# angelocatalani/neural-network-compression

Hardware: AMD Instinct MI355X
Metric: weights/sec through prune+k-means (K=256) (higher is better)
Workload: dtype f32

## Files before the change

include/nnc.h:

```cpp
#ifndef NNC_H
#define NNC_H

#include <stddef.h>
#include <stdint.h>

#ifdef __cplusplus
extern "C" {
#endif

#define NNC_VERSION 100

#define NNC_OK 0
#define NNC_EINVAL (-1)
#define NNC_ENOSPACE (-2)
#define NNC_EHIP (-3)
#define NNC_ENODEV (-4)

#define NNC_KMAX 1040
#define NNC_CHUNK 8192

int nnc_version(void);
const char *nnc_last_error(void);
int nnc_device_info(char *arch_out, size_t arch_len, int *cu_count_out);


int nnc_chunk_sums_f32(const float *x, int64_t n, int sqdev, const float *mean_dev, float *chunk_out,
                       void *stream);

#define NNC_FOLD_SUM 0
#define NNC_FOLD_MEAN 1
#define NNC_FOLD_STD 2
int nnc_fold_f32(const float *chunks, int64_t nchunks, int64_t count, int op, const float *scale_dev,
                 float *out_dev, void *stream);


size_t nnc_prune_workspace_bytes(int64_t n);

int nnc_prune_f32(float *x, int64_t n, float q, int std_smooth, uint8_t *mask, float *stats_dev,
                  int64_t *nzeroed_dev, void *ws, size_t ws_bytes, void *stream);

size_t nnc_prune_stats_workspace_bytes(int64_t n);
int nnc_prune_stats_f32(float *x, int64_t n, float q, int std_smooth, uint8_t *mask, float *stats_dev, int64_t *nzeroed_dev,
                        float *minmax4_dev, int64_t *signs_dev, void *ws, size_t ws_bytes, void *stream);

int nnc_threshold_mask_f32(float *x, int64_t n, const float *thr_dev, uint8_t *mask, int64_t *nzeroed_dev,
                           void *stream);

int nnc_apply_mask_f32(float *x, const uint8_t *mask, int64_t n, void *stream);


size_t nnc_minmax_workspace_bytes(int64_t n);
int nnc_minmax_f32(const float *x, int64_t n, int skip_zeros, float *out_dev, int64_t *count_dev, void *ws,
                   size_t ws_bytes, void *stream);

int nnc_minmax_signs_f32(const float *x, int64_t n, float *out_dev, int64_t *signs_dev, void *ws, size_t ws_bytes,
                         void *stream);

int32_t nnc_sort_pruned_bounded_bits(float vmin, float vmax, float thr, int64_t n_neg, int64_t n_pos);
size_t nnc_sort_pruned_bounded_workspace_bytes(int64_t n_nonzero);
const int32_t *nnc_sort_pruned_bounded_flag(void *ws, int64_t n_nonzero);
int nnc_sort_pruned_bounded_f32(const float *x, int64_t n, int64_t n_neg, int64_t n_zero, float vmin, float vmax, float thr,
                                float *sorted_out, void *ws, size_t ws_bytes, void *stream);

size_t nnc_layer_stats_workspace_bytes(int64_t n);
int nnc_layer_stats_f32(const float *x, int64_t n, float *out6_dev, int64_t *signs_dev, void *ws, size_t ws_bytes,
                        void *stream);

int nnc_rank_sorted_f32(const float *x_sorted, int64_t n, const float *values_dev, int32_t m, int64_t *ranks_out_dev, void *stream);
int nnc_hist31_f32(const float *x, int64_t n, int skip_zeros, const float *steps32_dev, int64_t *counts_dev,
                   void *stream);


size_t nnc_sort_workspace_bytes(int64_t n);
int nnc_sort_f32(const float *x, int64_t n, float *sorted_out, void *ws, size_t ws_bytes, void *stream);
size_t nnc_sort_pruned_workspace_bytes(int64_t n, int64_t n_neg, int64_t n_zero);
int nnc_sort_pruned_f32(const float *x, int64_t n, int64_t n_neg, int64_t n_zero, float *sorted_out, void *ws,
                        size_t ws_bytes, void *stream);

typedef struct nnc_kmeans_params {
    int64_t n;
    int64_t n_total;
    int32_t k;
    int32_t max_iter;
    int32_t fix_shift;
    int32_t grid_log2;
    int32_t replicas_log2;
    int32_t flags;
    float x_mean;
    float tol;
    float lo, hi;
    const int64_t *prefix_dev;
} nnc_kmeans_params;

#define NNC_KM_TWO_LAUNCH 1
#define NNC_KM_LOOP 2
#define NNC_KM_MASS_IN_PLACE 4
#define NNC_KM_LOOP_KMAX 64

typedef struct nnc_kmeans_status {
    int32_t iter;
    int32_t done;
    int32_t paused;
    int32_t n_empty;
    float shift_tot;
    float tol;
    int32_t k;
    int32_t same_counts;
    int32_t reloc_ties;
    int32_t reloc_multi;
    int32_t n_relocated;
    int32_t n_unproven;
    int32_t n_in_place;
    int32_t n_reloc_null;
} nnc_kmeans_status;

int32_t nnc_fix_shift(float absmax, int64_t n_total);
size_t nnc_kmeans_workspace_bytes(int32_t k);

#define NNC_PREFIX_BLOCK 256
size_t nnc_kmeans_prefix_bytes(int64_t n);
int nnc_kmeans_loop_stats(void *ws, int32_t *out8, void *stream);
int nnc_kmeans_prefix_build(const float *x_sorted, const nnc_kmeans_params *p, int64_t *prefix_dev, void *stream);

int nnc_kmeans_init(void *ws, size_t ws_bytes, const nnc_kmeans_params *p, const float *centers_init_dev,
                    void *stream);
int nnc_kmeans_set_centers(void *ws, const nnc_kmeans_params *p, const float *centers_dev, int centred, void *stream);
int nnc_kmeans_accumulate(const float *x, void *ws, const nnc_kmeans_params *p, void *stream);
int64_t *nnc_kmeans_partials(void *ws);
int nnc_kmeans_finalize(void *ws, int resume, void *stream);
int nnc_kmeans_iterate(const float *x, void *ws, const nnc_kmeans_params *p, int32_t iters, void *stream);
int nnc_kmeans_status_async(void *ws, nnc_kmeans_status *host_out, void *stream);
int nnc_kmeans_status_publish(void *ws, void *host_mapped, uint64_t ticket, void *stream);
int nnc_kmeans_iterate_publish(const float *x, void *ws, const nnc_kmeans_params *p, int32_t iters, void *host_mapped,
                               uint64_t ticket, void *stream);
int nnc_kmeans_fit(const float *x_iter, void *ws, const nnc_kmeans_params *p, int32_t max_batch, int32_t sorted,
                   void *reloc_scratch_dev, size_t reloc_scratch_bytes, void *host_mapped, uint64_t *ticket_io,
                   nnc_kmeans_status *status_out, int32_t *n_windowed_out, void *stream);
int nnc_kmeans_set_done(void *ws, int32_t done_code, void *stream);
int nnc_kmeans_label_counts(const float *x, void *ws, const nnc_kmeans_params *p, int which, int64_t *counts_dev,
                            void *stream);

int nnc_kmeans_get_centers(void *ws, int which, int centred, float *out_dev, void *stream);

int nnc_kmeans_assign(const float *x, void *ws, const nnc_kmeans_params *p, int which, void *labels_out,
                      int label_bytes, float *quant_out, float *dist_out, int64_t *dist_hist4096_dev, void *stream);

int nnc_topm_hist_f32(const float *d, int64_t n, int32_t shift, int32_t width, int32_t prefix_shift, uint32_t prefix,
                      int64_t *hist4096_dev, void *stream);
int nnc_topm_compact_f32(const float *d, const float *x, int64_t n, uint32_t thr_bits, int64_t *keys_dev,
                         int64_t cap, int64_t *count_dev, void *stream);

int nnc_kmeans_relocate(void *ws, const int64_t *keys_sorted_dev, int32_t nkeys, void *stream);

int nnc_kmeans_reloc_candidates(const float *x_sorted, void *ws, const nnc_kmeans_params *p, int32_t window,
                                float *cand_x_dev, int64_t cap, void *win_dev, int32_t *meta_dev, void *stream);
int nnc_kmeans_relocate_checked(void *ws, const float *cand_x_dev, const float *cand_d_dev, const void *win_dev,
                                const int32_t *meta_dev, int32_t n_empty, int64_t *keys_out_dev, void *stream);
int32_t nnc_kmeans_reloc_window(int64_t n, int32_t n_empty);
size_t nnc_kmeans_reloc_scratch_bytes(int32_t k, int32_t window);
int nnc_kmeans_relocate_windowed(const float *x_sorted, void *ws, const nnc_kmeans_params *p, int32_t n_empty,
                                 void *scratch_dev, size_t scratch_bytes, void *stream);
int nnc_kmeans_reloc_select_local(const float *x_sorted, void *ws, const nnc_kmeans_params *p, int32_t n_empty,
                                  void *scratch_dev, size_t scratch_bytes, int64_t *keys_out_dev, void *stream);
int32_t *nnc_kmeans_reloc_flag(void *ws);
int nnc_kmeans_relocate_if_proven(void *ws, const int64_t *keys_sorted_dev, int32_t nkeys, void *stream);
int nnc_labels_equal(const void *a, const void *b, int64_t n, int label_bytes, int32_t *flag_dev, void *stream);
int nnc_ref_sums_f32(const float *x, int64_t n, float x_mean, const void *labels, int32_t label_bytes, int32_t k,
                     float *sums_out_dev, int64_t *counts_out_dev, void *stream);
int nnc_kmeans_set_done_if(void *ws, const int32_t *flag_dev, int32_t done_code, void *stream);

int nnc_bincount(const void *labels, int label_bytes, int64_t n, int32_t k, int64_t *counts_dev, void *stream);

#define NNC_REF_NMAX 4096
#define NNC_REF_KMAX 128
int nnc_kmeans_fit_reference_f32(const float *x, int32_t n, const float *centers_init_dev, int32_t k, int32_t max_iter, float tol,
                                 uint8_t *labels_out, float *values_out, float *centers_out, int64_t *counts_out,
                                 void *result_dev, void *stream);

#define NNC_INIT_LINEAR 0
#define NNC_INIT_DENSITY 1
#define NNC_LAYER_DONE 0
#define NNC_LAYER_HOST 1
#define NNC_ARITH_FIXED 0
#define NNC_ARITH_REFERENCE 1
typedef struct nnc_layer_params {
    float q;
    int32_t prune;
    int32_t std_smooth;
    int32_t bits;
    int32_t mode;
    int32_t want_values;
    int32_t km_flags;
    int32_t reserved;
} nnc_layer_params;
typedef struct nnc_layer_result {
    int32_t status, k, label_bytes, arith;
    int32_t n_iter, stop, n_relocations, n_reloc_windowed, reloc_ties, reloc_multi;
    float sigma, threshold;
    int64_t n_zeroed, total_bits;
    float centers[NNC_KMAX];
    int64_t counts[NNC_KMAX];
    uint8_t code_lengths[NNC_KMAX];
} nnc_layer_result;
size_t nnc_compress_layer_workspace_bytes(int64_t n, int32_t k);
size_t nnc_compress_layer_host_bytes(void);
int nnc_compress_layer_f32(float *x, int64_t n, const nnc_layer_params *p, uint8_t *mask_out, void *labels_out, float *values_out,
                           void *ws_dev, size_t ws_bytes, void *host_pinned, size_t host_bytes, uint64_t *ticket_io,
                           nnc_layer_result *result, void *stream);
int nnc_host_linspace_f32(float start, float stop, int32_t num, float *out);
int nnc_host_cdf(const float *steps32, const int64_t *counts31, float *xnew300, double *cdf300);
int nnc_host_density_init(const float *xnew300, const double *cdf300, int32_t bits, float *space_out);

int32_t nnc_kmeanspp_trials(int32_t k);
size_t nnc_kmeanspp_workspace_bytes(int64_t n, int32_t k);
int nnc_kmeanspp_seed_f32(const float *x, int64_t n, float x_mean, int32_t k, int64_t first_id, const double *uniforms_dev,
                          float *seeds_out_dev, int64_t *seed_ids_out_dev, void *ws, size_t ws_bytes, void *stream);

int nnc_centroid_grad_f32(const float *grad, const void *labels, int label_bytes, int64_t n, int32_t k, int32_t fix_shift,
                          int64_t *sums_dev, int64_t *counts_dev, int64_t *nonfinite_dev, void *stream);
int nnc_gather_f32(const float *centers_dev, int32_t k, const void *labels, int label_bytes, int64_t n, float *out, void *stream);

int64_t nnc_cbmm_workspace_bytes(int64_t m, int64_t kdim, int64_t ncols, int label_bytes);
#define NNC_CBMM_NONE 0
#define NNC_CBMM_STREAM 1
#define NNC_CBMM_TILED 2
#define NNC_CBMM_BIAS 3
#define NNC_CBMM_P_PATH 0
#define NNC_CBMM_P_VB 1
#define NNC_CBMM_P_MT 2
#define NNC_CBMM_P_COPIES 3
#define NNC_CBMM_P_ENTRIES 4
#define NNC_CBMM_P_SPLITS 5
#define NNC_CBMM_P_RPS 6
#define NNC_CBMM_P_ALIGNED 7
#define NNC_CBMM_P_LDS 8
#define NNC_CBMM_P_COL_TILES 9
#define NNC_CBMM_P_ROW_TILES 10
#define NNC_CBMM_P_WORKSPACE 11
#define NNC_CBMM_PLAN_LEN 12
int nnc_cbmm_plan(int64_t m, int64_t kdim, int64_t ncols, int label_bytes, int32_t k, int32_t cus, uint64_t labels_addr, int64_t *out);
int nnc_cbmm_f32(const float *x, int64_t m, int64_t kdim, const void *labels, int label_bytes, int64_t ncols, const float *centers_dev, int32_t k,
                 const float *bias_dev, int32_t relu, float *y, void *workspace, int64_t workspace_bytes, void *stream);

#define NNC_DT_F32 0
#define NNC_DT_BF16 1
#define NNC_DT_F16 2
#define NNC_CBMM_MFMA 5
#define NNC_CBMM_H16_P_DTYPE 12
#define NNC_CBMM_H16_PLAN_LEN 13
int64_t nnc_cbmm_h16_workspace_bytes(int64_t m, int64_t kdim, int64_t ncols, int label_bytes);
int nnc_cbmm_h16_plan(int x_dtype, int64_t m, int64_t kdim, int64_t ncols, int label_bytes, int32_t k, int32_t cus, uint64_t labels_addr, int64_t *out);
int nnc_cbmm_h16(const void *x, int x_dtype, int64_t m, int64_t kdim, const void *labels, int label_bytes, int64_t ncols, const float *centers_dev,
                 int32_t k, const float *bias_dev, int32_t relu, void *y, int y_dtype, void *workspace, int64_t workspace_bytes, void *stream);

#define NNC_CBMM_GROUPED_P_GROUP_ROWS 13
#define NNC_CBMM_GROUPED_P_GROUPS 14
#define NNC_CBMM_GROUPED_P_MAX_GROUPS_PER_SPLIT 15
#define NNC_CBMM_GROUPED_PLAN_LEN 16
int64_t nnc_cbmm_grouped_workspace_bytes(int x_dtype, int64_t m, int64_t kdim, int64_t ncols);
int nnc_cbmm_grouped_plan(int x_dtype, int64_t m, int64_t kdim, int64_t ncols, int32_t k, int64_t group_rows, int32_t cus, uint64_t labels_addr, int64_t *out);
int nnc_cbmm_grouped(const void *x, int x_dtype, int64_t m, int64_t kdim, const void *labels, int64_t ncols, const float *centers_dev, int32_t k,
                     int64_t group_rows, const float *bias_dev, int32_t relu, void *y, int y_dtype, void *workspace, int64_t workspace_bytes, void *stream);

#define NNC_CBMM_ZERO 4
#define NNC_CBDX_P_PATH 0
#define NNC_CBDX_P_VB 1
#define NNC_CBDX_P_MT 2
#define NNC_CBDX_P_COPIES 3
#define NNC_CBDX_P_ENTRIES 4
#define NNC_CBDX_P_SPLITS 5
#define NNC_CBDX_P_CPS 6
#define NNC_CBDX_P_ALIGNED 7
#define NNC_CBDX_P_LDS 8
#define NNC_CBDX_P_COL_TILES 9
#define NNC_CBDX_P_ROW_TILES 10
#define NNC_CBDX_P_WORKSPACE 11
#define NNC_CBDX_PLAN_LEN 12
#define NNC_CBDC_P_PATH 0
#define NNC_CBDC_P_VB 1
#define NNC_CBDC_P_MT 2
#define NNC_CBDC_P_COPIES 3
#define NNC_CBDC_P_SPLITS 4
#define NNC_CBDC_P_RPS 5
#define NNC_CBDC_P_ALIGNED 6
#define NNC_CBDC_P_LDS 7
#define NNC_CBDC_P_COL_TILES 8
#define NNC_CBDC_P_ROW_TILES 9
#define NNC_CBDC_P_TERMS_LOG2 10
#define NNC_CBDC_P_WORKSPACE 11
#define NNC_CBDC_PLAN_LEN 12
int64_t nnc_cbmm_dx_workspace_bytes(int64_t m, int64_t kdim, int64_t ncols, int label_bytes);
int nnc_cbmm_dx_plan(int64_t m, int64_t kdim, int64_t ncols, int label_bytes, int32_t k, int32_t cus, uint64_t labels_addr, int64_t *out);
int nnc_cbmm_dx_f32(const float *g, int64_t m, int64_t kdim, const void *labels, int label_bytes, int64_t ncols, const float *centers_dev, int32_t k,
                    float *dx, void *workspace, int64_t workspace_bytes, void *stream);
// ... 221 lines not shown
```

neural_network_compression_amd/_native.py:

```python
from __future__ import annotations

import ctypes
import os

from . import build as _build

c_void_p = ctypes.c_void_p
c_int = ctypes.c_int
c_i32 = ctypes.c_int32
c_i64 = ctypes.c_int64
c_f32 = ctypes.c_float
c_size = ctypes.c_size_t

NNC_OK = 0
NNC_KMAX = 1040
NNC_CHUNK = 8192
FOLD_SUM, FOLD_MEAN, FOLD_STD = 0, 1, 2
NNC_KM_TWO_LAUNCH = 1
NNC_KM_LOOP = 2
NNC_KM_MASS_IN_PLACE = 4
NNC_KM_LOOP_KMAX = 64
CBMM_NONE, CBMM_STREAM, CBMM_TILED, CBMM_BIAS = 0, 1, 2, 3
CBMM_PLAN_LEN = 12
CBMM_PLAN_FIELDS = ("path", "vb", "mt", "copies", "entries", "splits", "rps", "aligned", "lds", "col_tiles", "row_tiles", "workspace")
# ... 24 lines not shown
CBPK_PLAN_LEN = 14
CBPK_PLAN_FIELDS = ("path", "vb", "mt", "cols", "xrows", "table", "copies", "entries", "splits", "rps", "lds", "col_tiles", "row_tiles", "workspace")
CBPK_GROUPED_PLAN_LEN = 19
CBPK_GROUPED_PLAN_FIELDS = CBPK_PLAN_FIELDS + ("dtype", "group_rows", "groups", "max_groups_per_split", "tables")
CBPKDX_PLAN_LEN = 12
CBPKDX_PLAN_FIELDS = ("path", "vb", "mt", "cols", "copies", "entries", "splits", "cps", "lds", "col_tiles", "row_tiles", "workspace")
CBPKDC_PLAN_LEN = 12
CBPKDC_PLAN_FIELDS = ("path", "vb", "mt", "cols", "copies", "splits", "rps", "lds", "col_tiles", "row_tiles", "terms_log2", "workspace")
CBPKGRAD_GROUPED_PLAN_LEN = 17
_CBPKGRAD_GROUPED_TAIL = _CBGRAD_GROUPED_TAIL + ("held",)
CBPKDX_GROUPED_PLAN_FIELDS = CBPKDX_PLAN_FIELDS + _CBPKGRAD_GROUPED_TAIL
CBPKDC_GROUPED_PLAN_FIELDS = CBPKDC_PLAN_FIELDS + _CBPKGRAD_GROUPED_TAIL
CBSPDX_PLAN_LEN = 11
CBSPDX_PLAN_FIELDS = ("path", "mt", "segs", "copies", "entries", "splits", "cps", "lds", "col_tiles", "row_tiles", "workspace")
CBSPDC_PLAN_LEN = 11
CBSPDC_PLAN_FIELDS = ("path", "mt", "segs", "copies", "splits", "rps", "lds", "col_tiles", "row_tiles", "terms_log2", "workspace")
CBSPGRAD_H16_PLAN_LEN = 12
CBSPDX_H16_PLAN_FIELDS = CBSPDX_PLAN_FIELDS + ("dtype",)
CBSPDC_H16_PLAN_FIELDS = CBSPDC_PLAN_FIELDS + ("dtype",)


class NativeLibraryError(RuntimeError):
    pass


class NncError(RuntimeError):
    def __init__(self, code: int, message: str):
        super().__init__(f"nnc error {code}: {message}")
        self.code = code


class KMeansParams(ctypes.Structure):
    _fields_ = [
        ("n", c_i64), ("n_total", c_i64), ("k", c_i32), ("max_iter", c_i32), ("fix_shift", c_i32),
        ("grid_log2", c_i32), ("replicas_log2", c_i32), ("flags", c_i32),
        ("x_mean", c_f32), ("tol", c_f32), ("lo", c_f32), ("hi", c_f32),
        ("prefix_dev", c_void_p),
    ]


class KMeansStatus(ctypes.Structure):
    _fields_ = [
        ("iter", c_i32), ("done", c_i32), ("paused", c_i32), ("n_empty", c_i32),
        ("shift_tot", c_f32), ("tol", c_f32), ("k", c_i32), ("same_counts", c_i32),
        ("reloc_ties", c_i32), ("reloc_multi", c_i32), ("n_relocated", c_i32), ("n_unproven", c_i32),
        ("n_in_place", c_i32), ("n_reloc_null", c_i32),
    ]


class LayerParams(ctypes.Structure):
    _fields_ = [("q", c_f32), ("prune", c_i32), ("std_smooth", c_i32), ("bits", c_i32), ("mode", c_i32), ("want_values", c_i32),
                ("km_flags", c_i32), ("reserved", c_i32)]


class LayerResult(ctypes.Structure):
    _fields_ = [
        ("status", c_i32), ("k", c_i32), ("label_bytes", c_i32), ("arith", c_i32),
        ("n_iter", c_i32), ("stop", c_i32), ("n_relocations", c_i32), ("n_reloc_windowed", c_i32), ("reloc_ties", c_i32), ("reloc_multi", c_i32),
        ("sigma", c_f32), ("threshold", c_f32),
        ("n_zeroed", c_i64), ("total_bits", c_i64),
        ("centers", c_f32 * NNC_KMAX), ("counts", c_i64 * NNC_KMAX), ("code_lengths", ctypes.c_uint8 * NNC_KMAX),
    ]


SIGNATURES = {
    "nnc_version": (c_int, []),
    "nnc_last_error": (ctypes.c_char_p, []),
    "nnc_device_info": (c_int, [ctypes.c_char_p, c_size, ctypes.POINTER(c_int)]),
    "nnc_chunk_sums_f32": (c_int, [c_void_p, c_i64, c_int, c_void_p, c_void_p, c_void_p]),
    "nnc_fold_f32": (c_int, [c_void_p, c_i64, c_i64, c_int, c_void_p, c_void_p, c_void_p]),
    "nnc_prune_workspace_bytes": (c_size, [c_i64]),
    "nnc_prune_f32": (c_int, [c_void_p, c_i64, c_f32, c_int, c_void_p, c_void_p, c_void_p, c_void_p, c_size, c_void_p]),
    "nnc_sort_pruned_bounded_bits": (c_i32, [c_f32, c_f32, c_f32, c_i64, c_i64]),
    "nnc_sort_pruned_bounded_workspace_bytes": (c_size, [c_i64]),
    "nnc_sort_pruned_bounded_flag": (c_void_p, [c_void_p, c_i64]),
    "nnc_sort_pruned_bounded_f32": (c_int, [c_void_p, c_i64, c_i64, c_i64, c_f32, c_f32, c_f32, c_void_p, c_void_p, c_size, c_void_p]),
    "nnc_prune_stats_workspace_bytes": (c_size, [c_i64]),
    "nnc_prune_stats_f32": (c_int, [c_void_p, c_i64, c_f32, c_int, c_void_p, c_void_p, c_void_p, c_void_p, c_void_p, c_void_p, c_size, c_void_p]),
    "nnc_threshold_mask_f32": (c_int, [c_void_p, c_i64, c_void_p, c_void_p, c_void_p, c_void_p]),
    "nnc_apply_mask_f32": (c_int, [c_void_p, c_void_p, c_i64, c_void_p]),
    "nnc_minmax_workspace_bytes": (c_size, [c_i64]),
    "nnc_minmax_f32": (c_int, [c_void_p, c_i64, c_int, c_void_p, c_void_p, c_void_p, c_size, c_void_p]),
    "nnc_minmax_signs_f32": (c_int, [c_void_p, c_i64, c_void_p, c_void_p, c_void_p, c_size, c_void_p]),
    "nnc_layer_stats_workspace_bytes": (c_size, [c_i64]),
    "nnc_layer_stats_f32": (c_int, [c_void_p, c_i64, c_void_p, c_void_p, c_void_p, c_size, c_void_p]),
    "nnc_rank_sorted_f32": (c_int, [c_void_p, c_i64, c_void_p, c_i32, c_void_p, c_void_p]),
    "nnc_hist31_f32": (c_int, [c_void_p, c_i64, c_int, c_void_p, c_void_p, c_void_p]),
    "nnc_sort_workspace_bytes": (c_size, [c_i64]),
    "nnc_sort_f32": (c_int, [c_void_p, c_i64, c_void_p, c_void_p, c_size, c_void_p]),
    "nnc_sort_pruned_workspace_bytes": (c_size, [c_i64, c_i64, c_i64]),
    "nnc_sort_pruned_f32": (c_int, [c_void_p, c_i64, c_i64, c_i64, c_void_p, c_void_p, c_size, c_void_p]),
    "nnc_fix_shift": (c_i32, [c_f32, c_i64]),
    "nnc_kmeans_workspace_bytes": (c_size, [c_i32]),
    "nnc_kmeans_prefix_bytes": (c_size, [c_i64]),
    "nnc_kmeans_loop_stats": (c_int, [c_void_p, c_void_p, c_void_p]),
    "nnc_kmeans_prefix_build": (c_int, [c_void_p, ctypes.POINTER(KMeansParams), c_void_p, c_void_p]),
    "nnc_kmeans_init": (c_int, [c_void_p, c_size, ctypes.POINTER(KMeansParams), c_void_p, c_void_p]),
    "nnc_kmeans_set_centers": (c_int, [c_void_p, ctypes.POINTER(KMeansParams), c_void_p, c_int, c_void_p]),
    "nnc_kmeans_accumulate": (c_int, [c_void_p, c_void_p, ctypes.POINTER(KMeansParams), c_void_p]),
    "nnc_kmeans_partials": (c_void_p, [c_void_p]),
    "nnc_kmeans_finalize": (c_int, [c_void_p, c_int, c_void_p]),
    "nnc_kmeans_iterate": (c_int, [c_void_p, c_void_p, ctypes.POINTER(KMeansParams), c_i32, c_void_p]),
    "nnc_kmeans_status_async": (c_int, [c_void_p, ctypes.POINTER(KMeansStatus), c_void_p]),
    "nnc_kmeans_status_publish": (c_int, [c_void_p, c_void_p, ctypes.c_uint64, c_void_p]),
    "nnc_kmeans_iterate_publish": (c_int, [c_void_p, c_void_p, ctypes.POINTER(KMeansParams), c_i32, c_void_p, ctypes.c_uint64, c_void_p]),
    "nnc_kmeans_fit": (c_int, [c_void_p, c_void_p, ctypes.POINTER(KMeansParams), c_i32, c_i32, c_void_p, c_size, c_void_p,
                               ctypes.POINTER(ctypes.c_uint64), ctypes.POINTER(KMeansStatus), ctypes.POINTER(c_i32), c_void_p]),
    "nnc_kmeans_fit_sharded": (c_int, [c_void_p, c_void_p, c_void_p, ctypes.POINTER(KMeansParams), ctypes.c_int64, c_i32, c_i32, c_void_p, c_size,
                                       c_void_p, ctypes.POINTER(ctypes.c_uint64), ctypes.POINTER(KMeansStatus), ctypes.POINTER(c_i32), c_void_p]),
    "nnc_kmeans_set_done": (c_int, [c_void_p, c_i32, c_void_p]),
    "nnc_kmeans_label_counts": (c_int, [c_void_p, c_void_p, ctypes.POINTER(KMeansParams), c_int, c_void_p, c_void_p]),
    "nnc_kmeans_get_centers": (c_int, [c_void_p, c_int, c_int, c_void_p, c_void_p]),
    "nnc_kmeans_assign": (c_int, [c_void_p, c_void_p, ctypes.POINTER(KMeansParams), c_int, c_void_p, c_int, c_void_p, c_void_p, c_void_p, c_void_p]),
    "nnc_topm_hist_f32": (c_int, [c_void_p, c_i64, c_i32, c_i32, c_i32, ctypes.c_uint32, c_void_p, c_void_p]),
    "nnc_topm_compact_f32": (c_int, [c_void_p, c_void_p, c_i64, ctypes.c_uint32, c_void_p, c_i64, c_void_p, c_void_p]),
    "nnc_kmeans_relocate": (c_int, [c_void_p, c_void_p, c_i32, c_void_p]),
    "nnc_kmeans_reloc_candidates": (c_int, [c_void_p, c_void_p, ctypes.POINTER(KMeansParams), c_i32, c_void_p, c_i64, c_void_p, c_void_p, c_void_p]),
    "nnc_kmeans_relocate_checked": (c_int, [c_void_p, c_void_p, c_void_p, c_void_p, c_void_p, c_i32, c_void_p, c_void_p]),
    "nnc_kmeans_reloc_window": (c_i32, [c_i64, c_i32]),
    "nnc_kmeans_reloc_scratch_bytes": (c_size, [c_i32, c_i32]),
    "nnc_kmeans_relocate_windowed": (c_int, [c_void_p, c_void_p, ctypes.POINTER(KMeansParams), c_i32, c_void_p, c_size, c_void_p]),
    "nnc_kmeans_reloc_select_local": (c_int, [c_void_p, c_void_p, ctypes.POINTER(KMeansParams), c_i32, c_void_p, c_size, c_void_p, c_void_p]),
    "nnc_kmeans_reloc_flag": (c_void_p, [c_void_p]),
    "nnc_kmeans_relocate_if_proven": (c_int, [c_void_p, c_void_p, c_i32, c_void_p]),
    "nnc_labels_equal": (c_int, [c_void_p, c_void_p, c_i64, c_int, c_void_p, c_void_p]),
    "nnc_ref_sums_f32": (c_int, [c_void_p, c_i64, ctypes.c_float, c_void_p, c_i32, c_i32, c_void_p, c_void_p, c_void_p]),
    "nnc_kmeans_set_done_if": (c_int, [c_void_p, c_void_p, c_i32, c_void_p]),
    "nnc_bincount": (c_int, [c_void_p, c_int, c_i64, c_i32, c_void_p, c_void_p]),
    "nnc_kmeans_fit_reference_f32": (c_int, [c_void_p, c_i32, c_void_p, c_i32, c_i32, c_f32, c_void_p, c_void_p, c_void_p, c_void_p, c_void_p, c_void_p]),
    "nnc_compress_layer_workspace_bytes": (c_size, [c_i64, c_i32]),
    "nnc_compress_layer_host_bytes": (c_size, []),
    "nnc_compress_layer_f32": (c_int, [c_void_p, c_i64, ctypes.POINTER(LayerParams), c_void_p, c_void_p, c_void_p, c_void_p, c_size, c_void_p, c_size,
                                       ctypes.POINTER(ctypes.c_uint64), ctypes.POINTER(LayerResult), c_void_p]),
    "nnc_host_linspace_f32": (c_int, [c_f32, c_f32, c_i32, c_void_p]),
    "nnc_host_cdf": (c_int, [c_void_p, c_void_p, c_void_p, c_void_p]),
    "nnc_host_density_init": (c_int, [c_void_p, c_void_p, c_i32, c_void_p]),
    "nnc_kmeanspp_trials": (c_i32, [c_i32]),
    "nnc_kmeanspp_workspace_bytes": (c_size, [c_i64, c_i32]),
    "nnc_kmeanspp_seed_f32": (c_int, [c_void_p, c_i64, c_f32, c_i32, c_i64, c_void_p, c_void_p, c_void_p, c_void_p, c_size, c_void_p]),
    "nnc_centroid_grad_f32": (c_int, [c_void_p, c_void_p, c_int, c_i64, c_i32, c_i32, c_void_p, c_void_p, c_void_p, c_void_p]),
    "nnc_gather_f32": (c_int, [c_void_p, c_i32, c_void_p, c_int, c_i64, c_void_p, c_void_p]),
    "nnc_cbmm_workspace_bytes": (c_i64, [c_i64, c_i64, c_i64, c_int]),
    "nnc_cbmm_plan": (c_int, [c_i64, c_i64, c_i64, c_int, c_i32, c_i32, ctypes.c_uint64, ctypes.POINTER(c_i64)]),
    "nnc_cbmm_f32": (c_int, [c_void_p, c_i64, c_i64, c_void_p, c_int, c_i64, c_void_p, c_i32, c_void_p, c_i32, c_void_p, c_void_p, c_i64, c_void_p]),
    "nnc_cbmm_h16_workspace_bytes": (c_i64, [c_i64, c_i64, c_i64, c_int]),
    "nnc_cbmm_h16_plan": (c_int, [c_int, c_i64, c_i64, c_i64, c_int, c_i32, c_i32, ctypes.c_uint64, ctypes.POINTER(c_i64)]),
    "nnc_cbmm_h16": (c_int, [c_void_p, c_int, c_i64, c_i64, c_void_p, c_int, c_i64, c_void_p, c_i32, c_void_p, c_i32, c_void_p, c_int, c_void_p, c_i64,
                             c_void_p]),
    "nnc_cbmm_grouped_workspace_bytes": (c_i64, [c_int, c_i64, c_i64, c_i64]),
    "nnc_cbmm_grouped_plan": (c_int, [c_int, c_i64, c_i64, c_i64, c_i32, c_i64, c_i32, ctypes.c_uint64, ctypes.POINTER(c_i64)]),
    "nnc_cbmm_grouped": (c_int, [c_void_p, c_int, c_i64, c_i64, c_void_p, c_i64, c_void_p, c_i32, c_i64, c_void_p, c_i32, c_void_p, c_int, c_void_p, c_i64,
                                 c_void_p]),
    "nnc_cbmm_dx_workspace_bytes": (c_i64, [c_i64, c_i64, c_i64, c_int]),
    "nnc_cbmm_dx_plan": (c_int, [c_i64, c_i64, c_i64, c_int, c_i32, c_i32, ctypes.c_uint64, ctypes.POINTER(c_i64)]),
    "nnc_cbmm_dx_f32": (c_int, [c_void_p, c_i64, c_i64, c_void_p, c_int, c_i64, c_void_p, c_i32, c_void_p, c_void_p, c_i64, c_void_p]),
    "nnc_cbmm_dc_workspace_bytes": (c_i64, [c_i64, c_i64, c_i64, c_int, c_i32]),
    "nnc_cbmm_dc_plan": (c_int, [c_i64, c_i64, c_i64, c_int, c_i32, c_i32, ctypes.c_uint64, ctypes.POINTER(c_i64)]),
    "nnc_cbmm_dc_f32": (c_int, [c_void_p, c_void_p, c_i64, c_i64, c_void_p, c_int, c_i64, c_i32, c_void_p, c_i32, c_void_p, c_i64, c_void_p]),
    "nnc_cbsp_pack_bytes": (c_i64, [c_i64, c_i64, c_int, c_i64]),
    "nnc_cbsp_pack": (c_int, [c_void_p, c_int, c_i64, c_i64, c_i32, c_void_p, c_i64, c_void_p, c_void_p]),
    "nnc_cbsp_unpack": (c_int, [c_void_p, c_i64, c_int, c_i64, c_i64, c_i32, c_i64, c_void_p, c_void_p]),
    "nnc_cbsp_workspace_bytes": (c_i64, [c_i64, c_i64, c_i64, c_int]),
    "nnc_cbsp_plan": (c_int, [c_i64, c_i64, c_i64, c_int, c_i32, c_i32, ctypes.POINTER(c_i64)]),
    "nnc_cbsp_f32": (c_int, [c_void_p, c_i64, c_i64, c_void_p, c_i64, c_int, c_i64, c_i32, c_i64, c_void_p, c_i32, c_void_p, c_i32, c_void_p,
                             c_void_p, c_i64, c_void_p]),
    "nnc_cbsp_dx_workspace_bytes": (c_i64, [c_i64, c_i64, c_i64, c_int]),
    "nnc_cbsp_dx_plan": (c_int, [c_i64, c_i64, c_i64, c_int, c_i32, c_i32, ctypes.POINTER(c_i64)]),
    "nnc_cbsp_dx_f32": (c_int, [c_void_p, c_i64, c_i64, c_void_p, c_i64, c_int, c_i64, c_i32, c_i64, c_void_p, c_i32, c_void_p, c_void_p, c_i64,
                                c_void_p]),
    "nnc_cbsp_dc_workspace_bytes": (c_i64, [c_i64, c_i64, c_i64, c_int, c_i32]),
    "nnc_cbsp_dc_plan": (c_int, [c_i64, c_i64, c_i64, c_int, c_i32, c_i32, ctypes.POINTER(c_i64)]),
    "nnc_cbsp_dc_f32": (c_int, [c_void_p, c_void_p, c_i64, c_i64, c_void_p, c_i64, c_int, c_i64, c_i32, c_i64, c_i32, c_void_p, c_i32, c_void_p,
                                c_i64, c_void_p]),
    "nnc_cbpk_row_bytes": (c_i64, [c_i64, c_int]),
    "nnc_cbpk_pack_bytes": (c_i64, [c_i64, c_i64, c_int]),
    "nnc_cbpk_pack": (c_int, [c_void_p, c_int, c_i64, c_i64, c_int, c_void_p, c_i64, c_void_p, c_void_p]),
    "nnc_cbpk_unpack": (c_int, [c_void_p, c_i64, c_int, c_i64, c_i64, c_void_p, c_int, c_void_p]),
    "nnc_cbpk_workspace_bytes": (c_i64, [c_i64, c_i64, c_i64, c_int]),
    "nnc_cbpk_plan": (c_int, [c_i64, c_i64, c_i64, c_int, c_i32, c_i32, ctypes.POINTER(c_i64)]),
    "nnc_cbpk_f32": (c_int, [c_void_p, c_i64, c_i64, c_void_p, c_i64, c_int, c_i64, c_void_p, c_i32, c_void_p, c_i32, c_void_p, c_void_p, c_i64,
                             c_void_p]),
    "nnc_cbpk_grouped_workspace_bytes": (c_i64, [c_int, c_i64, c_i64, c_i64, c_int]),
    "nnc_cbpk_grouped_plan": (c_int, [c_int, c_i64, c_i64, c_i64, c_int, c_i32, c_i64, c_i32, ctypes.POINTER(c_i64)]),
    "nnc_cbpk_grouped": (c_int, [c_void_p, c_int, c_i64, c_i64, c_void_p, c_i64, c_int, c_i64, c_void_p, c_i32, c_i64, c_void_p, c_i32, c_void_p, c_int,
                                 c_void_p, c_i64, c_void_p]),
    "nnc_cbpk_dx_workspace_bytes": (c_i64, [c_i64, c_i64, c_i64, c_int]),
    "nnc_cbpk_dx_plan": (c_int, [c_i64, c_i64, c_i64, c_int, c_i32, c_i32, ctypes.POINTER(c_i64)]),
    "nnc_cbpk_dx_f32": (c_int, [c_void_p, c_i64, c_i64, c_void_p, c_i64, c_int, c_i64, c_void_p, c_i32, c_void_p, c_void_p, c_i64, c_void_p]),
    "nnc_cbpk_dc_workspace_bytes": (c_i64, [c_i64, c_i64, c_i64, c_int, c_i32]),
    "nnc_cbpk_dc_plan": (c_int, [c_i64, c_i64, c_i64, c_int, c_i32, c_i32, ctypes.POINTER(c_i64)]),
    "nnc_cbpk_dc_f32": (c_int, [c_void_p, c_void_p, c_i64, c_i64, c_void_p, c_i64, c_int, c_i64, c_i32, c_void_p, c_i32, c_void_p, c_i64, c_void_p]),
    "nnc_huffman_codes": (c_int, [ctypes.POINTER(ctypes.c_uint8), c_i32, ctypes.POINTER(ctypes.c_uint32)]),
    "nnc_codec_chunks": (c_size, [c_i64]),
    "nnc_huffman_chunk_offsets": (c_int, [c_void_p, c_int, c_i64, c_void_p, c_i32, c_void_p, c_void_p]),
    "nnc_huffman_encode": (c_int, [c_void_p, c_int, c_i64, c_void_p, c_void_p, c_i32, c_void_p, c_void_p, c_i64, c_void_p]),
    "nnc_huffman_decode_tables_bytes": (c_size, []),
    "nnc_huffman_decode_tables": (c_int, [ctypes.POINTER(ctypes.c_uint8), c_i32, c_void_p, c_size]),
    "nnc_huffman_decode": (c_int, [c_void_p, c_void_p, c_i64, c_void_p, c_i32, c_void_p, c_int, c_void_p, c_void_p]),
    "nnc_sparse_entry_offsets": (c_int, [c_void_p, c_int, c_i64, c_i32, c_i32, c_void_p, c_void_p]),
    "nnc_sparse_emit": (c_int, [c_void_p, c_int, c_i64, c_i32, c_i32, c_void_p, c_void_p, c_void_p, c_void_p]),
    "nnc_sparse_expand": (c_int, [c_void_p, c_void_p, c_int, c_void_p, c_i64, c_i32, c_void_p, c_void_p, c_void_p]),
    "nnc_comm_unique_id": (c_int, [c_void_p, c_size]),
    "nnc_comm_init": (c_int, [ctypes.POINTER(c_void_p), c_void_p, c_size, c_i32, c_i32]),
    "nnc_comm_destroy": (c_int, [c_void_p]),
    "nnc_comm_rank": (c_int, [c_void_p]),
    "nnc_comm_world": (c_int, [c_void_p]),
    "nnc_comm_allreduce": (c_int, [c_void_p, c_void_p, c_i64, c_i32, c_i32, c_void_p]),
    "nnc_comm_allgather": (c_int, [c_void_p, c_void_p, c_void_p, c_i64, c_void_p]),
    "nnc_kmeans_iterate_sharded": (c_int, [c_void_p, c_void_p, c_void_p, ctypes.POINTER(KMeansParams), c_i32, c_void_p, ctypes.c_uint64, c_void_p]),
    "nnc_merge_keys": (c_int, [c_void_p, c_i32, c_i32, c_void_p, c_i32, c_void_p]),
    "nnc_kmeans_reloc_scratch_bytes_sharded": (c_size, [c_i32, c_i32, c_i32]),
    "nnc_kmeans_relocate_windowed_sharded": (c_int, [c_void_p, c_void_p, c_void_p, ctypes.POINTER(KMeansParams), c_i32, c_void_p, c_size, c_void_p]),
    "nnc_comm_available": (c_int, []),
    "nnc_profile_tags": (c_int, [ctypes.c_uint32]),
    "nnc_profile_begin": (c_int, [c_i32]),
    "nnc_profile_end": (c_int, [ctypes.POINTER(c_f32), ctypes.POINTER(c_i32), c_i64, ctypes.POINTER(c_i64)]),
    "nnc_huffman_lengths": (c_int, [ctypes.POINTER(c_i64), c_i32, ctypes.POINTER(ctypes.c_uint8), ctypes.POINTER(c_i64), ctypes.POINTER(c_i64)]),
}

# ... 95 lines not shown
```

neural_network_compression_amd/csrc/nnc_hip.hip:

```cpp
#include "nnc_common.hpp"
#include "nnc_km_shared.hpp"


extern "C" size_t nnc_kmeans_workspace_bytes(int32_t k)
{
    (void)k;
    return sizeof(KmWs) + 256;
}

extern "C" int32_t nnc_fix_shift(float absmax, int64_t n_total)
{
    int L = 1;
    while (((int64_t)1 << L) < n_total && L < 62) L++;
    if (!(absmax > 0.0f) || !std::isfinite(absmax)) return 0;
    int P = 0;
    (void)std::frexp((double)absmax, &P);
    return std::min(28, 62 - L) - P;
}

__device__ __forceinline__ int fix_f32(float v, int Sft)
{
    return (int)rintf(ldexpf(v, Sft));
}

// ... 1742 lines not shown
    }
}

__global__ void k_cells_prepare(KmWs *__restrict__ ws, int which) { ws->tab[ws->cur ^ (which & 1)].n_ovf = 0; }

__device__ __forceinline__ void km_cells_body(KmWs *__restrict__ ws, nnc_kmeans_status *host_st, unsigned long long *host_ticket,
                                              unsigned long long ticket, int force, int which, int spec, const int bid)
{
    __shared__ int gcell[NNC_KMAX], hcell[NNC_KMAX];
    if (spec && !ws->spec_go) return;
    if (host_st && bid == 0 && threadIdx.x == 0) {
        *host_st = ws->st;
        __threadfence_system();
        *reinterpret_cast<volatile unsigned long long *>(host_ticket) = ticket;
    }
    if (!force && !ws->cells_pending) return;
    const int G = 1 << ws->glog2;
    const int g = bid * KM_THREADS + threadIdx.x;
    if ((int)(bid * KM_THREADS) >= G) return;
    KmTab *tab = &ws->tab[ws->cur ^ (which & 1)];
    const int ku = force ? tab->ku : ws->ku_cur;
    if (!force) {
        for (int p = threadIdx.x; p < ku; p += KM_THREADS) { gcell[p] = tab->gc[p]; hcell[p] = tab->hc[p]; }
        __syncthreads();
    } else {
        const double U = 5.9604644775390625e-08;
        const double lo = (double)ws->p.lo, inv = (double)ws->inv;
        const double ra = inv > 0.0 ? (1.0 - 4.0 * U) / inv * (1.0 - 4.0 * U) : 0.0;
        const double rb = inv > 0.0 ? (1.0 + 4.0 * U) / inv * (1.0 + 4.0 * U) : 0.0;
        for (int p = threadIdx.x; p < ku; p += KM_THREADS) {
            const double left = tab->zl[p], right = tab->zr[p];
            int gp = G - 1, hp_ = 0;
            if (inv > 0.0) {
                const double qa = (right - lo) / ra;
                gp = (qa >= (double)(G - 1)) ? (G - 1) : (qa < 0.0 ? -1 : (int)(qa * (1.0 + 1e-12)));
                if (gp > G - 1) gp = G - 1;
                const double qb = ((left - lo) / rb - 1.0) * (1.0 - 1e-12);
                if (qb <= 0.0) hp_ = 0;
                else if (qb >= (double)G) hp_ = G;
                else { hp_ = (int)qb; if ((double)hp_ < qb) hp_++; }
            }
            gcell[p] = gp; hcell[p] = hp_;
        }
        __syncthreads();
        for (int off = 1; off < ku; off <<= 1) {
            int a[2], b[2];
            for (int r = 0; r < 2; r++) {
                const int q = threadIdx.x + r * KM_THREADS;
                a[r] = (q < ku) ? ((q >= off) ? max(gcell[q], gcell[q - off]) : gcell[q]) : 0;
                b[r] = (q < ku) ? ((q + off < ku) ? min(hcell[q], hcell[q + off]) : hcell[q]) : 0;
            }
            __syncthreads();
            for (int r = 0; r < 2; r++) {
                const int q = threadIdx.x + r * KM_THREADS;
                if (q < ku) { gcell[q] = a[r]; hcell[q] = b[r]; }
            }
            __syncthreads();
        }
    }
    if (g >= G) return;
    tab->cell[g] = km_cell_entry(g, G, ku, gcell, hcell, &tab->n_ovf, tab->ovf);
}

__global__ __launch_bounds__(KM_THREADS) void k_cells(KmWs *__restrict__ ws, nnc_kmeans_status *host_st,
                                                      unsigned long long *host_ticket, unsigned long long ticket,
                                                      int force = 0, int which = 0, int spec = 0)
{
    km_cells_body(ws, host_st, host_ticket, ticket, force, which, spec, (int)blockIdx.x);
}


static bool km_fused(const nnc_kmeans_params *p)
{
    int glog2, rlog2;
    km_defaults(p, &glog2, &rlog2);
    return p->k <= KM_FUSE_KMAX && glog2 <= KM_FUSE_GLOG2;
}

static bool km_one_launch_fit(const nnc_kmeans_params *p, const float *x)
{
    return p->prefix_dev && p->n > 0 && p->n == p->n_total && km_fused(p) && (reinterpret_cast<uintptr_t>(x) & 15) == 0;
}

static int km_ensure_cells(KmWs *w, const nnc_kmeans_params *p, int which, void *stream)
{
    if (!p->prefix_dev) return NNC_OK;
    hipLaunchKernelGGL(k_cells_prepare, dim3(1), dim3(1), 0, S(stream), w, which);
    LAUNCHCHK("k_cells_prepare");
    hipLaunchKernelGGL(k_cells, dim3(KM_GMAX / KM_THREADS), dim3(KM_THREADS), 0, S(stream), w, (nnc_kmeans_status *)nullptr,
                       (unsigned long long *)nullptr, 0ull, 1, which);
    LAUNCHCHK("k_cells");
    return NNC_OK;
}

int km_launch_finalize(KmWs *w, const nnc_kmeans_params *p, int mode, int resume, void *stream, void *host_mapped,
                       uint64_t ticket, bool cond, const float *reloc_xs)
{
    const int k = p ? p->k : 0;
    bool fused = false;
    if (p && mode != FIN_PACK_ONLY) fused = km_fused(p);
    const bool lazy = p && p->prefix_dev;
    const bool cells = mode != FIN_PACK_ONLY && !fused && !lazy;
    unsigned char *hb = reinterpret_cast<unsigned char *>(host_mapped);
    nnc_kmeans_status *hs = reinterpret_cast<nnc_kmeans_status *>(hb);
    unsigned long long *ht = reinterpret_cast<unsigned long long *>(hb ? hb + sizeof(nnc_kmeans_status) : nullptr);
    nnc_kmeans_status *fs = cells ? nullptr : hs;
#define KM_LAUNCH_FIN(NT, FUSED, THREADS) NNC_LAUNCH_PROF(NNC_PROF_FINALIZE, (k_finalize<NT, FUSED>), dim3(1), dim3(THREADS), 0, S(stream), w, mode, resume, fs, ht, (unsigned long long)ticket, (lazy ? 1 : 0) | (cond ? 2 : 0) | (k > 0 ? k << 8 : 0), reloc_xs, (long long)(p ? p->n : 0))
#define KM_LAUNCH_FIN_MASS(NT, THREADS) NNC_LAUNCH_PROF(NNC_PROF_FINALIZE, (k_finalize<NT, false, true>), dim3(1), dim3(THREADS), 0, S(stream), w, mode, resume, fs, ht, (unsigned long long)ticket, (lazy ? 1 : 0) | (cond ? 2 : 0) | (k > 0 ? k << 8 : 0), reloc_xs, (long long)(p ? p->n : 0))
    const bool mass = p && (p->flags & NNC_KM_MASS_IN_PLACE) && reloc_xs && !fused && k > 64;
    if (fused) KM_LAUNCH_FIN(64, true, KM_THREADS);
    else if (k > 0 && k <= 64) KM_LAUNCH_FIN(64, false, 64);
    else if (k > 0 && k <= 256) { if (mass) KM_LAUNCH_FIN_MASS(256, 256); else KM_LAUNCH_FIN(256, false, 256); }
    else { if (mass) KM_LAUNCH_FIN_MASS(KM_THREADS, KM_THREADS); else KM_LAUNCH_FIN(KM_THREADS, false, KM_THREADS); }
#undef KM_LAUNCH_FIN_MASS
#undef KM_LAUNCH_FIN
    LAUNCHCHK("k_finalize");
    if (cells) {
        hipLaunchKernelGGL(k_cells, dim3(KM_GMAX / KM_THREADS), dim3(KM_THREADS), 0, S(stream), w, hs, ht, (unsigned long long)ticket, 0, 0);
        LAUNCHCHK("k_cells");
    }
    return NNC_OK;
}

int km_check(void *ws, const nnc_kmeans_params *p, const char *who)
{
    if (!ws || !p) return fail(NNC_EINVAL, std::string(who) + ": null workspace/params");
    if (p->k < 1 || p->k > NNC_KMAX - 8) return fail(NNC_EINVAL, std::string(who) + ": k out of range");
    if (p->n < 0 || p->n_total < p->n) return fail(NNC_EINVAL, std::string(who) + ": bad n / n_total");
    if ((reinterpret_cast<uintptr_t>(ws) & 15) != 0) return fail(NNC_EINVAL, std::string(who) + ": workspace must be 16-byte aligned");
    return NNC_OK;
}

__device__ __forceinline__ void km_init_body(KmWs *ws, const nnc_kmeans_params &p, int glog2, int rlog2, float inv,
                                             const float *__restrict__ centers_init)
{
    const int tid = threadIdx.x;
    if (tid == 0) {
        ws->st.iter = 0; ws->st.done = 0; ws->st.paused = 0; ws->st.n_empty = 0;
        ws->st.shift_tot = 0.0f; ws->st.tol = p.tol; ws->st.k = p.k; ws->st.same_counts = 0;
        ws->st.reloc_ties = 0; ws->st.reloc_multi = 0; ws->st.n_relocated = 0; ws->st.n_unproven = 0; ws->st.n_in_place = 0; ws->st.n_reloc_null = 0; ws->spec_go = 0;
        ws->p = p; ws->cur = 0; ws->glog2 = glog2; ws->rlog2 = rlog2; ws->inv = inv; ws->reloc_fail = 0; ws->cells_pending = 0;
    }
    for (int j = tid; j < p.k; j += KM_THREADS) {
        float c = centers_init[j] - p.x_mean;
        ws->c[0][j] = c; ws->c[1][j] = c;
    }
    for (int i = tid; i < KM_NSHARD * NNC_KMAX; i += KM_THREADS) {
        (&ws->shard_sum[0][0])[i] = 0; (&ws->shard_cnt[0][0])[i] = 0;
    }
    for (int i = tid; i < 2 * NNC_KMAX; i += KM_THREADS) { ws->partials[i] = 0; ws->partials_local[i] = 0; }
    for (int i = tid; i < NNC_KMAX; i += KM_THREADS) { ws->prev_counts[i] = -1; ws->q_w0[i] = 0ull; ws->q_w1[i] = 0ull; ws->q_next[i] = 0; ws->hint_a[i] = -1; ws->hint_b[i] = -1; }
    for (int i = tid; i < 2 * NNC_KMAX; i += KM_THREADS) { ws->kl_hL[i] = 0.0f; ws->kl_hR[i] = 0.0f; }
    if (tid == 0) { ws->q_n = 0; ws->q_searched = 0; ws->help_hint = 0; ws->help_pad = 0; ws->wide = 0; ws->kl_budget = 0; }
    if (tid < 8) ws->kl_stats[tid] = 0;
    if (tid < 24) ws->kl_trace[tid] = 0ull;
}

__global__ __launch_bounds__(KM_THREADS) void k_km_init(KmWs *ws, nnc_kmeans_params p, int glog2, int rlog2, float inv,
                                                        const float *__restrict__ centers_init)
{
    km_init_body(ws, p, glog2, rlog2, inv, centers_init);
}

__global__ __launch_bounds__(KM_THREADS) void k_km_init_finalize(KmWs *ws, nnc_kmeans_params p, int glog2, int rlog2, float inv,
                                                                 const float *__restrict__ centers_init)
{
    km_init_body(ws, p, glog2, rlog2, inv, centers_init);
    __syncthreads();
    __builtin_amdgcn_fence(__ATOMIC_ACQUIRE, "agent");
    km_finalize_kernel<KM_THREADS, false, false>(ws, FIN_INIT, 0, nullptr, nullptr, 0ull, 1 | (p.k << 8), nullptr, 0);
}

extern "C" int nnc_kmeans_init(void *ws, size_t ws_bytes, const nnc_kmeans_params *p, const float *centers_init_dev,
                               void *stream)
{
    int rc = km_check(ws, p, "nnc_kmeans_init");
    if (rc) return rc;
    if (!centers_init_dev) return fail(NNC_EINVAL, "nnc_kmeans_init: null centers");
    if (ws_bytes < nnc_kmeans_workspace_bytes(p->k)) return fail(NNC_ENOSPACE, "nnc_kmeans_init: workspace too small");
    if (!std::isfinite(p->x_mean) || !std::isfinite(p->tol) || !std::isfinite(p->lo) || !std::isfinite(p->hi))
        return fail(NNC_EINVAL, "nnc_kmeans_init: Input X contains NaN or infinity (mean / variance / range of the data are not finite)");
    int glog2, rlog2;
    km_defaults(p, &glog2, &rlog2);
    float inv = 0.0f;
    double range = (double)p->hi - (double)p->lo;
    if (range > 0.0) inv = (float)(((double)(1 << glog2)) / range * (1.0 - 1.0 / 1048576.0));
    if (!std::isfinite(inv)) inv = 0.0f;
    KmWs *w = reinterpret_cast<KmWs *>(ws);
#ifndef KM_INIT_TWO
    if (p->k > 256 && !km_fused(p) && p->prefix_dev) {
        hipLaunchKernelGGL(k_km_init_finalize, dim3(1), dim3(KM_THREADS), 0, S(stream), w, *p, glog2, rlog2, inv, centers_init_dev);
        LAUNCHCHK("k_km_init_finalize");
        return NNC_OK;
    }
#endif
    hipLaunchKernelGGL(k_km_init, dim3(1), dim3(KM_THREADS), 0, S(stream), w, *p, glog2, rlog2, inv, centers_init_dev);
    LAUNCHCHK("k_km_init");
    return km_launch_finalize(w, p, FIN_INIT, 0, stream);
}

__global__ __launch_bounds__(KM_THREADS) void k_km_set_centers(KmWs *ws, const float *__restrict__ centers, int centred)
{
    const int tid = threadIdx.x;
    const int k = ws->p.k, cur = ws->cur;
    const float mean = ws->p.x_mean;
    for (int j = tid; j < k; j += KM_THREADS) ws->c[cur][j] = centred ? centers[j] : (centers[j] - mean);
    for (int j = tid; j < NNC_KMAX; j += KM_THREADS) ws->prev_counts[j] = -1;
    if (tid == 0) { ws->st.done = 0; ws->st.paused = 0; ws->st.n_empty = 0; ws->st.same_counts = 0; ws->reloc_fail = 0; }
}

extern "C" int nnc_kmeans_set_centers(void *ws, const nnc_kmeans_params *p, const float *centers_dev, int centred, void *stream)
{
    int rc = km_check(ws, p, "nnc_kmeans_set_centers");
    if (rc) return rc;
    if (!centers_dev) return fail(NNC_EINVAL, "nnc_kmeans_set_centers: null centers");
    KmWs *w = reinterpret_cast<KmWs *>(ws);
    hipLaunchKernelGGL(k_km_set_centers, dim3(1), dim3(KM_THREADS), 0, S(stream), w, centers_dev, centred);
    LAUNCHCHK("k_km_set_centers");
    return km_launch_finalize(w, p, FIN_INIT, 0, stream);
}

static int km_grid(int64_t n, size_t lds_bytes)
{
    int64_t blocks = ((n + 7) / 8 + KM_THREADS - 1) / KM_THREADS;
    if (blocks < 1) blocks = 1;
    int per_cu = (lds_bytes + 1024 <= 80 * 1024) ? 2 : 1;
    int mult_q = 4;
#ifdef NNC_DIAG
    static int mult_env = -1;
    if (mult_env < 0) { const char *e = getenv("NNC_KM_GRID_QUARTERS"); mult_env = e ? atoi(e) : 4; if (mult_env < 1) mult_env = 4; }
    mult_q = mult_env;
#endif
    return (int)std::min<int64_t>(blocks, (int64_t)cu_count() * per_cu * mult_q / 4);
}

#ifdef NNC_DIAG
__global__ void k_debug_clock(int iters, float *out)
{
    float a = threadIdx.x * 1e-3f, b = 1.0001f;
    unsigned long long t0 = __builtin_amdgcn_s_memtime();
    unsigned long long r0 = __builtin_amdgcn_s_memrealtime();
    for (int i = 0; i < iters; i++) { a = a * b + 0.5f; b = b * 0.99999f + 1e-6f; }
    unsigned long long t1 = __builtin_amdgcn_s_memtime();
    unsigned long long r1 = __builtin_amdgcn_s_memrealtime();
    if (threadIdx.x == 0) {
        out[2 * blockIdx.x] = (float)((double)(t1 - t0) / (double)(r1 - r0) * 0.1);
        out[2 * blockIdx.x + 1] = (float)((double)(r1 - r0) * 0.01);
    }
    if (a + b == 123.456f) out[0] = a;
}

extern "C" int nnc_debug_kl_trace(void *ws, unsigned long long *out8)
{
    if (!ws || !out8) return fail(NNC_EINVAL, "nnc_debug_kl_trace: null pointer");
    HIPCHK(hipMemcpy(out8, reinterpret_cast<KmWs *>(ws)->kl_trace, 24 * sizeof(unsigned long long), hipMemcpyDeviceToHost));
    return NNC_OK;
}

extern "C" int nnc_debug_set_trace(unsigned long long *buf_dev)
{
    HIPCHK(hipMemcpyToSymbol(HIP_SYMBOL(g_km_trace), &buf_dev, sizeof(buf_dev)));
    unsigned long long *fin = buf_dev ? buf_dev + 6 * 1024 : nullptr;
    HIPCHK(hipMemcpyToSymbol(HIP_SYMBOL(g_fin_trace), &fin, sizeof(fin)));
    return NNC_OK;
}

extern "C" int nnc_debug_clock(int blocks, int iters, float *out_dev, void *stream)
{
    hipLaunchKernelGGL(k_debug_clock, dim3(blocks), dim3(256), 0, S(stream), iters, out_dev);
    LAUNCHCHK("k_debug_clock");
// ... 270 lines not shown
                           (unsigned long long)ticket);
        LAUNCHCHK("k_fit_small");
        return NNC_OK;
    }
    for (int i = 0; i < iters; i++) {
        if ((rc = km_launch_accumulate(x, w, &p, stream))) return rc;
        const bool last = i == std::max(0, (int)iters - 1 - lag);
        if ((rc = km_launch_finalize(w, &p, FIN_FROM_SHARDS, 0, stream, last ? host_mapped : nullptr, ticket, false,
                                     (reloc_in_place && p.prefix_dev) ? x : nullptr))) return rc;
    }
    return NNC_OK;
}

extern "C" int nnc_kmeans_status_async(void *ws, nnc_kmeans_status *host_out, void *stream)
{
    if (!ws || !host_out) return fail(NNC_EINVAL, "nnc_kmeans_status_async: null pointer");
    HIPCHK(hipMemcpyAsync(host_out, &reinterpret_cast<KmWs *>(ws)->st, sizeof(nnc_kmeans_status), hipMemcpyDeviceToHost, S(stream)));
    return NNC_OK;
}

__global__ void k_publish_status(const KmWs *ws, nnc_kmeans_status *host_st, unsigned long long *host_ticket, unsigned long long ticket)
{
    *host_st = ws->st;
    __threadfence_system();
    *reinterpret_cast<volatile unsigned long long *>(host_ticket) = ticket;
}

extern "C" int nnc_kmeans_status_publish(void *ws, void *host_mapped, uint64_t ticket, void *stream)
{
    if (!ws || !host_mapped || (reinterpret_cast<uintptr_t>(host_mapped) & 7) != 0) return fail(NNC_EINVAL, "nnc_kmeans_status_publish: null or unaligned pointer");
    unsigned char *b = reinterpret_cast<unsigned char *>(host_mapped);
    hipLaunchKernelGGL(k_publish_status, dim3(1), dim3(1), 0, S(stream), reinterpret_cast<const KmWs *>(ws),
                       reinterpret_cast<nnc_kmeans_status *>(b), reinterpret_cast<unsigned long long *>(b + sizeof(nnc_kmeans_status)),
                       (unsigned long long)ticket);
    LAUNCHCHK("k_publish_status");
    return NNC_OK;
}

__global__ __launch_bounds__(256) void k_publish_bytes(const unsigned long long *__restrict__ src, unsigned long long *__restrict__ dst_host, int nwords,
                                                       unsigned long long *host_ticket, unsigned long long ticket)
{
    for (int i = threadIdx.x; i < nwords; i += 256) dst_host[i] = src[i];
    __threadfence_system();
    __syncthreads();
    if (threadIdx.x == 0) *reinterpret_cast<volatile unsigned long long *>(host_ticket) = ticket;
}

int nnc_publish_bytes_(const void *src_dev, void *dst_host_mapped, int nbytes, void *host_ticket, uint64_t ticket, void *stream)
{
    if (!src_dev || !dst_host_mapped || !host_ticket || nbytes < 0 || (nbytes & 7) || ((reinterpret_cast<uintptr_t>(src_dev) | reinterpret_cast<uintptr_t>(dst_host_mapped)) & 7))
        return fail(NNC_EINVAL, "publish: bad argument");
    hipLaunchKernelGGL(k_publish_bytes, dim3(1), dim3(256), 0, S(stream), reinterpret_cast<const unsigned long long *>(src_dev),
                       reinterpret_cast<unsigned long long *>(dst_host_mapped), nbytes / 8, reinterpret_cast<unsigned long long *>(host_ticket), (unsigned long long)ticket);
    LAUNCHCHK("k_publish_bytes");
    return NNC_OK;
}

__global__ void k_set_done(KmWs *ws, int code) { ws->st.done = code; }

extern "C" int nnc_kmeans_set_done(void *ws, int32_t done_code, void *stream)
{
    if (!ws) return fail(NNC_EINVAL, "nnc_kmeans_set_done: null workspace");
    hipLaunchKernelGGL(k_set_done, dim3(1), dim3(1), 0, S(stream), reinterpret_cast<KmWs *>(ws), done_code);
    LAUNCHCHK("k_set_done");
    return NNC_OK;
}

__global__ void k_get_centers(const KmWs *ws, int which, int centred, float *out)
{
    const int k = ws->p.k;
    const float *c = ws->c[ws->cur ^ (which & 1)];
    const float mean = ws->p.x_mean;
    for (int j = threadIdx.x; j < k; j += blockDim.x) out[j] = centred ? c[j] : (c[j] + mean);
}

extern "C" int nnc_kmeans_get_centers(void *ws, int which, int centred, float *out_dev, void *stream)
{
    if (!ws || !out_dev) return fail(NNC_EINVAL, "nnc_kmeans_get_centers: null pointer");
    hipLaunchKernelGGL(k_get_centers, dim3(1), dim3(256), 0, S(stream), reinterpret_cast<const KmWs *>(ws), which, centred, out_dev);
    LAUNCHCHK("k_get_centers");
    return NNC_OK;
}

static int km_assign(const float *x, void *ws, const nnc_kmeans_params *pp, int which, void *labels_out,
                     int label_bytes, float *quant_out, float *dist_out, int64_t *dist_hist4096_dev,
                     const int *n_dev, void *stream)
{
    int rc = km_check(ws, pp, "nnc_kmeans_assign");
    if (rc) return rc;
    const nnc_kmeans_params p = *pp;
    if (p.n > 0 && !x) return fail(NNC_EINVAL, "nnc_kmeans_assign: null x");
    if (labels_out && label_bytes != 1 && label_bytes != 2) return fail(NNC_EINVAL, "nnc_kmeans_assign: label_bytes must be 1 or 2");
    if (labels_out && label_bytes == 1 && p.k > 256) return fail(NNC_EINVAL, "nnc_kmeans_assign: k > 256 needs 2-byte labels");
    if (p.n == 0) return NNC_OK;
    if ((rc = km_set_lds_attr())) return rc;
    int glog2, rlog2;
    km_defaults(&p, &glog2, &rlog2);
    if (dist_hist4096_dev && !dist_out) return fail(NNC_EINVAL, "nnc_kmeans_assign: the distance histogram needs dist_out");
    size_t lds = km_lds_bytes(p.k, glog2, rlog2, false) + (dist_hist4096_dev ? 4096 * sizeof(unsigned) : 0);
    const bool vec = ((reinterpret_cast<uintptr_t>(x) | reinterpret_cast<uintptr_t>(quant_out) | reinterpret_cast<uintptr_t>(dist_out)) & 15) == 0 &&
                     (reinterpret_cast<uintptr_t>(labels_out) & (size_t)(4 * label_bytes - 1)) == 0;
    int grid = km_grid(p.n, lds);
    KmWs *w = reinterpret_cast<KmWs *>(ws);
    if ((rc = km_ensure_cells(w, &p, which, stream))) return rc;
    unsigned long long *dh = reinterpret_cast<unsigned long long *>(dist_hist4096_dev);
    if (dh) HIPCHK(hipMemsetAsync(dh, 0, 4096 * sizeof(int64_t), S(stream)));
    if (label_bytes == 2) {
        if (vec) NNC_LAUNCH_PROF(NNC_PROF_ASSIGN_LABELS, (k_assign<1, true, uint16_t>), dim3(grid), dim3(KM_THREADS), lds, S(stream), x, p.n, w, which, reinterpret_cast<uint16_t *>(labels_out), quant_out, dist_out, dh, n_dev);
        else NNC_LAUNCH_PROF(NNC_PROF_ASSIGN_LABELS, (k_assign<1, false, uint16_t>), dim3(grid), dim3(KM_THREADS), lds, S(stream), x, p.n, w, which, reinterpret_cast<uint16_t *>(labels_out), quant_out, dist_out, dh, n_dev);
    } else {
        if (vec) NNC_LAUNCH_PROF(NNC_PROF_ASSIGN_LABELS, (k_assign<1, true, uint8_t>), dim3(grid), dim3(KM_THREADS), lds, S(stream), x, p.n, w, which, reinterpret_cast<uint8_t *>(labels_out), quant_out, dist_out, dh, n_dev);
        else NNC_LAUNCH_PROF(NNC_PROF_ASSIGN_LABELS, (k_assign<1, false, uint8_t>), dim3(grid), dim3(KM_THREADS), lds, S(stream), x, p.n, w, which, reinterpret_cast<uint8_t *>(labels_out), quant_out, dist_out, dh, n_dev);
    }
    LAUNCHCHK("k_assign<labels>");
    return NNC_OK;
}

extern "C" int nnc_kmeans_assign(const float *x, void *ws, const nnc_kmeans_params *pp, int which, void *labels_out,
                                 int label_bytes, float *quant_out, float *dist_out, int64_t *dist_hist4096_dev,
                                 void *stream)
{
    return km_assign(x, ws, pp, which, labels_out, label_bytes, quant_out, dist_out, dist_hist4096_dev, nullptr, stream);
}



__global__ __launch_bounds__(256) void k_topm_hist(const float *__restrict__ d, int64_t n, int shift, unsigned mask, int pshift,
                                                   unsigned prefix, unsigned long long *__restrict__ hist)
{
    __shared__ unsigned h[4096];
    for (int i = threadIdx.x; i < 4096; i += 256) h[i] = 0;
    __syncthreads();
    const int64_t tid = (int64_t)blockIdx.x * blockDim.x + threadIdx.x;
    const int64_t nthreads = (int64_t)gridDim.x * blockDim.x;
    const int64_t nvec = ((reinterpret_cast<uintptr_t>(d) & 15) == 0) ? (n >> 2) : 0;
    const uint4 *d4 = reinterpret_cast<const uint4 *>(d);
    unsigned run_bin = 0xFFFFFFFFu, run_cnt = 0;
#define TH1(u) do { const unsigned u_ = (u); if (pshift < 0 || (u_ >> pshift) == prefix) { const unsigned b_ = (u_ >> shift) & mask; \
        if (b_ != run_bin) { if (run_cnt) atomicAdd(&h[run_bin], run_cnt); run_bin = b_; run_cnt = 0; } run_cnt++; } } while (0)
    for (int64_t v = tid; v < nvec; v += nthreads) {
        const uint4 a = d4[v];
        TH1(a.x); TH1(a.y); TH1(a.z); TH1(a.w);
    }
    for (int64_t i = (nvec << 2) + tid; i < n; i += nthreads) TH1(__float_as_uint(d[i]));
#undef TH1
    if (run_cnt) atomicAdd(&h[run_bin], run_cnt);
    __syncthreads();
    for (int i = threadIdx.x; i < 4096; i += 256)
        if (h[i]) atomicAdd(&hist[i], (unsigned long long)h[i]);
}

__global__ __launch_bounds__(256) void k_topm_compact(const float *__restrict__ d, const float *__restrict__ x, int64_t n,
                                                      unsigned thr_bits, long long *__restrict__ keys, long long cap,
                                                      unsigned long long *__restrict__ count)
{
    const int64_t tid = (int64_t)blockIdx.x * blockDim.x + threadIdx.x;
    const int64_t nthreads = (int64_t)gridDim.x * blockDim.x;
    for (int64_t i = tid; i < n; i += nthreads) {
        const unsigned u = __float_as_uint(d[i]);
        if (u >= thr_bits) {
            const unsigned long long slot = atomicAdd(count, 1ull);
            if ((long long)slot < cap) keys[slot] = ((long long)u << 32) | (long long)f32_ordered_bits(x[i]);
        }
    }
}

extern "C" int nnc_topm_hist_f32(const float *d, int64_t n, int32_t shift, int32_t width, int32_t prefix_shift, uint32_t prefix,
                                 int64_t *hist4096_dev, void *stream)
{
    if (n < 0 || !hist4096_dev || (n > 0 && !d) || shift < 0 || shift > 31 || prefix_shift > 31 || width < 1 || width > 12)
        return fail(NNC_EINVAL, "nnc_topm_hist_f32: bad argument");
    HIPCHK(hipMemsetAsync(hist4096_dev, 0, 4096 * sizeof(int64_t), S(stream)));
    if (n == 0) return NNC_OK;
    int grid = stream_grid((n + 3) / 4, 256, 2);
    hipLaunchKernelGGL(k_topm_hist, dim3(grid), dim3(256), 0, S(stream), d, n, (int)shift, (1u << width) - 1u, (int)prefix_shift, (unsigned)prefix,
                       reinterpret_cast<unsigned long long *>(hist4096_dev));
    LAUNCHCHK("k_topm_hist");
    return NNC_OK;
}

extern "C" int nnc_topm_compact_f32(const float *d, const float *x, int64_t n, uint32_t thr_bits, int64_t *keys_dev,
                                    int64_t cap, int64_t *count_dev, void *stream)
{
    if (n < 0 || !keys_dev || !count_dev || cap <= 0 || (n > 0 && (!d || !x)))
        return fail(NNC_EINVAL, "nnc_topm_compact_f32: bad argument");
    HIPCHK(hipMemsetAsync(count_dev, 0, sizeof(int64_t), S(stream)));
    if (n == 0) return NNC_OK;
// ... 994 lines not shown
```

neural_network_compression_amd/csrc/nnc_layer.hip:

```cpp
#include <hip/hip_runtime.h>

#include <algorithm>
#include <cmath>
#include <cstdint>
#include <cstring>
#include <string>
#include <vector>

#include "nnc.h"

int nnc_set_error_(int code, const char *msg);
int nnc_publish_bytes_(const void *src_dev, void *dst_host_mapped, int nbytes, void *host_ticket, uint64_t ticket, void *stream);
int nnc_wait_ticket_(void *host_ticket, uint64_t ticket, void *stream);
int nnc_sort_pruned_bounded_flagged_(const float *x, int64_t n, int64_t n_neg, int64_t n_zero, float vmin, float vmax, float thr,
                                     float *sorted_out, void *ws, size_t ws_bytes, int32_t *flag_dev, void *stream);
extern "C" int nnc_host_linspace_f32(float start, float stop, int32_t num, float *out)
{
    if (num < 0 || (num > 0 && !out)) return nnc_set_error_(NNC_EINVAL, "nnc_host_linspace_f32: bad argument");
    if (num == 0) return NNC_OK;
    const int div = num - 1;
    const volatile float delta = stop - start;
    if (div > 0) {
        const volatile float step = delta / (float)div;
        for (int i = 0; i < num; i++) {
            volatile float y = (float)i;
            if (step == 0.0f) { y = y / (float)div; y = y * delta; }
            else y = y * step;
            y = y + start;
            out[i] = y;
        }
        out[num - 1] = stop;
    } else {
        volatile float y = 0.0f;
        y = y * delta;
        y = y + start;
        out[0] = y;
    }
    return NNC_OK;
}

static void linspace_f64(double start, double stop, int num, double *out)
{
    const int div = num - 1;
    const volatile double delta = stop - start;
    if (div > 0) {
        const volatile double step = delta / (double)div;
        for (int i = 0; i < num; i++) {
            volatile double y = (double)i;
            if (step == 0.0) { y = y / (double)div; y = y * delta; }
            else y = y * step;
            y = y + start;
            out[i] = y;
        }
        out[num - 1] = stop;
    } else if (num == 1) {
        volatile double y = 0.0;
        y = y * delta;
        out[0] = y + start;
    }
}

extern "C" int nnc_host_cdf(const float *steps32, const int64_t *counts31, float *xnew300, double *cdf300)
{
    if (!steps32 || !counts31 || !xnew300 || !cdf300) return nnc_set_error_(NNC_EINVAL, "nnc_host_cdf: null pointer");
    const float *x = steps32;
    int64_t tot = 0;
    for (int i = 0; i < 31; i++) tot += counts31[i];
    double cdf[31];
    volatile double acc = 0.0;
    for (int i = 0; i < 31; i++) {
        const volatile double t = (double)counts31[i] / (double)tot;
        acc = (i == 0) ? (double)t : acc + t;
        cdf[i] = acc;
    }
    const double last = cdf[30];
    for (int i = 0; i < 31; i++) { const volatile double q = cdf[i] / last; cdf[i] = q; }
    float xmin = x[0], xmax = x[0];
    for (int i = 1; i < 31; i++) { xmin = std::min(xmin, x[i]); xmax = std::max(xmax, x[i]); }
    int rc = nnc_host_linspace_f32(xmin, xmax, 300, xnew300);
    if (rc) return rc;
    for (int j = 0; j < 300; j++) {
        const float v = xnew300[j];
        int idx = (int)(std::lower_bound(x, x + 31, v) - x);
        idx = std::min(std::max(idx, 1), 30);
        const int lo = idx - 1, hi = idx;
        const volatile float dx = x[hi] - x[lo];
        const volatile double dy = cdf[hi] - cdf[lo];
        const volatile double slope = dy / (double)dx;
        const volatile float xr = v - x[lo];
        const volatile double prod = slope * (double)xr;
        cdf300[j] = prod + cdf[lo];
    }
    return NNC_OK;
}

extern "C" int nnc_host_density_init(const float *xnew300, const double *cdf300, int32_t bits, float *space_out)
{
    if (!xnew300 || !cdf300 || !space_out || bits < 0 || bits > 10) return nnc_set_error_(NNC_EINVAL, "nnc_host_density_init: bad argument");
    const int k = (1 << bits) + 1;
    std::vector<double> tmp((size_t)k);
    linspace_f64(0.0, 1.0, k, tmp.data());
    bool rising = true;
    for (int j = 1; j < 300; j++) rising = rising && cdf300[j - 1] <= cdf300[j];
    for (int t = 0; rising && t < k; t++) {
        const int hi = (int)(std::lower_bound(cdf300, cdf300 + 300, tmp[t]) - cdf300);
        int best = hi;
        if (hi > 0) {
            const double dl = std::fabs(cdf300[hi - 1] - tmp[t]);
            if (hi == 300 || dl <= std::fabs(cdf300[hi] - tmp[t])) {
                best = hi - 1;
                while (best > 0 && std::fabs(cdf300[best - 1] - tmp[t]) == dl) best--;
            }
        }
        space_out[t] = xnew300[best];
    }
    if (rising) return NNC_OK;
    for (int t = 0; t < k; t++) {
        int best = 0;
        double bd = std::fabs(cdf300[0] - tmp[t]);
        for (int j = 1; j < 300; j++) {
            const double d = std::fabs(cdf300[j] - tmp[t]);
            if (d < bd) { bd = d; best = j; }
        }
        space_out[t] = xnew300[best];
    }
    return NNC_OK;
}

static size_t al(size_t b) { return (b + 255) & ~(size_t)255; }

struct SideStream { int dev = -1; hipStream_t stream = nullptr; hipEvent_t fork = nullptr, sorted = nullptr, join = nullptr; };
static int side_stream(SideStream **out)
{
    static thread_local SideStream side;
    int dev = 0;
    if (hipGetDevice(&dev) != hipSuccess) return nnc_set_error_(NNC_EHIP, "hipGetDevice failed");
    if (side.dev != dev) {
        if (side.stream) { (void)hipStreamDestroy(side.stream); (void)hipEventDestroy(side.fork); (void)hipEventDestroy(side.sorted); (void)hipEventDestroy(side.join); side = SideStream(); }
        if (hipStreamCreateWithFlags(&side.stream, hipStreamNonBlocking) != hipSuccess || hipEventCreateWithFlags(&side.fork, hipEventDisableTiming) != hipSuccess ||
            hipEventCreateWithFlags(&side.sorted, hipEventDisableTiming) != hipSuccess || hipEventCreateWithFlags(&side.join, hipEventDisableTiming) != hipSuccess)
            return nnc_set_error_(NNC_EHIP, "could not create the second stream");
        side.dev = dev;
    }
    *out = &side;
    return NNC_OK;
}

struct LayerLayout {
    size_t prune_ws, stats_out, stats_ws, sorted, sort_ws, km_ws, prefix, reloc, back, small_out, total;
    size_t prune_ws_bytes, stats_ws_bytes, sort_ws_bytes, km_ws_bytes, prefix_bytes, reloc_bytes;
};

static LayerLayout layer_layout(int64_t n, int32_t k)
{
    LayerLayout L;
    size_t o = 0;
    auto take = [&](size_t bytes) { const size_t at = o; o += al(bytes); return at; };
    L.prune_ws_bytes = nnc_prune_stats_workspace_bytes(n);
    L.stats_ws_bytes = std::max(nnc_layer_stats_workspace_bytes(n), nnc_minmax_workspace_bytes(n));
    L.sort_ws_bytes = std::max(std::max(nnc_sort_workspace_bytes(n), nnc_sort_pruned_workspace_bytes(n, 0, (n + 3) / 4)),
                               nnc_sort_pruned_bounded_workspace_bytes(n - (n + 3) / 4));
    L.km_ws_bytes = nnc_kmeans_workspace_bytes(k);
    L.prefix_bytes = nnc_kmeans_prefix_bytes(n);
    L.reloc_bytes = n >= 512 ? nnc_kmeans_reloc_scratch_bytes(k, 256) : 0;
    L.prune_ws = take(std::max<size_t>(L.prune_ws_bytes, 16));
    L.stats_out = take(512);
    L.stats_ws = take(std::max<size_t>(L.stats_ws_bytes, 16));
    L.sorted = take((size_t)n * 4 + 16);
    L.sort_ws = take(std::max<size_t>(L.sort_ws_bytes, 16));
    L.km_ws = take(L.km_ws_bytes);
    L.prefix = take(std::max<size_t>(L.prefix_bytes, 16));
    L.reloc = take(std::max<size_t>(L.reloc_bytes, 16));
    L.back = take((size_t)k * 12);
    L.small_out = take(64 + 256);
    L.total = o + 256;
    return L;
}

extern "C" size_t nnc_compress_layer_workspace_bytes(int64_t n, int32_t k)
{
    if (n < 1 || k < 1 || k > NNC_KMAX - 8) return 0;
    return layer_layout(n, k).total;
}

extern "C" size_t nnc_compress_layer_host_bytes(void) { return 24576; }

#define LCHK(call) do { int rc_ = (call); if (rc_) return rc_; } while (0)
#define LHIP(call) do { hipError_t e_ = (call); if (e_ != hipSuccess) return nnc_set_error_(NNC_EHIP, hipGetErrorString(e_)); } while (0)

extern "C" int nnc_compress_layer_f32(float *x, int64_t n, const nnc_layer_params *lp, uint8_t *mask_out, void *labels_out,
                                      float *values_out, void *ws_dev, size_t ws_bytes, void *host_pinned, size_t host_bytes,
                                      uint64_t *ticket_io, nnc_layer_result *res, void *stream)
{
    if (!x || n < 1 || !lp || !labels_out || !ws_dev || !host_pinned || !ticket_io || !res)
        return nnc_set_error_(NNC_EINVAL, "nnc_compress_layer_f32: null pointer or empty tensor");
    if (lp->bits < 1 || lp->bits > 10 || (lp->mode != NNC_INIT_LINEAR && lp->mode != NNC_INIT_DENSITY))
        return nnc_set_error_(NNC_EINVAL, "nnc_compress_layer_f32: bits in 1..10, mode linear or density");
    if (lp->prune && !mask_out) return nnc_set_error_(NNC_EINVAL, "nnc_compress_layer_f32: pruning needs mask_out");
    const int32_t k = (1 << lp->bits) + (lp->mode == NNC_INIT_DENSITY ? 1 : 0);
    if (n < (int64_t)(1 << lp->bits) + 1) return nnc_set_error_(NNC_EINVAL, "nnc_compress_layer_f32: not enough weights for this many centroids");
    if (host_bytes < nnc_compress_layer_host_bytes() || (reinterpret_cast<uintptr_t>(host_pinned) & 7) != 0)
        return nnc_set_error_(NNC_EINVAL, "nnc_compress_layer_f32: host block too small or unaligned");
    const LayerLayout L = layer_layout(n, k);
    if (ws_bytes < L.total) return nnc_set_error_(NNC_ENOSPACE, "nnc_compress_layer_f32: workspace too small");
    hipStream_t s = reinterpret_cast<hipStream_t>(stream);
    unsigned char *wb = reinterpret_cast<unsigned char *>((reinterpret_cast<uintptr_t>(ws_dev) + 255) & ~(uintptr_t)255);
    unsigned char *hb = reinterpret_cast<unsigned char *>(host_pinned);
    const float *h_f = reinterpret_cast<const float *>(hb + 512);
    const int64_t *h_signs = reinterpret_cast<const int64_t *>(hb + 512 + 32);
    const float *h_prune = reinterpret_cast<const float *>(hb + 512 + 48);
    const int64_t *h_nz = reinterpret_cast<const int64_t *>(hb + 512 + 56);
    int64_t *h_ranks = reinterpret_cast<int64_t *>(hb + 576);
    void *h_ticket = hb + 504;
    auto read_back = [&](const void *src, void *dst, int nbytes) -> int {
        const uint64_t t = ++(*ticket_io);
        int rc = nnc_publish_bytes_(src, dst, nbytes, h_ticket, t, stream);
        if (rc) return rc;
        return nnc_wait_ticket_(h_ticket, t, stream);
    };
    std::memset(res, 0, sizeof(*res));
    res->k = k;
    res->label_bytes = k <= 256 ? 1 : 2;

    float *out6 = reinterpret_cast<float *>(wb + L.stats_out);
    int64_t *signs = reinterpret_cast<int64_t *>(wb + L.stats_out + 32);
    float *pstats = reinterpret_cast<float *>(wb + L.stats_out + 48);
    int64_t *nzeroed = reinterpret_cast<int64_t *>(wb + L.stats_out + 56);
    if (lp->prune)
        LCHK(nnc_prune_stats_f32(x, n, lp->q, lp->std_smooth ? 1 : 0, mask_out, pstats, nzeroed, out6 + 2, signs, wb + L.prune_ws, L.prune_ws_bytes, stream));
    else
        LCHK(nnc_minmax_signs_f32(x, n, out6 + 2, signs, wb + L.stats_ws, L.stats_ws_bytes, stream));
    const bool short_tensor = n <= NNC_REF_NMAX && k <= NNC_REF_KMAX;
    if ((short_tensor && lp->mode != NNC_INIT_LINEAR) || (!short_tensor && n < 512)) {
        if (lp->prune) {
            LCHK(read_back(out6, hb + 512, 64));
            res->sigma = h_prune[0]; res->threshold = h_prune[1]; res->n_zeroed = h_nz[0];
        }
        res->status = NNC_LAYER_HOST;
        return NNC_OK;
    }
    float space[NNC_KMAX];
    unsigned char *back = wb + L.back;
    int64_t *counts_d = reinterpret_cast<int64_t *>(back);
    float *centers_d = reinterpret_cast<float *>(back + (size_t)k * 8);
    int64_t *h_counts = reinterpret_cast<int64_t *>(hb + 1024);
    float *h_centers = reinterpret_cast<float *>(hb + 1024 + (size_t)k * 8);
    float *h_steps = reinterpret_cast<float *>(hb + 896), *h_space = reinterpret_cast<float *>(hb + 16384);

    if (short_tensor) {
        LCHK(read_back(out6, hb + 512, 64));
        LCHK(nnc_host_linspace_f32(h_f[2], h_f[3], k, space));
        std::memcpy(h_space, space, (size_t)k * 4);
        void *result_d = wb + L.small_out;
        LCHK(nnc_kmeans_fit_reference_f32(x, (int32_t)n, h_space, k, 300, 1e-4f, reinterpret_cast<uint8_t *>(labels_out), lp->want_values ? values_out : nullptr,
                                          centers_d, counts_d, result_d, stream));
        const int back_bytes = (int)al((size_t)k * 12) + 32;
        LCHK(read_back(back, hb + 1024, back_bytes));
        const int32_t *h_res = reinterpret_cast<const int32_t *>(hb + 1024 + al((size_t)k * 12));
        {
            const float *h_resf = reinterpret_cast<const float *>(h_res);
            if (!std::isfinite(h_resf[6]) || !std::isfinite(h_resf[7])) {
                if (lp->prune) { res->sigma = h_prune[0]; res->threshold = h_prune[1]; res->n_zeroed = h_nz[0]; }
                res->status = NNC_LAYER_HOST;
                return NNC_OK;
            }
        }
        res->n_iter = h_res[0]; res->stop = h_res[1]; res->n_relocations = h_res[2]; res->reloc_ties = h_res[3]; res->reloc_multi = h_res[4];
        res->arith = NNC_ARITH_REFERENCE;
    } else {
        const int64_t nch = (n + 8191) / 8192;
        float *c1 = reinterpret_cast<float *>(wb + L.stats_ws), *c2 = c1 + nch;
        SideStream *side = nullptr;
        LCHK(side_stream(&side));
        LHIP(hipEventRecord(side->fork, s));
        const uint64_t t_mm = ++(*ticket_io);
        LCHK(nnc_publish_bytes_(out6 + 2, hb + 512 + 8, 56, h_ticket, t_mm, stream));
        LHIP(hipStreamWaitEvent(side->stream, side->fork, 0));
        struct SideJoin {
            SideStream *side; hipStream_t s; bool joined = false;
            ~SideJoin() { if (!joined) { (void)hipEventRecord(side->join, side->stream); (void)hipStreamWaitEvent(s, side->join, 0); (void)hipStreamSynchronize(s); } }
        } side_join{side, s};
        LCHK(nnc_chunk_sums_f32(x, n, 0, nullptr, c1, side->stream));
        LCHK(nnc_fold_f32(c1, nch, n, NNC_FOLD_MEAN, nullptr, out6, side->stream));
        LCHK(nnc_chunk_sums_f32(x, n, 1, out6, c2, side->stream));
        LCHK(nnc_fold_f32(c2, nch, n, NNC_FOLD_MEAN, nullptr, out6 + 1, side->stream));
        void *h_ticket_side = hb + 864;
        const float *h_mv = reinterpret_cast<const float *>(hb + 872);
        const uint64_t t_mv = ++(*ticket_io);
        LCHK(nnc_publish_bytes_(out6, hb + 872, 8, h_ticket_side, t_mv, side->stream));
        LCHK(nnc_wait_ticket_(h_ticket, t_mm, stream));
        const float xmin = h_f[2], xmax = h_f[3], min_nz = h_f[4], max_nz = h_f[5];
        const int64_t n_neg = h_signs[0], n_zero = h_signs[1];
        float *xs = reinterpret_cast<float *>(wb + L.sorted);
        int32_t *oob_d = reinterpret_cast<int32_t *>(wb + L.stats_out + 336);
        const int32_t *h_oob = reinterpret_cast<const int32_t *>(hb + 512 + 336);
        bool bounded = false;
        if (4 * n_zero >= n && lp->prune && nnc_sort_pruned_bounded_bits(xmin, xmax, h_prune[1], n_neg, n - n_neg - n_zero) > 0) {
            LCHK(nnc_sort_pruned_bounded_flagged_(x, n, n_neg, n_zero, xmin, xmax, h_prune[1], xs, wb + L.sort_ws, L.sort_ws_bytes, oob_d, stream));
            bounded = true;
        } else if (4 * n_zero >= n) LCHK(nnc_sort_pruned_f32(x, n, n_neg, n_zero, xs, wb + L.sort_ws, L.sort_ws_bytes, stream));
        else LCHK(nnc_sort_f32(x, n, xs, wb + L.sort_ws, L.sort_ws_bytes, stream));
        LHIP(hipEventRecord(side->sorted, s));
        const bool with_prefix = (reinterpret_cast<uintptr_t>(xs) & 15) == 0;
        int64_t *ranks_d = reinterpret_cast<int64_t *>(wb + L.stats_out + 64);
        h_ranks = reinterpret_cast<int64_t *>(hb + 512 + 64);
        float steps[32];
        if (lp->mode == NNC_INIT_DENSITY) {
            if (!std::isfinite(min_nz)) {
                if (lp->prune) { res->sigma = h_prune[0]; res->threshold = h_prune[1]; res->n_zeroed = h_nz[0]; }
                res->status = NNC_LAYER_HOST;
                return NNC_OK;
            }
            LCHK(nnc_host_linspace_f32(min_nz, max_nz, 32, steps));
            std::memcpy(h_steps, steps, 128);
            LCHK(nnc_rank_sorted_f32(xs, n, h_steps, 32, ranks_d, stream));
        }
        const uint64_t t_rk = ++(*ticket_io);
        LCHK(nnc_publish_bytes_(out6 + 2, hb + 512 + 8, 56 + 33 * 8 + 16, h_ticket, t_rk, stream));
        LCHK(nnc_wait_ticket_(h_ticket_side, t_mv, side->stream));
        const float mean = h_mv[0], var = h_mv[1];
        if (!std::isfinite(mean) || !std::isfinite(var) || !std::isfinite(xmin) || !std::isfinite(xmax)) {
            LCHK(nnc_wait_ticket_(h_ticket, t_rk, stream));
            if (lp->prune) { res->sigma = h_prune[0]; res->threshold = h_prune[1]; res->n_zeroed = h_nz[0]; }
            res->status = NNC_LAYER_HOST;
            return NNC_OK;
        }
        nnc_kmeans_params p;
        std::memset(&p, 0, sizeof(p));
        const volatile float tol = var * 1e-4f;
        const volatile float lo = xmin - mean, hi = xmax - mean;
        p.n = n; p.n_total = n; p.k = k; p.max_iter = 300;
        p.fix_shift = nnc_fix_shift(std::max(std::fabs((float)lo), std::fabs((float)hi)), n);
        p.grid_log2 = 0; p.replicas_log2 = -1; p.flags = lp->km_flags & (NNC_KM_TWO_LAUNCH | NNC_KM_LOOP);
        p.x_mean = mean; p.tol = tol; p.lo = lo; p.hi = hi;
        if (with_prefix) {
            LHIP(hipStreamWaitEvent(side->stream, side->sorted, 0));
            LCHK(nnc_kmeans_prefix_build(xs, &p, reinterpret_cast<int64_t *>(wb + L.prefix), side->stream));
            p.prefix_dev = reinterpret_cast<int64_t *>(wb + L.prefix);
        }
        LHIP(hipEventRecord(side->join, side->stream));
        LCHK(nnc_wait_ticket_(h_ticket, t_rk, stream));
        if (bounded && *h_oob) {
            if (lp->prune) { res->sigma = h_prune[0]; res->threshold = h_prune[1]; res->n_zeroed = h_nz[0]; }
            res->status = NNC_LAYER_HOST;
            return NNC_OK;
        }
        if (lp->mode == NNC_INIT_LINEAR) {
            LCHK(nnc_host_linspace_f32(xmin, xmax, k, space));
        } else {
            int64_t counts31[31];
            for (int b = 0; b < 31; b++) counts31[b] = h_ranks[b + 1] - h_ranks[b];
            for (int b = 0; b < 31; b++)
                if (steps[b] <= 0.0f && 0.0f < steps[b + 1]) { counts31[b] -= n_zero; break; }
            float xnew[300];
            double cdf[300];
            LCHK(nnc_host_cdf(steps, counts31, xnew, cdf));
            LCHK(nnc_host_density_init(xnew, cdf, lp->bits, space));
        }
        std::memcpy(h_space, space, (size_t)k * 4);
        LCHK(nnc_kmeans_init(wb + L.km_ws, L.km_ws_bytes, &p, h_space, stream));
        LHIP(hipStreamWaitEvent(s, side->join, 0));
        side_join.joined = true;
        nnc_kmeans_status st;
        std::memset(&st, 0, sizeof(st));
        int32_t nwin = 0;
        LCHK(nnc_kmeans_fit(xs, wb + L.km_ws, &p, 16, 1, L.reloc_bytes ? wb + L.reloc : nullptr, L.reloc_bytes, hb, ticket_io, &st, &nwin, stream));
        if (!st.done) {
            if (lp->prune) { res->sigma = h_prune[0]; res->threshold = h_prune[1]; res->n_zeroed = h_nz[0]; }
            res->status = NNC_LAYER_HOST;
            return NNC_OK;
        }
        LCHK(nnc_kmeans_get_centers(wb + L.km_ws, 0, 0, centers_d, stream));
        LCHK(nnc_kmeans_label_counts(xs, wb + L.km_ws, &p, 0, counts_d, stream));
        const uint64_t t_back = ++(*ticket_io);
        LCHK(nnc_publish_bytes_(back, hb + 1024, (int)al((size_t)k * 12), h_ticket, t_back, stream));
        LCHK(nnc_kmeans_assign(x, wb + L.km_ws, &p, 0, labels_out, res->label_bytes, lp->want_values ? values_out : nullptr, nullptr, nullptr, stream));
        LCHK(nnc_wait_ticket_(h_ticket, t_back, stream));
        res->n_iter = st.iter; res->stop = st.done; res->n_relocations = nwin - st.n_reloc_null; res->n_reloc_windowed = nwin - st.n_reloc_null;
        res->reloc_ties = st.reloc_ties; res->reloc_multi = st.reloc_multi;
        res->arith = NNC_ARITH_FIXED;
    }
    if (lp->prune) { res->sigma = h_prune[0]; res->threshold = h_prune[1]; res->n_zeroed = h_nz[0]; }
    std::memcpy(res->counts, h_counts, (size_t)k * 8);
    std::memcpy(res->centers, h_centers, (size_t)k * 4);
    int64_t hist[72];
    LCHK(nnc_huffman_lengths(res->counts, k, res->code_lengths, hist, &res->total_bits));
    res->status = NNC_LAYER_DONE;
    return NNC_OK;
}
```

neural_network_compression_amd/csrc/nnc_reduce.hip:

```cpp
#include "nnc_common.hpp"

#define LEAF_PAD 136
#define STEP_ELEMS 1024

template <bool SQDEV>
__device__ __forceinline__ float4 xform4(float4 v, float mean)
{
    if (SQDEV) {
        float a = v.x - mean, b = v.y - mean, c = v.z - mean, d = v.w - mean;
        v.x = a * a; v.y = b * b; v.z = c * c; v.w = d * d;
    }
    return v;
}

template <bool SQDEV>
__device__ __forceinline__ float xform1(float v, float mean)
{
    if (SQDEV) { float a = v - mean; return a * a; }
    return v;
}

struct PwFrame { int start, len, stage; float left; };

template <bool SQDEV, bool VEC>
// ... 234 lines not shown
    const int64_t tid = (int64_t)blockIdx.x * blockDim.x + threadIdx.x;
    const int64_t nthreads = (int64_t)gridDim.x * blockDim.x;
    int64_t done = 0;
    if (VEC) {
        const int64_t nvec = n >> 2;
        float4 *x4 = reinterpret_cast<float4 *>(x);
        const uchar4 *m4 = reinterpret_cast<const uchar4 *>(mask);
        for (int64_t v = tid; v < nvec; v += nthreads) {
            uchar4 m = m4[v];
            if (m.x | m.y | m.z | m.w) {
                float4 a = x4[v];
                a.x = m.x ? 0.0f : a.x; a.y = m.y ? 0.0f : a.y; a.z = m.z ? 0.0f : a.z; a.w = m.w ? 0.0f : a.w;
                x4[v] = a;
            }
        }
        done = nvec << 2;
    }
    for (int64_t i = done + tid; i < n; i += nthreads)
        if (mask[i]) x[i] = 0.0f;
}

extern "C" int nnc_apply_mask_f32(float *x, const uint8_t *mask, int64_t n, void *stream)
{
    if (n < 0 || (n > 0 && (!x || !mask))) return fail(NNC_EINVAL, "nnc_apply_mask_f32: bad argument");
    if (n == 0) return NNC_OK;
    const bool vec = ((reinterpret_cast<uintptr_t>(x) & 15) == 0) && ((reinterpret_cast<uintptr_t>(mask) & 3) == 0);
    int grid = stream_grid((n + 3) / 4, 256, 16);
    if (vec) hipLaunchKernelGGL((k_apply_mask<true>), dim3(grid), dim3(256), 0, S(stream), x, mask, n);
    else hipLaunchKernelGGL((k_apply_mask<false>), dim3(grid), dim3(256), 0, S(stream), x, mask, n);
    LAUNCHCHK("k_apply_mask");
    return NNC_OK;
}

struct MinMaxPartial { float mn, mx; unsigned long long cnt; unsigned long long neg, zer; float mn_nz, mx_nz; };

template <bool VEC>
__global__ __launch_bounds__(256) void k_minmax(const float *__restrict__ x, int64_t n, int skip_zeros,
                                                MinMaxPartial *__restrict__ part)
{
    float mn = INFINITY, mx = -INFINITY, mn_nz = INFINITY, mx_nz = -INFINITY;
    unsigned long long cnt = 0;
    unsigned neg = 0, zer = 0;
    const int64_t tid = (int64_t)blockIdx.x * blockDim.x + threadIdx.x;
    const int64_t nthreads = (int64_t)gridDim.x * blockDim.x;
    int64_t done = 0;
#define MM1(v) do { float v_ = (v); neg += (v_ < 0.0f); const bool z_ = (v_ == 0.0f); zer += z_; if (!z_) { mn_nz = fminf(mn_nz, v_); mx_nz = fmaxf(mx_nz, v_); } \
        bool use_ = !(skip_zeros && z_); if (use_) { mn = fminf(mn, v_); mx = fmaxf(mx, v_); cnt++; } } while (0)
    if (VEC) {
        const int64_t nvec = n >> 2;
        const float4 *x4 = reinterpret_cast<const float4 *>(x);
        for (int64_t v = tid; v < nvec; v += nthreads) {
            float4 a = x4[v];
            MM1(a.x); MM1(a.y); MM1(a.z); MM1(a.w);
        }
        done = nvec << 2;
    }
    for (int64_t i = done + tid; i < n; i += nthreads) MM1(x[i]);
#undef MM1
    unsigned long long negl = neg, zerl = zer;
    for (int off = 32; off > 0; off >>= 1) {
        mn = fminf(mn, __shfl_down(mn, off));
        mx = fmaxf(mx, __shfl_down(mx, off));
        mn_nz = fminf(mn_nz, __shfl_down(mn_nz, off));
        mx_nz = fmaxf(mx_nz, __shfl_down(mx_nz, off));
        cnt += __shfl_down(cnt, off);
        negl += __shfl_down(negl, off);
        zerl += __shfl_down(zerl, off);
    }
    __shared__ MinMaxPartial sh[4];
    if ((threadIdx.x & 63) == 0) { MinMaxPartial q; q.mn = mn; q.mx = mx; q.cnt = cnt; q.neg = negl; q.zer = zerl; q.mn_nz = mn_nz; q.mx_nz = mx_nz; sh[threadIdx.x >> 6] = q; }
    __syncthreads();
    if (threadIdx.x == 0) {
        MinMaxPartial p = sh[0];
        for (int w = 1; w < 4; w++) {
            p.mn = fminf(p.mn, sh[w].mn); p.mx = fmaxf(p.mx, sh[w].mx); p.cnt += sh[w].cnt; p.neg += sh[w].neg; p.zer += sh[w].zer;
            p.mn_nz = fminf(p.mn_nz, sh[w].mn_nz); p.mx_nz = fmaxf(p.mx_nz, sh[w].mx_nz);
        }
        part[blockIdx.x] = p;
    }
}

__global__ __launch_bounds__(256) void k_minmax_final(const MinMaxPartial *__restrict__ part, int nparts,
                                                      float *__restrict__ out, long long *__restrict__ count,
                                                      long long *__restrict__ signs)
{
    float mn = INFINITY, mx = -INFINITY, mn_nz = INFINITY, mx_nz = -INFINITY;
    unsigned long long cnt = 0, neg = 0, zer = 0;
    for (int i = threadIdx.x; i < nparts; i += 256) {
        mn = fminf(mn, part[i].mn); mx = fmaxf(mx, part[i].mx); cnt += part[i].cnt; neg += part[i].neg; zer += part[i].zer;
        mn_nz = fminf(mn_nz, part[i].mn_nz); mx_nz = fmaxf(mx_nz, part[i].mx_nz);
    }
    for (int off = 32; off > 0; off >>= 1) {
        mn = fminf(mn, __shfl_down(mn, off));
        mx = fmaxf(mx, __shfl_down(mx, off));
        mn_nz = fminf(mn_nz, __shfl_down(mn_nz, off));
        mx_nz = fmaxf(mx_nz, __shfl_down(mx_nz, off));
        cnt += __shfl_down(cnt, off);
        neg += __shfl_down(neg, off);
        zer += __shfl_down(zer, off);
    }
    __shared__ MinMaxPartial sh[4];
    if ((threadIdx.x & 63) == 0) { MinMaxPartial q; q.mn = mn; q.mx = mx; q.cnt = cnt; q.neg = neg; q.zer = zer; q.mn_nz = mn_nz; q.mx_nz = mx_nz; sh[threadIdx.x >> 6] = q; }
    __syncthreads();
    if (threadIdx.x == 0) {
        MinMaxPartial p = sh[0];
        for (int w = 1; w < 4; w++) {
            p.mn = fminf(p.mn, sh[w].mn); p.mx = fmaxf(p.mx, sh[w].mx); p.cnt += sh[w].cnt; p.neg += sh[w].neg; p.zer += sh[w].zer;
            p.mn_nz = fminf(p.mn_nz, sh[w].mn_nz); p.mx_nz = fmaxf(p.mx_nz, sh[w].mx_nz);
        }
        out[0] = p.mn; out[1] = p.mx;
        if (count) *count = (long long)p.cnt;
        if (signs) { signs[0] = (long long)p.neg; signs[1] = (long long)p.zer; out[2] = p.mn_nz; out[3] = p.mx_nz; }
    }
}

static int minmax_grid(int64_t n) { return stream_grid((n + 3) / 4, 256, 8); }

extern "C" size_t nnc_minmax_workspace_bytes(int64_t n)
{
    (void)n;
    return (size_t)(cu_count() * 8 + 8) * sizeof(MinMaxPartial);
}

static int minmax_impl(const float *x, int64_t n, int skip_zeros, float *out_dev, int64_t *count_dev, int64_t *signs_dev,
                       void *ws, size_t ws_bytes, void *stream)
{
    if (n <= 0 || !x || !out_dev || !ws) return fail(NNC_EINVAL, "nnc_minmax_f32: bad argument (n must be > 0)");
    if (ws_bytes < nnc_minmax_workspace_bytes(n)) return fail(NNC_ENOSPACE, "nnc_minmax_f32: workspace too small");
    int grid = minmax_grid(n);
    MinMaxPartial *part = reinterpret_cast<MinMaxPartial *>(ws);
    const bool vec = (reinterpret_cast<uintptr_t>(x) & 15) == 0;
    if (vec) NNC_LAUNCH_PROF(NNC_PROF_MINMAX, (k_minmax<true>), dim3(grid), dim3(256), 0, S(stream), x, n, skip_zeros, part);
    else NNC_LAUNCH_PROF(NNC_PROF_MINMAX, (k_minmax<false>), dim3(grid), dim3(256), 0, S(stream), x, n, skip_zeros, part);
    LAUNCHCHK("k_minmax");
    hipLaunchKernelGGL(k_minmax_final, dim3(1), dim3(256), 0, S(stream), part, grid, out_dev, reinterpret_cast<long long *>(count_dev),
                       reinterpret_cast<long long *>(signs_dev));
    LAUNCHCHK("k_minmax_final");
    return NNC_OK;
}

extern "C" int nnc_minmax_f32(const float *x, int64_t n, int skip_zeros, float *out_dev, int64_t *count_dev,
                              void *ws, size_t ws_bytes, void *stream)
{
    return minmax_impl(x, n, skip_zeros, out_dev, count_dev, nullptr, ws, ws_bytes, stream);
}

extern "C" int nnc_minmax_signs_f32(const float *x, int64_t n, float *out_dev, int64_t *signs_dev, void *ws, size_t ws_bytes,
                                    void *stream)
{
    if (!signs_dev) return fail(NNC_EINVAL, "nnc_minmax_signs_f32: null signs_dev");
    return minmax_impl(x, n, 0, out_dev, nullptr, signs_dev, ws, ws_bytes, stream);
}

template <bool VEC>
__global__ __launch_bounds__(256) void k_threshold_stats(float *__restrict__ x, int64_t n, const float *__restrict__ thr_dev,
                                                         uint8_t *__restrict__ mask, unsigned long long *__restrict__ nzeroed,
                                                         MinMaxPartial *__restrict__ part)
{
    const float thr = *thr_dev;
    unsigned cnt = 0, neg = 0, zer = 0;
    float mn = INFINITY, mx = -INFINITY, mn_nz = INFINITY, mx_nz = -INFINITY;
    const int64_t tid = (int64_t)blockIdx.x * blockDim.x + threadIdx.x;
    const int64_t nthreads = (int64_t)gridDim.x * blockDim.x;
    int64_t done = 0;
#define TS1(v) do { const float v_ = (v); neg += (v_ < 0.0f); const bool z_ = (v_ == 0.0f); zer += z_; \
        if (!z_) { mn_nz = fminf(mn_nz, v_); mx_nz = fmaxf(mx_nz, v_); } mn = fminf(mn, v_); mx = fmaxf(mx, v_); } while (0)
    if (VEC) {
        const int64_t nvec = n >> 2;
        float4 *x4 = reinterpret_cast<float4 *>(x);
        uchar4 *m4 = reinterpret_cast<uchar4 *>(mask);
        for (int64_t v = tid; v < nvec; v += nthreads) {
            float4 a = x4[v];
            uchar4 m;
            m.x = fabsf(a.x) < thr; m.y = fabsf(a.y) < thr; m.z = fabsf(a.z) < thr; m.w = fabsf(a.w) < thr;
            cnt += m.x + m.y + m.z + m.w;
            a.x = m.x ? 0.0f : a.x; a.y = m.y ? 0.0f : a.y; a.z = m.z ? 0.0f : a.z; a.w = m.w ? 0.0f : a.w;
            x4[v] = a;
            m4[v] = m;
            TS1(a.x); TS1(a.y); TS1(a.z); TS1(a.w);
        }
        done = nvec << 2;
    }
    for (int64_t i = done + tid; i < n; i += nthreads) {
        float a = x[i];
        const uint8_t m = fabsf(a) < thr;
        cnt += m;
        if (m) { a = 0.0f; x[i] = 0.0f; }
        mask[i] = m;
        TS1(a);
    }
#undef TS1
    unsigned long long negl = neg, zerl = zer, cntl = cnt;
    for (int off = 32; off > 0; off >>= 1) {
        mn = fminf(mn, __shfl_down(mn, off));
        mx = fmaxf(mx, __shfl_down(mx, off));
        mn_nz = fminf(mn_nz, __shfl_down(mn_nz, off));
        mx_nz = fmaxf(mx_nz, __shfl_down(mx_nz, off));
        negl += __shfl_down(negl, off);
        zerl += __shfl_down(zerl, off);
        cntl += __shfl_down(cntl, off);
    }
    __shared__ MinMaxPartial sh[4];
    __shared__ unsigned long long shc[4];
    if ((threadIdx.x & 63) == 0) {
        MinMaxPartial q; q.mn = mn; q.mx = mx; q.cnt = 0; q.neg = negl; q.zer = zerl; q.mn_nz = mn_nz; q.mx_nz = mx_nz;
        sh[threadIdx.x >> 6] = q; shc[threadIdx.x >> 6] = cntl;
    }
    __syncthreads();
    if (threadIdx.x == 0) {
        MinMaxPartial p = sh[0];
        unsigned long long tot = shc[0];
        for (int w = 1; w < 4; w++) {
            p.mn = fminf(p.mn, sh[w].mn); p.mx = fmaxf(p.mx, sh[w].mx); p.neg += sh[w].neg; p.zer += sh[w].zer;
            p.mn_nz = fminf(p.mn_nz, sh[w].mn_nz); p.mx_nz = fmaxf(p.mx_nz, sh[w].mx_nz);
            tot += shc[w];
        }
        part[blockIdx.x] = p;
        if (nzeroed && tot) atomicAdd(nzeroed, tot);
    }
}

extern "C" size_t nnc_prune_stats_workspace_bytes(int64_t n) { return ((nnc_prune_workspace_bytes(n) + 255) & ~(size_t)255) + nnc_minmax_workspace_bytes(n); }

extern "C" int nnc_prune_stats_f32(float *x, int64_t n, float q, int std_smooth, uint8_t *mask, float *stats_dev, int64_t *nzeroed_dev,
                                   float *minmax4_dev, int64_t *signs_dev, void *ws, size_t ws_bytes, void *stream)
{
    if (n <= 0 || !x || !mask || !stats_dev || !minmax4_dev || !signs_dev || !ws) return fail(NNC_EINVAL, "nnc_prune_stats_f32: bad argument (n must be > 0)");
    if (ws_bytes < nnc_prune_stats_workspace_bytes(n)) return fail(NNC_ENOSPACE, "nnc_prune_stats_f32: workspace too small");
    if (std_smooth) {
        float *wsf = reinterpret_cast<float *>(ws);
        float *scal = wsf;
        float *chunks = wsf + 16;
        const int64_t nchunks = (n + NNC_CHUNK - 1) / NNC_CHUNK;
        int rc;
        if ((rc = nnc_chunk_sums_f32(x, n, 0, nullptr, chunks, stream))) return rc;
        if ((rc = nnc_fold_f32(chunks, nchunks, n, NNC_FOLD_MEAN, nullptr, scal, stream))) return rc;
        if ((rc = nnc_chunk_sums_f32(x, n, 1, scal, chunks, stream))) return rc;
        hipLaunchKernelGGL(k_fold, dim3(1), dim3(1024), 0, S(stream), chunks, nchunks, n, (int)NNC_FOLD_STD, (const float *)nullptr, stats_dev, q, 1,
                           reinterpret_cast<unsigned long long *>(nzeroed_dev));
        LAUNCHCHK("k_fold");
    } else {
        hipLaunchKernelGGL(k_set_thr, dim3(1), dim3(1), 0, S(stream), q, stats_dev);
        LAUNCHCHK("k_set_thr");
        if (nzeroed_dev) HIPCHK(hipMemsetAsync(nzeroed_dev, 0, sizeof(int64_t), S(stream)));
    }
    MinMaxPartial *part = reinterpret_cast<MinMaxPartial *>(reinterpret_cast<unsigned char *>(ws) + ((nnc_prune_workspace_bytes(n) + 255) & ~(size_t)255));
    const bool vec = ((reinterpret_cast<uintptr_t>(x) & 15) == 0) && ((reinterpret_cast<uintptr_t>(mask) & 3) == 0);
    const int grid = std::min(stream_grid((n + 3) / 4, 256, 4), cu_count() * 8);
    if (vec) NNC_LAUNCH_PROF(NNC_PROF_THRESHOLD, (k_threshold_stats<true>), dim3(grid), dim3(256), 0, S(stream), x, n, stats_dev + 1, mask, reinterpret_cast<unsigned long long *>(nzeroed_dev), part);
    else NNC_LAUNCH_PROF(NNC_PROF_THRESHOLD, (k_threshold_stats<false>), dim3(grid), dim3(256), 0, S(stream), x, n, stats_dev + 1, mask, reinterpret_cast<unsigned long long *>(nzeroed_dev), part);
    LAUNCHCHK("k_threshold_stats");
    hipLaunchKernelGGL(k_minmax_final, dim3(1), dim3(256), 0, S(stream), part, grid, minmax4_dev, (long long *)nullptr, reinterpret_cast<long long *>(signs_dev));
    LAUNCHCHK("k_minmax_final");
    return NNC_OK;
}

extern "C" size_t nnc_layer_stats_workspace_bytes(int64_t n)
{
    const size_t nch = (size_t)((n + NNC_CHUNK - 1) / NNC_CHUNK);
    return ((2 * nch * sizeof(float) + 255) & ~(size_t)255) + nnc_minmax_workspace_bytes(n);
}

extern "C" int nnc_layer_stats_f32(const float *x, int64_t n, float *out6_dev, int64_t *signs_dev, void *ws, size_t ws_bytes,
                                   void *stream)
{
    if (n <= 0 || !x || !out6_dev || !signs_dev || !ws) return fail(NNC_EINVAL, "nnc_layer_stats_f32: bad argument (n must be > 0)");
    if (ws_bytes < nnc_layer_stats_workspace_bytes(n)) return fail(NNC_ENOSPACE, "nnc_layer_stats_f32: workspace too small");
    const int64_t nch = (n + NNC_CHUNK - 1) / NNC_CHUNK;
    float *c1 = reinterpret_cast<float *>(ws), *c2 = c1 + nch;
    unsigned char *mm_ws = reinterpret_cast<unsigned char *>(ws) + ((2 * (size_t)nch * sizeof(float) + 255) & ~(size_t)255);
    int rc;
    if ((rc = nnc_chunk_sums_f32(x, n, 0, nullptr, c1, stream))) return rc;
    if ((rc = nnc_fold_f32(c1, nch, n, NNC_FOLD_MEAN, nullptr, out6_dev, stream))) return rc;
    if ((rc = nnc_chunk_sums_f32(x, n, 1, out6_dev, c2, stream))) return rc;
    if ((rc = nnc_fold_f32(c2, nch, n, NNC_FOLD_MEAN, nullptr, out6_dev + 1, stream))) return rc;
    return minmax_impl(x, n, 0, out6_dev + 2, nullptr, signs_dev, mm_ws, nnc_minmax_workspace_bytes(n), stream);
}

template <bool VEC>
__global__ __launch_bounds__(256) void k_hist31(const float *__restrict__ x, int64_t n, int skip_zeros,
                                                const float *__restrict__ steps,
                                                unsigned long long *__restrict__ counts)
{
    __shared__ unsigned h[32][32];
    __shared__ float st[32];
    for (int i = threadIdx.x; i < 32 * 32; i += 256) (&h[0][0])[i] = 0;
    if (threadIdx.x < 32) st[threadIdx.x] = steps[threadIdx.x];
    __syncthreads();
    float s[32];
#pragma unroll
    for (int i = 0; i < 32; i++) s[i] = st[i];
    const int rep = threadIdx.x & 31;
    const int64_t tid = (int64_t)blockIdx.x * blockDim.x + threadIdx.x;
    const int64_t nthreads = (int64_t)gridDim.x * blockDim.x;
#define H1(v) do { float v_ = (v); if (!(skip_zeros && v_ == 0.0f)) { int c_ = 0; _Pragma("unroll") for (int i = 0; i < 32; i++) c_ += (v_ >= s[i]); if (c_ >= 1 && c_ <= 31) atomicAdd(&h[c_ - 1][rep], 1u); } } while (0)
    int64_t done = 0;
    if (VEC) {
        const int64_t nvec = n >> 2;
        const float4 *x4 = reinterpret_cast<const float4 *>(x);
        for (int64_t v = tid; v < nvec; v += nthreads) {
            float4 a = x4[v];
            H1(a.x); H1(a.y); H1(a.z); H1(a.w);
        }
        done = nvec << 2;
    }
    for (int64_t i = done + tid; i < n; i += nthreads) H1(x[i]);
#undef H1
    __syncthreads();
    if (threadIdx.x < 31) {
        unsigned long long t = 0;
        for (int r = 0; r < 32; r++) t += h[threadIdx.x][r];
        if (t) atomicAdd(&counts[threadIdx.x], t);
    }
}

extern "C" int nnc_hist31_f32(const float *x, int64_t n, int skip_zeros, const float *steps32_dev,
                              int64_t *counts_dev, void *stream)
{
    if (n < 0 || !steps32_dev || !counts_dev || (n > 0 && !x)) return fail(NNC_EINVAL, "nnc_hist31_f32: bad argument");
    if (n == 0) return NNC_OK;
    int grid = stream_grid((n + 3) / 4, 256, 2);
    const bool vec = (reinterpret_cast<uintptr_t>(x) & 15) == 0;
    if (vec) hipLaunchKernelGGL((k_hist31<true>), dim3(grid), dim3(256), 0, S(stream), x, n, skip_zeros, steps32_dev, reinterpret_cast<unsigned long long *>(counts_dev));
    else hipLaunchKernelGGL((k_hist31<false>), dim3(grid), dim3(256), 0, S(stream), x, n, skip_zeros, steps32_dev, reinterpret_cast<unsigned long long *>(counts_dev));
    LAUNCHCHK("k_hist31");
    return NNC_OK;
}

__global__ __launch_bounds__(64) void k_rank_sorted(const float *__restrict__ xs, long long n, const float *__restrict__ values, int m,
                                                    long long *__restrict__ ranks_out)
{
    const int i = blockIdx.x * 64 + threadIdx.x;
    if (i >= m) return;
    const float v = values[i];
    long long lo = 0, hi = n;
// ... 49 lines not shown
```

neural_network_compression_amd/csrc/nnc_sort.hip:

```cpp
#include <hip/hip_runtime.h>
#include <cmath>
#include <cstdlib>
#include <cstring>

#include <algorithm>
#include <string>

#include "nnc.h"

extern "C" const char *nnc_last_error(void);
int nnc_set_error_(int code, const char *msg);

#ifndef OS_THREADS
#define OS_THREADS 1024
#endif
#define OS_WAVES (OS_THREADS / 64)
#ifndef OS_ITEMS
#define OS_ITEMS 16
#endif
#ifndef OS_BLOCKS_PER_CU
#define OS_BLOCKS_PER_CU 1
#endif
#ifndef OS_RANK_LDS
#define OS_RANK_LDS 1
#endif
#define OS_TILE (OS_THREADS * OS_ITEMS)
#define OS_MAXBITS 9
#define OS_MAXR (1 << OS_MAXBITS)
#define OS_MAXPASS 4
#define OS_SPIN_LIMIT (1 << 22)
#define OSP_THREADS 1024
#define OSP_PER 16
#define OSP_TILE (OSP_THREADS * OSP_PER)

__device__ __forceinline__ unsigned f32_ord(float v)
{
    const unsigned b = __float_as_uint(v);
    return (b & 0x80000000u) ? ~b : (b | 0x80000000u);
}
__device__ __forceinline__ float f32_unord(unsigned o)
{
    return __uint_as_float((o & 0x80000000u) ? (o ^ 0x80000000u) : ~o);
}

struct OsMap { unsigned lo_neg, hi_neg, lo_pos, hi_pos, span_neg; int bounded; };
struct OsPlan { int passes; int shift[OS_MAXPASS]; int rb[OS_MAXPASS]; };

__device__ __forceinline__ unsigned os_key(const OsMap &m, float e, bool &outside)
{
    const unsigned o = f32_ord(e);
    if (!m.bounded) return o;
    if (e < 0.0f) { outside |= (o < m.lo_neg) | (o > m.hi_neg); const unsigned c = o < m.lo_neg ? m.lo_neg : (o > m.hi_neg ? m.hi_neg : o); return c - m.lo_neg; }
    outside |= (o < m.lo_pos) | (o > m.hi_pos);
    const unsigned c = o < m.lo_pos ? m.lo_pos : (o > m.hi_pos ? m.hi_pos : o);
    return m.span_neg + (c - m.lo_pos);
}
__device__ __forceinline__ float os_value(const OsMap &m, unsigned k)
{
    if (!m.bounded) return f32_unord(k);
    return f32_unord(k < m.span_neg ? k + m.lo_neg : k - m.span_neg + m.lo_pos);
}

#define OS_CTRL_WORDS 4

template <bool SKIPZ>
__global__ __launch_bounds__(OSP_THREADS) void k_os_prep(const float *__restrict__ x, long long n, unsigned *__restrict__ keys,
                                                         unsigned long long *__restrict__ ctrl, long long cap, OsMap km, int rb0, unsigned *__restrict__ ghist)
{
    __shared__ unsigned comp_s[SKIPZ ? OSP_TILE : 1];
    __shared__ unsigned hist_s[OS_MAXR];
    __shared__ unsigned wave_tot[OSP_THREADS / 64];
    __shared__ unsigned long long base_s;
    const int tid = threadIdx.x, lane = tid & 63, wv = tid >> 6;
    for (int i = tid; i < OS_MAXR; i += OSP_THREADS) hist_s[i] = 0u;
    __syncthreads();
    const bool vec = (reinterpret_cast<uintptr_t>(x) & 15) == 0;
    const float4 *x4 = reinterpret_cast<const float4 *>(x);
    const unsigned mask0 = (1u << rb0) - 1u;
    bool outside = false;
    const long long ntiles = (n + OSP_TILE - 1) / OSP_TILE;
    auto load_tile = [&](long long tt, float (&e)[OSP_PER]) {
        const long long tile0 = tt * OSP_TILE;
        if (tt >= ntiles) return;
        if (vec && tile0 + OSP_TILE <= n) {
#pragma unroll
            for (int j = 0; j < OSP_PER / 4; j++) {
                const float4 q = x4[(tile0 >> 2) + (long long)j * OSP_THREADS + tid];
                e[4 * j] = q.x; e[4 * j + 1] = q.y; e[4 * j + 2] = q.z; e[4 * j + 3] = q.w;
            }
        } else {
#pragma unroll
            for (int j = 0; j < OSP_PER; j++) {
                const long long i = tile0 + (long long)j * OSP_THREADS + tid;
                e[j] = i < n ? x[i] : 0.0f;
            }
        }
    };
    float en[OSP_PER];
    load_tile(blockIdx.x, en);
    for (long long t = blockIdx.x; t < ntiles; t += gridDim.x) {
        const long long tile0 = t * OSP_TILE;
        const bool fast = vec && tile0 + OSP_TILE <= n;
        float e[OSP_PER];
#pragma unroll
        for (int j = 0; j < OSP_PER; j++) e[j] = en[j];
        load_tile(t + gridDim.x, en);
        unsigned key[OSP_PER];
        unsigned take = 0;
#pragma unroll
        for (int j = 0; j < OSP_PER; j++) {
            bool ok = SKIPZ ? !(e[j] == 0.0f) : true;
            if (!SKIPZ && !fast) ok = tile0 + (long long)j * OSP_THREADS + tid < n;
            key[j] = 0u;
            if (ok) { key[j] = os_key(km, e[j], outside); take |= 1u << j; }
        }
#pragma unroll
        for (int j = 0; j < OSP_PER; j++)
            if (take & (1u << j)) atomicAdd(&hist_s[key[j] & mask0], 1u);
        if (SKIPZ) {
            const unsigned c = (unsigned)__popc(take);
            unsigned sc = c;
            for (int off = 1; off < 64; off <<= 1) { const unsigned o = __shfl_up(sc, off); if (lane >= off) sc += o; }
            if (lane == 63) wave_tot[wv] = sc;
            __syncthreads();
            unsigned pre = 0, tot = 0;
            for (int w = 0; w < OSP_THREADS / 64; w++) { const unsigned o = wave_tot[w]; if (w < wv) pre += o; tot += o; }
            if (tid == 0) base_s = atomicAdd(ctrl, (unsigned long long)tot);
            unsigned at = pre + sc - c;
#pragma unroll
            for (int j = 0; j < OSP_PER; j++)
                if (take & (1u << j)) comp_s[at++] = key[j];
            __syncthreads();
            const long long base = (long long)base_s;
            for (unsigned i = tid; i < tot; i += OSP_THREADS)
                if (base + i < cap) keys[base + i] = comp_s[i];
            __syncthreads();
        }
    }
    if (outside) atomicOr(ctrl + 1, 1ull);
    __syncthreads();
    for (int i = tid; i < OS_MAXR; i += OSP_THREADS) {
        const unsigned v = hist_s[i];
        if (v) atomicAdd(&ghist[i], v);
    }
}

#ifdef NNC_DIAG
__device__ unsigned long long *g_os_trace = nullptr;
extern "C" int nnc_debug_os_trace(void *buf)
{
    unsigned long long *p = reinterpret_cast<unsigned long long *>(buf);
// ... 180 lines not shown
            const long long per = ((n_zero + ntiles - 1) / ntiles + 3) & ~3ll;
            const long long z0 = tile * per, z1 = (z0 + per < n_zero) ? z0 + per : n_zero;
            float *zp = out_f + n_neg;
            if ((reinterpret_cast<uintptr_t>(zp) & 15) == 0) {
                for (long long i = z0 + 4ll * t; i + 3 < z1; i += 4ll * OS_THREADS) *reinterpret_cast<float4 *>(zp + i) = make_float4(0.f, 0.f, 0.f, 0.f);
                if (t == 0) for (long long i = z0 + ((z1 - z0) & ~3ll); i < z1; i++) zp[i] = 0.0f;
            } else {
                for (long long i = z0 + t; i < z1; i += OS_THREADS) zp[i] = 0.0f;
            }
        }
#pragma unroll
        for (int r = 0; r < DPT; r++) {
            const int d = t * DPT + r;
            if (d >= R) continue;
            unsigned excl = 0;
            if (tile > 0 && !(abl & 1)) {
                long long i = tile - 1;
                int polls = 0;
                bool done = false;
                while (!done) {
                    unsigned long long w[OS_LOOK];
#pragma unroll
                    for (int j = 0; j < OS_LOOK; j++) w[j] = (i - j >= 0) ? os_peek(&status[(size_t)(i - j) * R + d]) : 0ull;
                    int used = 0;
#pragma unroll
                    for (int j = 0; j < OS_LOOK; j++) {
                        if (!done && used == j) {
                            const unsigned tg = (unsigned)(w[j] >> 32);
                            if (tg == tagP) { excl += (unsigned)w[j]; done = true; }
                            else if (tg == tagA) { excl += (unsigned)w[j]; used = j + 1; }
                        }
                    }
                    if (!done) {
                        i -= used;
                        if (used == 0) {
                            if (++polls > OS_SPIN_LIMIT) { gave_up = true; done = true; }
                            __builtin_amdgcn_s_sleep(1);
                        } else polls = 0;
                    }
                }
                os_publish(&status[(size_t)tile * R + d], tagP, excl + tc[r]);
            }
            gpos[d] = gdig[d] + excl - (unsigned)tpre[d];
        }
        OS_STAMP(4);
        __syncthreads();
        OS_STAMP(5);
        for (int j = t; j < cnt_tile; j += OS_THREADS) {
            const unsigned kv = keys_s[j];
            const unsigned d = (kv >> shift) & MASK;
            const unsigned r = gpos[d] + (unsigned)j;
            if ((long long)r < n && !(abl & 4)) {
                if (DST == 0) out_k[r] = kv;
                else out_f[(long long)r + ((long long)r >= n_neg ? n_zero : 0)] = os_value(km, kv);
            }
        }
        OS_STAMP(6);
        __syncthreads();
        OS_STAMP(7);
    }
    if (gave_up) atomicOr(ctrl + 1, 2ull);
    if (nrb > 0) {
        for (int i = t; i <= (int)nmask; i += OS_THREADS) {
            const unsigned v = nhist[i];
            if (v) atomicAdd(&ghist_next[i], v);
        }
    }
}

static unsigned host_ord(float v)
{
    unsigned b;
    std::memcpy(&b, &v, 4);
    return (b & 0x80000000u) ? ~b : (b | 0x80000000u);
}

static size_t al256(size_t b) { return (b + 255) & ~(size_t)255; }

__global__ __launch_bounds__(256) void k_os_clear(uint4 *__restrict__ p, long long n16)
{
    const long long stride = (long long)gridDim.x * 256;
    for (long long i = (long long)blockIdx.x * 256 + threadIdx.x; i < n16; i += stride) p[i] = make_uint4(0u, 0u, 0u, 0u);
}
__global__ void k_os_verdict(const unsigned long long *__restrict__ ctrl, int32_t *__restrict__ flag) { *flag = reinterpret_cast<const int32_t *>(ctrl)[2]; }

static int os_cus()
{
    static int cus[64] = {0};
    int dev = 0;
    if (hipGetDevice(&dev) != hipSuccess || dev < 0 || dev >= 64) return 256;
    if (!cus[dev]) {
        int v = 0;
        if (hipDeviceGetAttribute(&v, hipDeviceAttributeMultiprocessorCount, dev) != hipSuccess || v <= 0) v = 256;
        cus[dev] = v;
    }
    return cus[dev];
}

static OsPlan os_plan(int bits)
{
    OsPlan pl;
    std::memset(&pl, 0, sizeof(pl));
    int rb;
    if (bits <= 8) { pl.passes = 1; rb = 8; }
    else if (bits <= 16) { pl.passes = 2; rb = 8; }
    else if (bits <= 18) { pl.passes = 2; rb = 9; }
    else if (bits <= 24) { pl.passes = 3; rb = 8; }
    else if (bits <= 27) { pl.passes = 3; rb = 9; }
    else { pl.passes = 4; rb = 8; }
    for (int p = 0; p < pl.passes; p++) { pl.shift[p] = p * rb; pl.rb[p] = rb; }
    return pl;
}

static size_t os_status_bytes(int64_t n_keys)
{
    const int64_t ntiles = (n_keys + OS_TILE - 1) / OS_TILE;
    return al256((size_t)std::max<int64_t>(ntiles, 1) * OS_MAXR * 8);
}
static size_t os_ws_bytes(int64_t n_keys)
{
    return 2 * al256((size_t)n_keys * 4 + 16) + al256(OS_CTRL_WORDS * 8) + al256((size_t)(OS_MAXPASS + 1) * OS_MAXR * 4) + os_status_bytes(n_keys) + 256;
}
static unsigned char *os_ws_base(void *ws) { return reinterpret_cast<unsigned char *>((reinterpret_cast<uintptr_t>(ws) + 255) & ~(uintptr_t)255); }

static int os_sort(const float *x, int64_t n, bool skip_zeros, int64_t n_neg, int64_t n_zero, const OsMap &km, int bits, float *sorted_out, void *ws,
                   size_t ws_bytes, int32_t *flag_dev, const char *who, void *stream)
{
    const int64_t n_keys = skip_zeros ? n - n_zero : n;
    if (!ws || ws_bytes < os_ws_bytes(n_keys)) return nnc_set_error_(NNC_ENOSPACE, (std::string(who) + ": workspace too small").c_str());
    hipStream_t s = reinterpret_cast<hipStream_t>(stream);
    unsigned char *b = os_ws_base(ws);
    unsigned *ka = reinterpret_cast<unsigned *>(b); b += al256((size_t)n_keys * 4 + 16);
    unsigned *kb = reinterpret_cast<unsigned *>(b); b += al256((size_t)n_keys * 4 + 16);
    unsigned long long *ctrl = reinterpret_cast<unsigned long long *>(b); b += al256(OS_CTRL_WORDS * 8);
    unsigned *ghist = reinterpret_cast<unsigned *>(b); b += al256((size_t)(OS_MAXPASS + 1) * OS_MAXR * 4);
    unsigned long long *status = reinterpret_cast<unsigned long long *>(b);
    hipError_t e;
    const size_t zero_bytes = al256(OS_CTRL_WORDS * 8) + al256((size_t)(OS_MAXPASS + 1) * OS_MAXR * 4) + os_status_bytes(n_keys);
    const long long n16 = (long long)(zero_bytes / 16);
    hipLaunchKernelGGL(k_os_clear, dim3((unsigned)std::min<long long>((n16 + 255) / 256, 1024)), dim3(256), 0, s, reinterpret_cast<uint4 *>(ctrl), n16);
    if ((e = hipGetLastError()) != hipSuccess) return nnc_set_error_(NNC_EHIP, hipGetErrorString(e));
    if (skip_zeros && n_zero > 0 && n_keys == 0 && (e = hipMemsetAsync(sorted_out + n_neg, 0, (size_t)n_zero * 4, s)) != hipSuccess) return nnc_set_error_(NNC_EHIP, hipGetErrorString(e));
    const OsPlan pl = os_plan(bits);
    int abl = 0;
#ifdef NNC_DIAG
    { const char *ev = getenv("NNC_OS_ABLATE"); abl = ev ? atoi(ev) : 0; }
#endif
    if (n_keys > 0) {
        const long long ptiles = (n + OSP_TILE - 1) / OSP_TILE;
        const int pgrid = (int)std::min<long long>(std::max<long long>(ptiles, 1), 2LL * os_cus());
        if (skip_zeros) hipLaunchKernelGGL((k_os_prep<true>), dim3(pgrid), dim3(OSP_THREADS), 0, s, x, (long long)n, ka, ctrl, (long long)n_keys, km, pl.rb[0], ghist);
        else hipLaunchKernelGGL((k_os_prep<false>), dim3(pgrid), dim3(OSP_THREADS), 0, s, x, (long long)n, (unsigned *)nullptr, ctrl, (long long)n_keys, km, pl.rb[0], ghist);
        if ((e = hipGetLastError()) != hipSuccess) return nnc_set_error_(NNC_EHIP, hipGetErrorString(e));
        const long long ntiles = (n_keys + OS_TILE - 1) / OS_TILE;
        const int grid = (int)std::min<long long>(ntiles, (long long)OS_BLOCKS_PER_CU * os_cus());
        const void *src = skip_zeros ? (const void *)ka : (const void *)x;
        unsigned *dst = skip_zeros ? kb : ka;
        for (int p = 0; p < pl.passes; p++) {
            const bool first_f = (p == 0 && !skip_zeros), last = (p == pl.passes - 1);
            void *o = last ? (void *)sorted_out : (void *)dst;
#define OS_LAUNCH(SRC, DST) do { \
                if (pl.rb[p] == 9) hipLaunchKernelGGL((k_os_pass<9, SRC, DST>), dim3(grid), dim3(OS_THREADS), 0, s, src, o, (long long)n_keys, pl.shift[p], p, last ? 0 : pl.rb[p + 1], \
                                                      ghist + (size_t)p * OS_MAXR, ghist + (size_t)(p + 1) * OS_MAXR, status, ctrl, km, (long long)(skip_zeros ? n_neg : n_keys), (long long)(skip_zeros ? n_zero : 0), abl); \
                else hipLaunchKernelGGL((k_os_pass<8, SRC, DST>), dim3(grid), dim3(OS_THREADS), 0, s, src, o, (long long)n_keys, pl.shift[p], p, last ? 0 : pl.rb[p + 1], \
                                        ghist + (size_t)p * OS_MAXR, ghist + (size_t)(p + 1) * OS_MAXR, status, ctrl, km, (long long)(skip_zeros ? n_neg : n_keys), (long long)(skip_zeros ? n_zero : 0), abl); \
            } while (0)
            if (first_f && last) OS_LAUNCH(1, 1);
            else if (first_f) OS_LAUNCH(1, 0);
            else if (last) OS_LAUNCH(0, 1);
            else OS_LAUNCH(0, 0);
#undef OS_LAUNCH
            if ((e = hipGetLastError()) != hipSuccess) return nnc_set_error_(NNC_EHIP, hipGetErrorString(e));
            src = dst;
            dst = (dst == ka) ? kb : ka;
        }
    }
    if (flag_dev) {
        hipLaunchKernelGGL(k_os_verdict, dim3(1), dim3(1), 0, s, (const unsigned long long *)ctrl, flag_dev);
        if ((e = hipGetLastError()) != hipSuccess) return nnc_set_error_(NNC_EHIP, hipGetErrorString(e));
    }
    return NNC_OK;
}

static OsMap os_identity()
{
    OsMap m;
    std::memset(&m, 0, sizeof(m));
    return m;
}

extern "C" size_t nnc_sort_workspace_bytes(int64_t n) { return n <= 0 ? 0 : os_ws_bytes(n); }

extern "C" int nnc_sort_f32(const float *x, int64_t n, float *sorted_out, void *ws, size_t ws_bytes, void *stream)
{
    if (n < 0 || n >= ((int64_t)1 << 31) || (n > 0 && (!x || !sorted_out))) return nnc_set_error_(NNC_EINVAL, "nnc_sort_f32: bad argument");
    if (n == 0) return NNC_OK;
    return os_sort(x, n, false, 0, 0, os_identity(), 32, sorted_out, ws, ws_bytes, nullptr, "nnc_sort_f32", stream);
}

extern "C" size_t nnc_sort_pruned_workspace_bytes(int64_t n, int64_t n_neg, int64_t n_zero)
{
    if (n <= 0 || n_neg < 0 || n_zero < 0 || n_neg + n_zero > n) return 0;
    return os_ws_bytes(n - n_zero);
}

extern "C" int nnc_sort_pruned_f32(const float *x, int64_t n, int64_t n_neg, int64_t n_zero, float *sorted_out, void *ws,
                                   size_t ws_bytes, void *stream)
{
    if (n < 0 || n_neg < 0 || n_zero < 0 || n_neg + n_zero > n || n >= ((int64_t)1 << 31) || (n > 0 && (!x || !sorted_out)))
        return nnc_set_error_(NNC_EINVAL, "nnc_sort_pruned_f32: bad argument");
    if (n == 0) return NNC_OK;
    return os_sort(x, n, true, n_neg, n_zero, os_identity(), 32, sorted_out, ws, ws_bytes, nullptr, "nnc_sort_pruned_f32", stream);
}

static int rs_bounds(float vmin, float vmax, float thr, int64_t n_neg, int64_t n_pos, OsMap *bd)
{
    if (!(thr > 0.0f) || !std::isfinite(thr) || !std::isfinite(vmin) || !std::isfinite(vmax)) return 0;
    OsMap b;
    std::memset(&b, 0, sizeof(b));
    b.bounded = 1;
    unsigned long long total = 0;
    if (n_neg > 0) {
        if (!(vmin <= -thr)) return 0;
        b.lo_neg = host_ord(vmin); b.hi_neg = host_ord(-thr);
        b.span_neg = b.hi_neg - b.lo_neg + 1u;
        total += b.span_neg;
    }
    if (n_pos > 0) {
        if (!(vmax >= thr)) return 0;
        b.lo_pos = host_ord(thr); b.hi_pos = host_ord(vmax);
        total += (unsigned long long)(b.hi_pos - b.lo_pos) + 1ull;
    }
    if (total == 0 || total > (1ull << 27)) return 0;
    int bits = 1;
    while ((1ull << bits) < total) bits++;
    *bd = b;
    return bits;
}

extern "C" int32_t nnc_sort_pruned_bounded_bits(float vmin, float vmax, float thr, int64_t n_neg, int64_t n_pos)
{
    OsMap b;
    return rs_bounds(vmin, vmax, thr, n_neg, n_pos, &b);
}

extern "C" size_t nnc_sort_pruned_bounded_workspace_bytes(int64_t n_nz)
{
    if (n_nz < 0) return 0;
    return os_ws_bytes(n_nz);
}

int nnc_sort_pruned_bounded_flagged_(const float *x, int64_t n, int64_t n_neg, int64_t n_zero, float vmin, float vmax, float thr,
                                     float *sorted_out, void *ws, size_t ws_bytes, int32_t *flag_dev, void *stream);
extern "C" int nnc_sort_pruned_bounded_f32(const float *x, int64_t n, int64_t n_neg, int64_t n_zero, float vmin, float vmax, float thr,
                                           float *sorted_out, void *ws, size_t ws_bytes, void *stream)
{
    return nnc_sort_pruned_bounded_flagged_(x, n, n_neg, n_zero, vmin, vmax, thr, sorted_out, ws, ws_bytes, nullptr, stream);
}

extern "C" const int32_t *nnc_sort_pruned_bounded_flag(void *ws, int64_t n_nonzero)
{
    if (!ws || n_nonzero < 0) return nullptr;
    unsigned char *b = os_ws_base(ws) + 2 * al256((size_t)n_nonzero * 4 + 16);
    return reinterpret_cast<const int32_t *>(b + 8);
}

int nnc_sort_pruned_bounded_flagged_(const float *x, int64_t n, int64_t n_neg, int64_t n_zero, float vmin, float vmax, float thr,
                                     float *sorted_out, void *ws, size_t ws_bytes, int32_t *flag_dev, void *stream)
{
    if (n < 0 || n_neg < 0 || n_zero < 0 || n_neg + n_zero > n || n >= ((int64_t)1 << 31) || (n > 0 && (!x || !sorted_out)))
        return nnc_set_error_(NNC_EINVAL, "nnc_sort_pruned_bounded_f32: bad argument");
    if (n == 0) return NNC_OK;
    const int64_t n_pos = n - n_neg - n_zero, n_nz = n_neg + n_pos;
    OsMap bd;
    std::memset(&bd, 0, sizeof(bd));
    bd.bounded = 1;
    const int bits = n_nz > 0 ? rs_bounds(vmin, vmax, thr, n_neg, n_pos, &bd) : 1;
    if (bits == 0) return nnc_set_error_(NNC_EINVAL, "nnc_sort_pruned_bounded_f32: bounds do not apply (see nnc_sort_pruned_bounded_bits)");
    return os_sort(x, n, true, n_neg, n_zero, bd, bits, sorted_out, ws, ws_bytes, flag_dev, "nnc_sort_pruned_bounded_f32", stream);
}
```

Baseline: 10.47 billion.

## Move layer density init and tail onto device, fusing launches and clearing sort head early

Adds a single-block kernel that computes the density-based centre initialisation on the device: it ranks the 32 steps in the sorted data, builds the CDF, interpolates it over 300 points and picks centres. This replaces the host-side CDF and density-init round trip and also initialises the k-means state in the same launch. It also adds a tail kernel that publishes counts and centres to pinned host memory with a ticket, a minmax variant that publishes to the host, and lets the sort skip its separate clear launch when the workspace head has already been zeroed. The aim is to remove host syncs and small kernel launches per layer, at the cost of more complex single-block device code and a changed sort workspace layout.

```diff
diff --git a/include/nnc.h b/include/nnc.h
--- a/include/nnc.h
+++ b/include/nnc.h
@@ -55,6 +55,8 @@
 
 int nnc_minmax_signs_f32(const float *x, int64_t n, float *out_dev, int64_t *signs_dev, void *ws, size_t ws_bytes,
                          void *stream);
+int nnc_minmax_signs_publish_f32(const float *x, int64_t n, float *out_dev, int64_t *signs_dev, void *ws, size_t ws_bytes, void *host_dst,
+                                 const void *extra_src, int extra_words, void *host_ticket, uint64_t ticket, void *stream);
 
 int32_t nnc_sort_pruned_bounded_bits(float vmin, float vmax, float thr, int64_t n_neg, int64_t n_pos);
 size_t nnc_sort_pruned_bounded_workspace_bytes(int64_t n_nonzero);
@@ -210,6 +212,10 @@
 int nnc_host_linspace_f32(float start, float stop, int32_t num, float *out);
 int nnc_host_cdf(const float *steps32, const int64_t *counts31, float *xnew300, double *cdf300);
 int nnc_host_density_init(const float *xnew300, const double *cdf300, int32_t bits, float *space_out);
+#define NNC_KM_DONE_OOB 4
+int nnc_layer_init_f32(void *ws, size_t ws_bytes, const nnc_kmeans_params *p, const float *x_sorted, const float *steps32,
+                       const int64_t *signs_dev, const int32_t *oob_flag_dev, int32_t bits, const float *centers_init,
+                       float *space_out_dev, void *stream);
 
 int32_t nnc_kmeanspp_trials(int32_t k);
 size_t nnc_kmeanspp_workspace_bytes(int64_t n, int32_t k);
diff --git a/neural_network_compression_amd/_native.py b/neural_network_compression_amd/_native.py
--- a/neural_network_compression_amd/_native.py
+++ b/neural_network_compression_amd/_native.py
@@ -130,6 +130,8 @@
     "nnc_minmax_workspace_bytes": (c_size, [c_i64]),
     "nnc_minmax_f32": (c_int, [c_void_p, c_i64, c_int, c_void_p, c_void_p, c_void_p, c_size, c_void_p]),
     "nnc_minmax_signs_f32": (c_int, [c_void_p, c_i64, c_void_p, c_void_p, c_void_p, c_size, c_void_p]),
+    "nnc_minmax_signs_publish_f32": (c_int, [c_void_p, c_i64, c_void_p, c_void_p, c_void_p, c_size, c_void_p, c_void_p, c_int, c_void_p,
+                                             ctypes.c_uint64, c_void_p]),
     "nnc_layer_stats_workspace_bytes": (c_size, [c_i64]),
     "nnc_layer_stats_f32": (c_int, [c_void_p, c_i64, c_void_p, c_void_p, c_void_p, c_size, c_void_p]),
     "nnc_rank_sorted_f32": (c_int, [c_void_p, c_i64, c_void_p, c_i32, c_void_p, c_void_p]),
@@ -183,6 +185,8 @@
     "nnc_host_linspace_f32": (c_int, [c_f32, c_f32, c_i32, c_void_p]),
     "nnc_host_cdf": (c_int, [c_void_p, c_void_p, c_void_p, c_void_p]),
     "nnc_host_density_init": (c_int, [c_void_p, c_void_p, c_i32, c_void_p]),
+    "nnc_layer_init_f32": (c_int, [c_void_p, c_size, ctypes.POINTER(KMeansParams), c_void_p, c_void_p, c_void_p, c_void_p, c_i32, c_void_p,
+                                   c_void_p, c_void_p]),
     "nnc_kmeanspp_trials": (c_i32, [c_i32]),
     "nnc_kmeanspp_workspace_bytes": (c_size, [c_i64, c_i32]),
     "nnc_kmeanspp_seed_f32": (c_int, [c_void_p, c_i64, c_f32, c_i32, c_i64, c_void_p, c_void_p, c_void_p, c_void_p, c_size, c_void_p]),
diff --git a/neural_network_compression_amd/csrc/nnc_hip.hip b/neural_network_compression_amd/csrc/nnc_hip.hip
--- a/neural_network_compression_amd/csrc/nnc_hip.hip
+++ b/neural_network_compression_amd/csrc/nnc_hip.hip
@@ -1848,11 +1848,13 @@
     return p->prefix_dev && p->n > 0 && p->n == p->n_total && km_fused(p) && (reinterpret_cast<uintptr_t>(x) & 15) == 0;
 }
 
-static int km_ensure_cells(KmWs *w, const nnc_kmeans_params *p, int which, void *stream)
+static int km_ensure_cells(KmWs *w, const nnc_kmeans_params *p, int which, void *stream, bool prepared = false)
 {
     if (!p->prefix_dev) return NNC_OK;
-    hipLaunchKernelGGL(k_cells_prepare, dim3(1), dim3(1), 0, S(stream), w, which);
-    LAUNCHCHK("k_cells_prepare");
+    if (!prepared) {
+        hipLaunchKernelGGL(k_cells_prepare, dim3(1), dim3(1), 0, S(stream), w, which);
+        LAUNCHCHK("k_cells_prepare");
+    }
     hipLaunchKernelGGL(k_cells, dim3(KM_GMAX / KM_THREADS), dim3(KM_THREADS), 0, S(stream), w, (nnc_kmeans_status *)nullptr,
                        (unsigned long long *)nullptr, 0ull, 1, which);
     LAUNCHCHK("k_cells");
@@ -1897,8 +1899,7 @@
     return NNC_OK;
 }
 
-__device__ __forceinline__ void km_init_body(KmWs *ws, const nnc_kmeans_params &p, int glog2, int rlog2, float inv,
-                                             const float *__restrict__ centers_init)
+__device__ __forceinline__ void km_init_state(KmWs *ws, const nnc_kmeans_params &p, int glog2, int rlog2, float inv)
 {
     const int tid = threadIdx.x;
     if (tid == 0) {
@@ -1907,10 +1908,6 @@
         ws->st.reloc_ties = 0; ws->st.reloc_multi = 0; ws->st.n_relocated = 0; ws->st.n_unproven = 0; ws->st.n_in_place = 0; ws->st.n_reloc_null = 0; ws->spec_go = 0;
         ws->p = p; ws->cur = 0; ws->glog2 = glog2; ws->rlog2 = rlog2; ws->inv = inv; ws->reloc_fail = 0; ws->cells_pending = 0;
     }
-    for (int j = tid; j < p.k; j += KM_THREADS) {
-        float c = centers_init[j] - p.x_mean;
-        ws->c[0][j] = c; ws->c[1][j] = c;
-    }
     for (int i = tid; i < KM_NSHARD * NNC_KMAX; i += KM_THREADS) {
         (&ws->shard_sum[0][0])[i] = 0; (&ws->shard_cnt[0][0])[i] = 0;
     }
@@ -1922,6 +1919,21 @@
     if (tid < 24) ws->kl_trace[tid] = 0ull;
 }
 
+__device__ __forceinline__ void km_init_centres(KmWs *ws, const nnc_kmeans_params &p, const float *__restrict__ centers_init)
+{
+    for (int j = threadIdx.x; j < p.k; j += KM_THREADS) {
+        float c = centers_init[j] - p.x_mean;
+        ws->c[0][j] = c; ws->c[1][j] = c;
+    }
+}
+
+__device__ __forceinline__ void km_init_body(KmWs *ws, const nnc_kmeans_params &p, int glog2, int rlog2, float inv,
+                                             const float *__restrict__ centers_init)
+{
+    km_init_state(ws, p, glog2, rlog2, inv);
+    km_init_centres(ws, p, centers_init);
+}
+
 __global__ __launch_bounds__(KM_THREADS) void k_km_init(KmWs *ws, nnc_kmeans_params p, int glog2, int rlog2, float inv,
                                                         const float *__restrict__ centers_init)
 {
@@ -1935,6 +1947,185 @@
     __syncthreads();
     __builtin_amdgcn_fence(__ATOMIC_ACQUIRE, "agent");
     km_finalize_kernel<KM_THREADS, false, false>(ws, FIN_INIT, 0, nullptr, nullptr, 0ull, 1 | (p.k << 8), nullptr, 0);
+}
+
+static float km_init_geometry(const nnc_kmeans_params *p, int *glog2, int *rlog2)
+{
+    km_defaults(p, glog2, rlog2);
+    float inv = 0.0f;
+    double range = (double)p->hi - (double)p->lo;
+    if (range > 0.0) inv = (float)(((double)(1 << *glog2)) / range * (1.0 - 1.0 / 1048576.0));
+    if (!std::isfinite(inv)) inv = 0.0f;
+    return inv;
+}
+
+__device__ __forceinline__ int li_lower_bound_f32(const float *a, int len, float v)
+{
+    int first = 0;
+    while (len > 0) { const int half = len >> 1; if (a[first + half] < v) { first += half + 1; len -= half + 1; } else len = half; }
+    return first;
+}
+__device__ __forceinline__ int li_lower_bound_f64(const double *a, int len, double v)
+{
+    int first = 0;
+    while (len > 0) { const int half = len >> 1; if (a[first + half] < v) { first += half + 1; len -= half + 1; } else len = half; }
+    return first;
+}
+
+__global__ __launch_bounds__(KM_THREADS) void k_layer_init(KmWs *ws, nnc_kmeans_params p, int glog2, int rlog2, float inv, const float *__restrict__ xs,
+                                                           const float *steps32, const long long *__restrict__ signs, const int *oob,
+                                                           const float *centers_in, float *__restrict__ space_out, int fused_finalize)
+{
+    __shared__ float steps_s[32], xnew_s[300], space_s[NNC_KMAX], mm_s[2];
+    __shared__ long long ranks_s[32], cnt_s[31], tot_s;
+    __shared__ double t_s[31], run_s[31], cdf_s[31], cdf300_s[300];
+    __shared__ int rising_s;
+    const int tid = threadIdx.x;
+    const int k = p.k;
+    const int stop = oob ? *oob : 0;
+    km_init_state(ws, p, glog2, rlog2, inv);
+    if (centers_in) {
+        for (int j = tid; j < k; j += KM_THREADS) space_s[j] = centers_in[j];
+    } else {
+        {
+            const int si = tid >> 5, j = tid & 31;
+            const float v = steps32[si];
+            if (j == 0) steps_s[si] = v;
+            long long lo = 0, hi = p.n;
+            for (;;) {
+                const long long len = hi - lo;
+                const bool last = len <= 32;
+                const long long q = last ? lo + j : lo + (len * (j + 1)) / 33;
+                const bool below = (!last || j < len) && xs[q] < v;
+                const unsigned long long b = __ballot(below);
+                const int cnt = __popc((unsigned)(b >> (threadIdx.x & 32)));
+                if (last) { lo += cnt; break; }
+                const long long nlo = cnt > 0 ? lo + (len * cnt) / 33 + 1 : lo;
+                if (cnt < 32) hi = lo + (len * (cnt + 1)) / 33;
+                lo = nlo;
+            }
+            if (j == 0) ranks_s[si] = lo;
+        }
+        __syncthreads();
+        if (tid < 31) cnt_s[tid] = ranks_s[tid + 1] - ranks_s[tid];
+        __syncthreads();
+        if (tid == 0) {
+            rising_s = 1;
+            const long long n_zero = signs[1];
+            for (int b = 0; b < 31; b++)
+                if (steps_s[b] <= 0.0f && 0.0f < steps_s[b + 1]) { cnt_s[b] -= n_zero; break; }
+            long long tot = 0;
+            for (int i = 0; i < 31; i++) tot += cnt_s[i];
+            tot_s = tot;
+            float xmin = steps_s[0], xmax = steps_s[0];
+            for (int i = 1; i < 31; i++) { const float b = steps_s[i]; xmin = (b < xmin) ? b : xmin; xmax = (xmax < b) ? b : xmax; }
+            mm_s[0] = xmin; mm_s[1] = xmax;
+        }
+        __syncthreads();
+        if (tid < 31) t_s[tid] = (double)cnt_s[tid] / (double)tot_s;
+        __syncthreads();
+        if (tid == 0) {
+            double acc = t_s[0];
+            run_s[0] = acc;
+            for (int i = 1; i < 31; i++) { acc = acc + t_s[i]; run_s[i] = acc; }
+        }
+        __syncthreads();
+        if (tid < 31) cdf_s[tid] = run_s[tid] / run_s[30];
+        float v = 0.0f;
+        if (tid < 300) {
+            const float start = mm_s[0], stopv = mm_s[1];
+            const float delta = stopv - start;
+            const float step = delta / 299.0f;
+            float y = (float)tid;
+            if (step == 0.0f) { y = y / 299.0f; y = y * delta; }
+            else y = y * step;
+            y = y + start;
+            v = (tid == 299) ? stopv : y;
+            xnew_s[tid] = v;
+        }
+        __syncthreads();
+        if (tid < 300) {
+            int idx = li_lower_bound_f32(steps_s, 31, v);
+            idx = min(max(idx, 1), 30);
+            const int lo = idx - 1, hi = idx;
+            const float dx = steps_s[hi] - steps_s[lo];
+            const double dy = cdf_s[hi] - cdf_s[lo];
+            const double slope = dy / (double)dx;
+            const float xr = v - steps_s[lo];
+            const double prod = slope * (double)xr;
+            cdf300_s[tid] = prod + cdf_s[lo];
+        }
+        __syncthreads();
+        if (tid >= 1 && tid < 300 && !(cdf300_s[tid - 1] <= cdf300_s[tid])) rising_s = 0;
+        __syncthreads();
+        const bool rising = rising_s != 0;
+        const int div = k - 1;
+        for (int t = tid; t < k; t += KM_THREADS) {
+            double tg;
+            if (div > 0) {
+                const double step = 1.0 / (double)div;
+                double y = (double)t;
+                y = y * step;
+                y = y + 0.0;
+                tg = (t == k - 1) ? 1.0 : y;
+            } else tg = 0.0;
+            int best;
+            if (rising) {
+                const int hi = li_lower_bound_f64(cdf300_s, 300, tg);
+                best = hi;
+                if (hi > 0) {
+                    const double dl = fabs(cdf300_s[hi - 1] - tg);
+                    if (hi == 300 || dl <= fabs(cdf300_s[hi] - tg)) {
+                        best = hi - 1;
+                        while (best > 0 && fabs(cdf300_s[best - 1] - tg) == dl) best--;
+                    }
+                }
+            } else {
+                best = 0;
+                double bd = fabs(cdf300_s[0] - tg);
+                for (int j = 1; j < 300; j++) {
+                    const double d = fabs(cdf300_s[j] - tg);
+                    if (d < bd) { bd = d; best = j; }
+                }
+            }
+            space_s[t] = xnew_s[best];
+        }
+    }
+    __syncthreads();
+    if (space_out) for (int j = tid; j < k; j += KM_THREADS) space_out[j] = space_s[j];
+    km_init_centres(ws, p, space_s);
+    if (stop) {
+        if (tid == 0) ws->st.done = NNC_KM_DONE_OOB;
+        return;
+    }
+    if (!fused_finalize) return;
+    __syncthreads();
+    __builtin_amdgcn_fence(__ATOMIC_ACQUIRE, "agent");
+    km_finalize_kernel<KM_THREADS, false, false>(ws, FIN_INIT, 0, nullptr, nullptr, 0ull, 1 | (p.k << 8), nullptr, 0);
+}
+
+extern "C" int nnc_layer_init_f32(void *ws, size_t ws_bytes, const nnc_kmeans_params *p, const float *x_sorted, const float *steps32,
+                                  const int64_t *signs_dev, const int32_t *oob_flag_dev, int32_t bits, const float *centers_init,
+                                  float *space_out_dev, void *stream)
+{
+    int rc = km_check(ws, p, "nnc_layer_init_f32");
+    if (rc) return rc;
+    if (ws_bytes < nnc_kmeans_workspace_bytes(p->k)) return fail(NNC_ENOSPACE, "nnc_layer_init_f32: workspace too small");
+    if (!centers_init) {
+        if (!x_sorted || !steps32 || !signs_dev || p->n < 1) return fail(NNC_EINVAL, "nnc_layer_init_f32: the density init needs the sorted copy, the 32 steps and the sign counts");
+        if (bits < 1 || bits > 10 || p->k != (1 << bits) + 1) return fail(NNC_EINVAL, "nnc_layer_init_f32: bits in 1..10 and k = 2^bits + 1");
+    }
+    if (!std::isfinite(p->x_mean) || !std::isfinite(p->tol) || !std::isfinite(p->lo) || !std::isfinite(p->hi))
+        return fail(NNC_EINVAL, "nnc_layer_init_f32: Input X contains NaN or infinity (mean / variance / range of the data are not finite)");
+    int glog2, rlog2;
+    const float inv = km_init_geometry(p, &glog2, &rlog2);
+    KmWs *w = reinterpret_cast<KmWs *>(ws);
+    const bool fused = p->k > 256 && !km_fused(p) && p->prefix_dev;
+    hipLaunchKernelGGL(k_layer_init, dim3(1), dim3(KM_THREADS), 0, S(stream), w, *p, glog2, rlog2, inv, x_sorted, steps32,
+                       reinterpret_cast<const long long *>(signs_dev), reinterpret_cast<const int *>(oob_flag_dev), centers_init, space_out_dev, fused ? 1 : 0);
+    LAUNCHCHK("k_layer_init");
+    if (fused) return NNC_OK;
+    return km_launch_finalize(w, p, FIN_INIT, 0, stream);
 }
 
 extern "C" int nnc_kmeans_init(void *ws, size_t ws_bytes, const nnc_kmeans_params *p, const float *centers_init_dev,
@@ -1947,11 +2138,7 @@
     if (!std::isfinite(p->x_mean) || !std::isfinite(p->tol) || !std::isfinite(p->lo) || !std::isfinite(p->hi))
         return fail(NNC_EINVAL, "nnc_kmeans_init: Input X contains NaN or infinity (mean / variance / range of the data are not finite)");
     int glog2, rlog2;
-    km_defaults(p, &glog2, &rlog2);
-    float inv = 0.0f;
-    double range = (double)p->hi - (double)p->lo;
-    if (range > 0.0) inv = (float)(((double)(1 << glog2)) / range * (1.0 - 1.0 / 1048576.0));
-    if (!std::isfinite(inv)) inv = 0.0f;
+    const float inv = km_init_geometry(p, &glog2, &rlog2);
     KmWs *w = reinterpret_cast<KmWs *>(ws);
 #ifndef KM_INIT_TWO
     if (p->k > 256 && !km_fused(p) && p->prefix_dev) {
@@ -2388,9 +2575,65 @@
     return NNC_OK;
 }
 
+__global__ __launch_bounds__(KM_THREADS) void k_layer_tail(KmWs *__restrict__ ws, int which, long long *__restrict__ counts, float *__restrict__ centers,
+                                                           long long *__restrict__ host_counts, unsigned long long *host_ticket, unsigned long long ticket,
+                                                           int prepare_cells)
+{
+    __shared__ long long cnt_s[NNC_KMAX];
+    KmTab *tab = &ws->tab[ws->cur ^ (which & 1)];
+    const int k = ws->p.k, ku = tab->ku;
+    const float *c = ws->c[ws->cur ^ (which & 1)];
+    const float mean = ws->p.x_mean;
+    const int qn = min(ws->q_n, (int)NNC_KMAX);
+    for (int r = threadIdx.x; r < qn; r += KM_THREADS) { ws->q_w0[r] = 0ull; ws->q_w1[r] = 0ull; ws->q_next[r] = 0; }
+    for (int j = threadIdx.x; j < NNC_KMAX; j += KM_THREADS) cnt_s[j] = 0;
+    __syncthreads();
+    if (threadIdx.x == 0) { ws->q_n = 0; if (prepare_cells) tab->n_ovf = 0; }
+    for (int p = threadIdx.x; p < ku; p += KM_THREADS) {
+        unsigned long long n = 0;
+        for (int sh = 0; sh < KM_NSHARD; sh++) {
+            n += ws->shard_cnt[sh][p];
+            ws->shard_sum[sh][p] = 0; ws->shard_cnt[sh][p] = 0;
+        }
+        const int o = tab->orig[p];
+        if (o >= 0 && o < k) cnt_s[o] = (long long)n;
+    }
+    __syncthreads();
+    float *host_centers = reinterpret_cast<float *>(host_counts + k);
+    for (int j = threadIdx.x; j < k; j += KM_THREADS) {
+        const long long n = cnt_s[j];
+        const float v = c[j] + mean;
+        counts[j] = n; centers[j] = v;
+        host_counts[j] = n; host_centers[j] = v;
+    }
+    __threadfence_system();
+    __syncthreads();
+    if (threadIdx.x == 0) *reinterpret_cast<volatile unsigned long long *>(host_ticket) = ticket;
+}
+
 static int km_assign(const float *x, void *ws, const nnc_kmeans_params *pp, int which, void *labels_out,
                      int label_bytes, float *quant_out, float *dist_out, int64_t *dist_hist4096_dev,
-                     const int *n_dev, void *stream)
+                     const int *n_dev, void *stream, bool cells_prepared = false);
+
+int nnc_layer_tail_assign_(const float *xs, const float *x, void *ws, const nnc_kmeans_params *pp, int64_t *counts_dev, float *centers_dev,
+                           void *host_counts, void *host_ticket, uint64_t ticket, void *labels_out, int label_bytes, float *quant_out, void *stream)
+{
+    int rc = km_check(ws, pp, "nnc_compress_layer_f32");
+    if (rc) return rc;
+    if (!counts_dev || !centers_dev || !host_counts || !host_ticket || (pp->n > 0 && !xs)) return fail(NNC_EINVAL, "nnc_compress_layer_f32: null pointer");
+    if ((rc = km_set_lds_attr())) return rc;
+    KmWs *w = reinterpret_cast<KmWs *>(ws);
+    const nnc_kmeans_params p = *pp;
+    if ((rc = km_launch_accumulate(xs, w, &p, stream, 2))) return rc;
+    hipLaunchKernelGGL(k_layer_tail, dim3(1), dim3(KM_THREADS), 0, S(stream), w, 0, reinterpret_cast<long long *>(counts_dev), centers_dev,
+                       reinterpret_cast<long long *>(host_counts), reinterpret_cast<unsigned long long *>(host_ticket), (unsigned long long)ticket, p.prefix_dev ? 1 : 0);
+    LAUNCHCHK("k_layer_tail");
+    return km_assign(x, ws, pp, 0, labels_out, label_bytes, quant_out, nullptr, nullptr, nullptr, stream, true);
+}
+
+static int km_assign(const float *x, void *ws, const nnc_kmeans_params *pp, int which, void *labels_out,
+                     int label_bytes, float *quant_out, float *dist_out, int64_t *dist_hist4096_dev,
+                     const int *n_dev, void *stream, bool cells_prepared)
 {
     int rc = km_check(ws, pp, "nnc_kmeans_assign");
     if (rc) return rc;
@@ -2408,7 +2651,7 @@
                      (reinterpret_cast<uintptr_t>(labels_out) & (size_t)(4 * label_bytes - 1)) == 0;
     int grid = km_grid(p.n, lds);
     KmWs *w = reinterpret_cast<KmWs *>(ws);
-    if ((rc = km_ensure_cells(w, &p, which, stream))) return rc;
+    if ((rc = km_ensure_cells(w, &p, which, stream, cells_prepared))) return rc;
     unsigned long long *dh = reinterpret_cast<unsigned long long *>(dist_hist4096_dev);
     if (dh) HIPCHK(hipMemsetAsync(dh, 0, 4096 * sizeof(int64_t), S(stream)));
     if (label_bytes == 2) {
diff --git a/neural_network_compression_amd/csrc/nnc_layer.hip b/neural_network_compression_amd/csrc/nnc_layer.hip
--- a/neural_network_compression_amd/csrc/nnc_layer.hip
+++ b/neural_network_compression_amd/csrc/nnc_layer.hip
@@ -12,8 +12,16 @@
 int nnc_set_error_(int code, const char *msg);
 int nnc_publish_bytes_(const void *src_dev, void *dst_host_mapped, int nbytes, void *host_ticket, uint64_t ticket, void *stream);
 int nnc_wait_ticket_(void *host_ticket, uint64_t ticket, void *stream);
-int nnc_sort_pruned_bounded_flagged_(const float *x, int64_t n, int64_t n_neg, int64_t n_zero, float vmin, float vmax, float thr,
-                                     float *sorted_out, void *ws, size_t ws_bytes, int32_t *flag_dev, void *stream);
+int nnc_prune_stats_publish_(float *x, int64_t n, float q, int std_smooth, uint8_t *mask, float *stats_dev, int64_t *nzeroed_dev,
+                             float *minmax4_dev, int64_t *signs_dev, void *ws, size_t ws_bytes, void *host_dst, const void *extra_src,
+                             int extra_words, void *host_ticket, uint64_t ticket, void *zero16, size_t zero_bytes, void *stream);
+int nnc_minmax_signs_publish_(const float *x, int64_t n, float *out_dev, int64_t *signs_dev, void *ws, size_t ws_bytes, void *host_dst,
+                              void *host_ticket, uint64_t ticket, void *zero16, size_t zero_bytes, void *stream);
+int nnc_layer_tail_assign_(const float *xs, const float *x, void *ws, const nnc_kmeans_params *pp, int64_t *counts_dev, float *centers_dev,
+                           void *host_counts, void *host_ticket, uint64_t ticket, void *labels_out, int label_bytes, float *quant_out, void *stream);
+int nnc_sort_head_(void *ws, size_t ws_bytes, void **head, size_t *head_bytes);
+int nnc_sort_cleared_(int kind, const float *x, int64_t n, int64_t n_neg, int64_t n_zero, float vmin, float vmax, float thr, float *sorted_out,
+                      void *ws, size_t ws_bytes, void *stream);
 extern "C" int nnc_host_linspace_f32(float start, float stop, int32_t num, float *out)
 {
     if (num < 0 || (num > 0 && !out)) return nnc_set_error_(NNC_EINVAL, "nnc_host_linspace_f32: bad argument");
@@ -147,7 +155,7 @@
 }
 
 struct LayerLayout {
-    size_t prune_ws, stats_out, stats_ws, sorted, sort_ws, km_ws, prefix, reloc, back, small_out, total;
+    size_t prune_ws, stats_out, stats_ws, sorted, sort_ws, km_ws, prefix, reloc, back, small_out, space, total;
     size_t prune_ws_bytes, stats_ws_bytes, sort_ws_bytes, km_ws_bytes, prefix_bytes, reloc_bytes;
 };
 
@@ -173,6 +181,7 @@
     L.reloc = take(std::max<size_t>(L.reloc_bytes, 16));
     L.back = take((size_t)k * 12);
     L.small_out = take(64 + 256);
+    L.space = take((size_t)k * 4);
     L.total = o + 256;
     return L;
 }
@@ -206,11 +215,12 @@
     hipStream_t s = reinterpret_cast<hipStream_t>(stream);
     unsigned char *wb = reinterpret_cast<unsigned char *>((reinterpret_cast<uintptr_t>(ws_dev) + 255) & ~(uintptr_t)255);
     unsigned char *hb = reinterpret_cast<unsigned char *>(host_pinned);
+    const bool short_tensor = n <= NNC_REF_NMAX && k <= NNC_REF_KMAX;
+    const bool long_path = !short_tensor && n >= 512;
     const float *h_f = reinterpret_cast<const float *>(hb + 512);
-    const int64_t *h_signs = reinterpret_cast<const int64_t *>(hb + 512 + 32);
-    const float *h_prune = reinterpret_cast<const float *>(hb + 512 + 48);
-    const int64_t *h_nz = reinterpret_cast<const int64_t *>(hb + 512 + 56);
-    int64_t *h_ranks = reinterpret_cast<int64_t *>(hb + 576);
+    const int64_t *h_signs = reinterpret_cast<const int64_t *>(hb + 512 + (long_path ? 24 : 32));
+    const float *h_prune = reinterpret_cast<const float *>(hb + 512 + (long_path ? 40 : 48));
+    const int64_t *h_nz = reinterpret_cast<const int64_t *>(hb + 512 + (long_path ? 48 : 56));
     void *h_ticket = hb + 504;
     auto read_back = [&](const void *src, void *dst, int nbytes) -> int {
         const uint64_t t = ++(*ticket_io);
@@ -226,11 +236,19 @@
     int64_t *signs = reinterpret_cast<int64_t *>(wb + L.stats_out + 32);
     float *pstats = reinterpret_cast<float *>(wb + L.stats_out + 48);
     int64_t *nzeroed = reinterpret_cast<int64_t *>(wb + L.stats_out + 56);
-    if (lp->prune)
+    const uint64_t t_mm = long_path ? ++(*ticket_io) : 0;
+    void *sort_head = nullptr;
+    size_t sort_head_bytes = 0;
+    if (long_path) LCHK(nnc_sort_head_(wb + L.sort_ws, L.sort_ws_bytes, &sort_head, &sort_head_bytes));
+    if (lp->prune && long_path)
+        LCHK(nnc_prune_stats_publish_(x, n, lp->q, lp->std_smooth ? 1 : 0, mask_out, pstats, nzeroed, out6 + 2, signs, wb + L.prune_ws, L.prune_ws_bytes,
+                                      hb + 512 + 8, pstats, 2, h_ticket, t_mm, sort_head, sort_head_bytes, stream));
+    else if (lp->prune)
         LCHK(nnc_prune_stats_f32(x, n, lp->q, lp->std_smooth ? 1 : 0, mask_out, pstats, nzeroed, out6 + 2, signs, wb + L.prune_ws, L.prune_ws_bytes, stream));
+    else if (long_path)
+        LCHK(nnc_minmax_signs_publish_(x, n, out6 + 2, signs, wb + L.stats_ws, L.stats_ws_bytes, hb + 512 + 8, h_ticket, t_mm, sort_head, sort_head_bytes, stream));
     else
         LCHK(nnc_minmax_signs_f32(x, n, out6 + 2, signs, wb + L.stats_ws, L.stats_ws_bytes, stream));
-    const bool short_tensor = n <= NNC_REF_NMAX && k <= NNC_REF_KMAX;
     if ((short_tensor && lp->mode != NNC_INIT_LINEAR) || (!short_tensor && n < 512)) {
         if (lp->prune) {
             LCHK(read_back(out6, hb + 512, 64));
@@ -273,8 +291,6 @@
         SideStream *side = nullptr;
         LCHK(side_stream(&side));
         LHIP(hipEventRecord(side->fork, s));
-        const uint64_t t_mm = ++(*ticket_io);
-        LCHK(nnc_publish_bytes_(out6 + 2, hb + 512 + 8, 56, h_ticket, t_mm, stream));
         LHIP(hipStreamWaitEvent(side->stream, side->fork, 0));
         struct SideJoin {
             SideStream *side; hipStream_t s; bool joined = false;
@@ -292,35 +308,27 @@
         const float xmin = h_f[2], xmax = h_f[3], min_nz = h_f[4], max_nz = h_f[5];
         const int64_t n_neg = h_signs[0], n_zero = h_signs[1];
         float *xs = reinterpret_cast<float *>(wb + L.sorted);
-        int32_t *oob_d = reinterpret_cast<int32_t *>(wb + L.stats_out + 336);
-        const int32_t *h_oob = reinterpret_cast<const int32_t *>(hb + 512 + 336);
         bool bounded = false;
         if (4 * n_zero >= n && lp->prune && nnc_sort_pruned_bounded_bits(xmin, xmax, h_prune[1], n_neg, n - n_neg - n_zero) > 0) {
-            LCHK(nnc_sort_pruned_bounded_flagged_(x, n, n_neg, n_zero, xmin, xmax, h_prune[1], xs, wb + L.sort_ws, L.sort_ws_bytes, oob_d, stream));
+            LCHK(nnc_sort_cleared_(2, x, n, n_neg, n_zero, xmin, xmax, h_prune[1], xs, wb + L.sort_ws, L.sort_ws_bytes, stream));
             bounded = true;
-        } else if (4 * n_zero >= n) LCHK(nnc_sort_pruned_f32(x, n, n_neg, n_zero, xs, wb + L.sort_ws, L.sort_ws_bytes, stream));
-        else LCHK(nnc_sort_f32(x, n, xs, wb + L.sort_ws, L.sort_ws_bytes, stream));
+        } else if (4 * n_zero >= n) LCHK(nnc_sort_cleared_(1, x, n, n_neg, n_zero, 0.0f, 0.0f, 0.0f, xs, wb + L.sort_ws, L.sort_ws_bytes, stream));
+        else LCHK(nnc_sort_cleared_(0, x, n, 0, 0, 0.0f, 0.0f, 0.0f, xs, wb + L.sort_ws, L.sort_ws_bytes, stream));
         LHIP(hipEventRecord(side->sorted, s));
         const bool with_prefix = (reinterpret_cast<uintptr_t>(xs) & 15) == 0;
-        int64_t *ranks_d = reinterpret_cast<int64_t *>(wb + L.stats_out + 64);
-        h_ranks = reinterpret_cast<int64_t *>(hb + 512 + 64);
-        float steps[32];
         if (lp->mode == NNC_INIT_DENSITY) {
             if (!std::isfinite(min_nz)) {
                 if (lp->prune) { res->sigma = h_prune[0]; res->threshold = h_prune[1]; res->n_zeroed = h_nz[0]; }
                 res->status = NNC_LAYER_HOST;
                 return NNC_OK;
             }
+            float steps[32];
             LCHK(nnc_host_linspace_f32(min_nz, max_nz, 32, steps));
             std::memcpy(h_steps, steps, 128);
-            LCHK(nnc_rank_sorted_f32(xs, n, h_steps, 32, ranks_d, stream));
-        }
-        const uint64_t t_rk = ++(*ticket_io);
-        LCHK(nnc_publish_bytes_(out6 + 2, hb + 512 + 8, 56 + 33 * 8 + 16, h_ticket, t_rk, stream));
+        }
         LCHK(nnc_wait_ticket_(h_ticket_side, t_mv, side->stream));
         const float mean = h_mv[0], var = h_mv[1];
         if (!std::isfinite(mean) || !std::isfinite(var) || !std::isfinite(xmin) || !std::isfinite(xmax)) {
-            LCHK(nnc_wait_ticket_(h_ticket, t_rk, stream));
             if (lp->prune) { res->sigma = h_prune[0]; res->threshold = h_prune[1]; res->n_zeroed = h_nz[0]; }
             res->status = NNC_LAYER_HOST;
             return NNC_OK;
@@ -334,47 +342,31 @@
         p.grid_log2 = 0; p.replicas_log2 = -1; p.flags = lp->km_flags & (NNC_KM_TWO_LAUNCH | NNC_KM_LOOP);
         p.x_mean = mean; p.tol = tol; p.lo = lo; p.hi = hi;
         if (with_prefix) {
-            LHIP(hipStreamWaitEvent(side->stream, side->sorted, 0));
-            LCHK(nnc_kmeans_prefix_build(xs, &p, reinterpret_cast<int64_t *>(wb + L.prefix), side->stream));
+            LCHK(nnc_kmeans_prefix_build(xs, &p, reinterpret_cast<int64_t *>(wb + L.prefix), stream));
             p.prefix_dev = reinterpret_cast<int64_t *>(wb + L.prefix);
-        }
-        LHIP(hipEventRecord(side->join, side->stream));
-        LCHK(nnc_wait_ticket_(h_ticket, t_rk, stream));
-        if (bounded && *h_oob) {
-            if (lp->prune) { res->sigma = h_prune[0]; res->threshold = h_prune[1]; res->n_zeroed = h_nz[0]; }
-            res->status = NNC_LAYER_HOST;
-            return NNC_OK;
         }
         if (lp->mode == NNC_INIT_LINEAR) {
             LCHK(nnc_host_linspace_f32(xmin, xmax, k, space));
-        } else {
-            int64_t counts31[31];
-            for (int b = 0; b < 31; b++) counts31[b] = h_ranks[b + 1] - h_ranks[b];
-            for (int b = 0; b < 31; b++)
-                if (steps[b] <= 0.0f && 0.0f < steps[b + 1]) { counts31[b] -= n_zero; break; }
-            float xnew[300];
-            double cdf[300];
-            LCHK(nnc_host_cdf(steps, counts31, xnew, cdf));
-            LCHK(nnc_host_density_init(xnew, cdf, lp->bits, space));
-        }
-        std::memcpy(h_space, space, (size_t)k * 4);
-        LCHK(nnc_kmeans_init(wb + L.km_ws, L.km_ws_bytes, &p, h_space, stream));
+            std::memcpy(h_space, space, (size_t)k * 4);
+        }
+        LHIP(hipStreamWaitEvent(side->stream, side->sorted, 0));
+        LCHK(nnc_layer_init_f32(wb + L.km_ws, L.km_ws_bytes, &p, xs, h_steps, signs, bounded ? nnc_sort_pruned_bounded_flag(wb + L.sort_ws, n - n_zero) : nullptr,
+                                lp->bits, lp->mode == NNC_INIT_LINEAR ? h_space : nullptr, reinterpret_cast<float *>(wb + L.space), side->stream));
+        LHIP(hipEventRecord(side->join, side->stream));
         LHIP(hipStreamWaitEvent(s, side->join, 0));
         side_join.joined = true;
         nnc_kmeans_status st;
         std::memset(&st, 0, sizeof(st));
         int32_t nwin = 0;
         LCHK(nnc_kmeans_fit(xs, wb + L.km_ws, &p, 16, 1, L.reloc_bytes ? wb + L.reloc : nullptr, L.reloc_bytes, hb, ticket_io, &st, &nwin, stream));
-        if (!st.done) {
+        if (!st.done || st.done == NNC_KM_DONE_OOB) {
             if (lp->prune) { res->sigma = h_prune[0]; res->threshold = h_prune[1]; res->n_zeroed = h_nz[0]; }
             res->status = NNC_LAYER_HOST;
             return NNC_OK;
         }
-        LCHK(nnc_kmeans_get_centers(wb + L.km_ws, 0, 0, centers_d, stream));
-        LCHK(nnc_kmeans_label_counts(xs, wb + L.km_ws, &p, 0, counts_d, stream));
         const uint64_t t_back = ++(*ticket_io);
-        LCHK(nnc_publish_bytes_(back, hb + 1024, (int)al((size_t)k * 12), h_ticket, t_back, stream));
-        LCHK(nnc_kmeans_assign(x, wb + L.km_ws, &p, 0, labels_out, res->label_bytes, lp->want_values ? values_out : nullptr, nullptr, nullptr, stream));
+        LCHK(nnc_layer_tail_assign_(xs, x, wb + L.km_ws, &p, counts_d, centers_d, hb + 1024, h_ticket, t_back, labels_out, res->label_bytes,
+                                    lp->want_values ? values_out : nullptr, stream));
         LCHK(nnc_wait_ticket_(h_ticket, t_back, stream));
         res->n_iter = st.iter; res->stop = st.done; res->n_relocations = nwin - st.n_reloc_null; res->n_reloc_windowed = nwin - st.n_reloc_null;
         res->reloc_ties = st.reloc_ties; res->reloc_multi = st.reloc_multi;
diff --git a/neural_network_compression_amd/csrc/nnc_reduce.hip b/neural_network_compression_amd/csrc/nnc_reduce.hip
--- a/neural_network_compression_amd/csrc/nnc_reduce.hip
+++ b/neural_network_compression_amd/csrc/nnc_reduce.hip
@@ -340,8 +340,12 @@
 
 __global__ __launch_bounds__(256) void k_minmax_final(const MinMaxPartial *__restrict__ part, int nparts,
                                                       float *__restrict__ out, long long *__restrict__ count,
-                                                      long long *__restrict__ signs)
-{
+                                                      long long *__restrict__ signs, unsigned long long *host_dst = nullptr,
+                                                      const unsigned long long *__restrict__ extra_src = nullptr, int extra_words = 0,
+                                                      unsigned long long *host_ticket = nullptr, unsigned long long ticket = 0ull,
+                                                      uint4 *__restrict__ zero16 = nullptr, int n16 = 0)
+{
+    for (int i = threadIdx.x; i < n16; i += 256) zero16[i] = make_uint4(0u, 0u, 0u, 0u);
     float mn = INFINITY, mx = -INFINITY, mn_nz = INFINITY, mx_nz = -INFINITY;
     unsigned long long cnt = 0, neg = 0, zer = 0;
     for (int i = threadIdx.x; i < nparts; i += 256) {
@@ -369,6 +373,14 @@
         out[0] = p.mn; out[1] = p.mx;
         if (count) *count = (long long)p.cnt;
         if (signs) { signs[0] = (long long)p.neg; signs[1] = (long long)p.zer; out[2] = p.mn_nz; out[3] = p.mx_nz; }
+        if (host_dst && signs) {
+            float *hf = reinterpret_cast<float *>(host_dst);
+            hf[0] = p.mn; hf[1] = p.mx; hf[2] = p.mn_nz; hf[3] = p.mx_nz;
+            host_dst[2] = p.neg; host_dst[3] = p.zer;
+            for (int i = 0; i < extra_words; i++) host_dst[4 + i] = extra_src[i];
+            __threadfence_system();
+            *reinterpret_cast<volatile unsigned long long *>(host_ticket) = ticket;
+        }
     }
 }
 
@@ -380,8 +392,10 @@
     return (size_t)(cu_count() * 8 + 8) * sizeof(MinMaxPartial);
 }
 
+struct MmPublish { void *host_dst; const void *extra_src; int extra_words; void *host_ticket; uint64_t ticket; void *zero16; size_t zero_bytes; };
+
 static int minmax_impl(const float *x, int64_t n, int skip_zeros, float *out_dev, int64_t *count_dev, int64_t *signs_dev,
-                       void *ws, size_t ws_bytes, void *stream)
+                       void *ws, size_t ws_bytes, void *stream, const MmPublish *pub = nullptr)
 {
     if (n <= 0 || !x || !out_dev || !ws) return fail(NNC_EINVAL, "nnc_minmax_f32: bad argument (n must be > 0)");
     if (ws_bytes < nnc_minmax_workspace_bytes(n)) return fail(NNC_ENOSPACE, "nnc_minmax_f32: workspace too small");
@@ -392,7 +406,10 @@
     else NNC_LAUNCH_PROF(NNC_PROF_MINMAX, (k_minmax<false>), dim3(grid), dim3(256), 0, S(stream), x, n, skip_zeros, part);
     LAUNCHCHK("k_minmax");
     hipLaunchKernelGGL(k_minmax_final, dim3(1), dim3(256), 0, S(stream), part, grid, out_dev, reinterpret_cast<long long *>(count_dev),
-                       reinterpret_cast<long long *>(signs_dev));
+                       reinterpret_cast<long long *>(signs_dev), reinterpret_cast<unsigned long long *>(pub ? pub->host_dst : nullptr),
+                       reinterpret_cast<const unsigned long long *>(pub ? pub->extra_src : nullptr), pub ? pub->extra_words : 0,
+                       reinterpret_cast<unsigned long long *>(pub ? pub->host_ticket : nullptr), (unsigned long long)(pub ? pub->ticket : 0),
+                       reinterpret_cast<uint4 *>(pub ? pub->zero16 : nullptr), pub ? (int)(pub->zero_bytes / 16) : 0);
     LAUNCHCHK("k_minmax_final");
     return NNC_OK;
 }
@@ -408,6 +425,21 @@
 {
     if (!signs_dev) return fail(NNC_EINVAL, "nnc_minmax_signs_f32: null signs_dev");
     return minmax_impl(x, n, 0, out_dev, nullptr, signs_dev, ws, ws_bytes, stream);
+}
+
+static bool mm_publish_ok(const MmPublish &pub)
+{
+    return pub.host_dst && pub.host_ticket && pub.extra_words >= 0 && (pub.extra_words == 0 || pub.extra_src) &&
+           ((reinterpret_cast<uintptr_t>(pub.host_dst) | reinterpret_cast<uintptr_t>(pub.host_ticket) | reinterpret_cast<uintptr_t>(pub.extra_src)) & 7) == 0 &&
+           (pub.zero_bytes == 0 || pub.zero16) && (reinterpret_cast<uintptr_t>(pub.zero16) & 15) == 0 && (pub.zero_bytes & 15) == 0 && pub.zero_bytes <= ((size_t)1 << 20);
+}
+
+extern "C" int nnc_minmax_signs_publish_f32(const float *x, int64_t n, float *out_dev, int64_t *signs_dev, void *ws, size_t ws_bytes, void *host_dst,
+                                            const void *extra_src, int extra_words, void *host_ticket, uint64_t ticket, void *stream)
+{
+    const MmPublish pub = {host_dst, extra_src, extra_words, host_ticket, ticket, nullptr, 0};
+    if (!signs_dev || !mm_publish_ok(pub)) return fail(NNC_EINVAL, "nnc_minmax_signs_f32: null signs_dev, or null / unaligned host block");
+    return minmax_impl(x, n, 0, out_dev, nullptr, signs_dev, ws, ws_bytes, stream, &pub);
 }
 
 template <bool VEC>
@@ -480,8 +512,34 @@
 
 extern "C" size_t nnc_prune_stats_workspace_bytes(int64_t n) { return ((nnc_prune_workspace_bytes(n) + 255) & ~(size_t)255) + nnc_minmax_workspace_bytes(n); }
 
+int nnc_minmax_signs_publish_(const float *x, int64_t n, float *out_dev, int64_t *signs_dev, void *ws, size_t ws_bytes, void *host_dst,
+                              void *host_ticket, uint64_t ticket, void *zero16, size_t zero_bytes, void *stream)
+{
+    const MmPublish pub = {host_dst, nullptr, 0, host_ticket, ticket, zero16, zero_bytes};
+    if (!signs_dev || !mm_publish_ok(pub)) return fail(NNC_EINVAL, "nnc_minmax_signs_f32: null signs_dev, or null / unaligned host block");
+    return minmax_impl(x, n, 0, out_dev, nullptr, signs_dev, ws, ws_bytes, stream, &pub);
+}
+
+static int prune_stats_impl(float *x, int64_t n, float q, int std_smooth, uint8_t *mask, float *stats_dev, int64_t *nzeroed_dev,
+                            float *minmax4_dev, int64_t *signs_dev, void *ws, size_t ws_bytes, void *stream, const MmPublish *pub);
+
 extern "C" int nnc_prune_stats_f32(float *x, int64_t n, float q, int std_smooth, uint8_t *mask, float *stats_dev, int64_t *nzeroed_dev,
                                    float *minmax4_dev, int64_t *signs_dev, void *ws, size_t ws_bytes, void *stream)
+{
+    return prune_stats_impl(x, n, q, std_smooth, mask, stats_dev, nzeroed_dev, minmax4_dev, signs_dev, ws, ws_bytes, stream, nullptr);
+}
+
+int nnc_prune_stats_publish_(float *x, int64_t n, float q, int std_smooth, uint8_t *mask, float *stats_dev, int64_t *nzeroed_dev,
+                             float *minmax4_dev, int64_t *signs_dev, void *ws, size_t ws_bytes, void *host_dst, const void *extra_src,
+                             int extra_words, void *host_ticket, uint64_t ticket, void *zero16, size_t zero_bytes, void *stream)
+{
+    const MmPublish pub = {host_dst, extra_src, extra_words, host_ticket, ticket, zero16, zero_bytes};
+    if (!mm_publish_ok(pub)) return fail(NNC_EINVAL, "nnc_prune_stats_f32: null / unaligned host block");
+    return prune_stats_impl(x, n, q, std_smooth, mask, stats_dev, nzeroed_dev, minmax4_dev, signs_dev, ws, ws_bytes, stream, &pub);
+}
+
+static int prune_stats_impl(float *x, int64_t n, float q, int std_smooth, uint8_t *mask, float *stats_dev, int64_t *nzeroed_dev,
+                            float *minmax4_dev, int64_t *signs_dev, void *ws, size_t ws_bytes, void *stream, const MmPublish *pub)
 {
     if (n <= 0 || !x || !mask || !stats_dev || !minmax4_dev || !signs_dev || !ws) return fail(NNC_EINVAL, "nnc_prune_stats_f32: bad argument (n must be > 0)");
     if (ws_bytes < nnc_prune_stats_workspace_bytes(n)) return fail(NNC_ENOSPACE, "nnc_prune_stats_f32: workspace too small");
@@ -508,7 +566,10 @@
     if (vec) NNC_LAUNCH_PROF(NNC_PROF_THRESHOLD, (k_threshold_stats<true>), dim3(grid), dim3(256), 0, S(stream), x, n, stats_dev + 1, mask, reinterpret_cast<unsigned long long *>(nzeroed_dev), part);
     else NNC_LAUNCH_PROF(NNC_PROF_THRESHOLD, (k_threshold_stats<false>), dim3(grid), dim3(256), 0, S(stream), x, n, stats_dev + 1, mask, reinterpret_cast<unsigned long long *>(nzeroed_dev), part);
     LAUNCHCHK("k_threshold_stats");
-    hipLaunchKernelGGL(k_minmax_final, dim3(1), dim3(256), 0, S(stream), part, grid, minmax4_dev, (long long *)nullptr, reinterpret_cast<long long *>(signs_dev));
+    hipLaunchKernelGGL(k_minmax_final, dim3(1), dim3(256), 0, S(stream), part, grid, minmax4_dev, (long long *)nullptr, reinterpret_cast<long long *>(signs_dev),
+                       reinterpret_cast<unsigned long long *>(pub ? pub->host_dst : nullptr), reinterpret_cast<const unsigned long long *>(pub ? pub->extra_src : nullptr),
+                       pub ? pub->extra_words : 0, reinterpret_cast<unsigned long long *>(pub ? pub->host_ticket : nullptr), (unsigned long long)(pub ? pub->ticket : 0),
+                       reinterpret_cast<uint4 *>(pub ? pub->zero16 : nullptr), pub ? (int)(pub->zero_bytes / 16) : 0);
     LAUNCHCHK("k_minmax_final");
     return NNC_OK;
 }
diff --git a/neural_network_compression_amd/csrc/nnc_sort.hip b/neural_network_compression_amd/csrc/nnc_sort.hip
--- a/neural_network_compression_amd/csrc/nnc_sort.hip
+++ b/neural_network_compression_amd/csrc/nnc_sort.hip
@@ -65,8 +65,10 @@
 
 template <bool SKIPZ>
 __global__ __launch_bounds__(OSP_THREADS) void k_os_prep(const float *__restrict__ x, long long n, unsigned *__restrict__ keys,
-                                                         unsigned long long *__restrict__ ctrl, long long cap, OsMap km, int rb0, unsigned *__restrict__ ghist)
-{
+                                                         unsigned long long *__restrict__ ctrl, long long cap, OsMap km, int rb0, unsigned *__restrict__ ghist,
+                                                         uint4 *__restrict__ zero16, long long n16)
+{
+    for (long long i = (long long)blockIdx.x * OSP_THREADS + threadIdx.x; i < n16; i += (long long)gridDim.x * OSP_THREADS) zero16[i] = make_uint4(0u, 0u, 0u, 0u);
     __shared__ unsigned comp_s[SKIPZ ? OSP_TILE : 1];
     __shared__ unsigned hist_s[OS_MAXR];
     __shared__ unsigned wave_tot[OSP_THREADS / 64];
@@ -413,7 +415,6 @@
     const long long stride = (long long)gridDim.x * 256;
     for (long long i = (long long)blockIdx.x * 256 + threadIdx.x; i < n16; i += stride) p[i] = make_uint4(0u, 0u, 0u, 0u);
 }
-__global__ void k_os_verdict(const unsigned long long *__restrict__ ctrl, int32_t *__restrict__ flag) { *flag = reinterpret_cast<const int32_t *>(ctrl)[2]; }
 
 static int os_cus()
 {
@@ -453,24 +454,33 @@
     return 2 * al256((size_t)n_keys * 4 + 16) + al256(OS_CTRL_WORDS * 8) + al256((size_t)(OS_MAXPASS + 1) * OS_MAXR * 4) + os_status_bytes(n_keys) + 256;
 }
 static unsigned char *os_ws_base(void *ws) { return reinterpret_cast<unsigned char *>((reinterpret_cast<uintptr_t>(ws) + 255) & ~(uintptr_t)255); }
+static size_t os_head_bytes() { return al256(OS_CTRL_WORDS * 8) + al256((size_t)(OS_MAXPASS + 1) * OS_MAXR * 4); }
+static size_t os_zero_bytes(int64_t n_keys) { return os_head_bytes() + os_status_bytes(n_keys); }
+
+static int os_clear(void *ws, int64_t n_keys, hipStream_t s)
+{
+    const long long n16 = (long long)(os_zero_bytes(n_keys) / 16);
+    hipLaunchKernelGGL(k_os_clear, dim3((unsigned)std::min<long long>((n16 + 255) / 256, 1024)), dim3(256), 0, s, reinterpret_cast<uint4 *>(os_ws_base(ws)), n16);
+    const hipError_t e = hipGetLastError();
+    return e != hipSuccess ? nnc_set_error_(NNC_EHIP, hipGetErrorString(e)) : NNC_OK;
+}
 
 static int os_sort(const float *x, int64_t n, bool skip_zeros, int64_t n_neg, int64_t n_zero, const OsMap &km, int bits, float *sorted_out, void *ws,
-                   size_t ws_bytes, int32_t *flag_dev, const char *who, void *stream)
+                   size_t ws_bytes, bool head_cleared, const char *who, void *stream)
 {
     const int64_t n_keys = skip_zeros ? n - n_zero : n;
     if (!ws || ws_bytes < os_ws_bytes(n_keys)) return nnc_set_error_(NNC_ENOSPACE, (std::string(who) + ": workspace too small").c_str());
     hipStream_t s = reinterpret_cast<hipStream_t>(stream);
     unsigned char *b = os_ws_base(ws);
-    unsigned *ka = reinterpret_cast<unsigned *>(b); b += al256((size_t)n_keys * 4 + 16);
-    unsigned *kb = reinterpret_cast<unsigned *>(b); b += al256((size_t)n_keys * 4 + 16);
     unsigned long long *ctrl = reinterpret_cast<unsigned long long *>(b); b += al256(OS_CTRL_WORDS * 8);
     unsigned *ghist = reinterpret_cast<unsigned *>(b); b += al256((size_t)(OS_MAXPASS + 1) * OS_MAXR * 4);
-    unsigned long long *status = reinterpret_cast<unsigned long long *>(b);
+    unsigned long long *status = reinterpret_cast<unsigned long long *>(b); b += os_status_bytes(n_keys);
+    unsigned *ka = reinterpret_cast<unsigned *>(b); b += al256((size_t)n_keys * 4 + 16);
+    unsigned *kb = reinterpret_cast<unsigned *>(b);
     hipError_t e;
-    const size_t zero_bytes = al256(OS_CTRL_WORDS * 8) + al256((size_t)(OS_MAXPASS + 1) * OS_MAXR * 4) + os_status_bytes(n_keys);
-    const long long n16 = (long long)(zero_bytes / 16);
-    hipLaunchKernelGGL(k_os_clear, dim3((unsigned)std::min<long long>((n16 + 255) / 256, 1024)), dim3(256), 0, s, reinterpret_cast<uint4 *>(ctrl), n16);
-    if ((e = hipGetLastError()) != hipSuccess) return nnc_set_error_(NNC_EHIP, hipGetErrorString(e));
+    if (!head_cleared) { const int rc = os_clear(ws, n_keys, s); if (rc) return rc; }
+    uint4 *zero16 = head_cleared ? reinterpret_cast<uint4 *>(status) : nullptr;
+    const long long n16 = head_cleared ? (long long)(os_status_bytes(n_keys) / 16) : 0;
     if (skip_zeros && n_zero > 0 && n_keys == 0 && (e = hipMemsetAsync(sorted_out + n_neg, 0, (size_t)n_zero * 4, s)) != hipSuccess) return nnc_set_error_(NNC_EHIP, hipGetErrorString(e));
     const OsPlan pl = os_plan(bits);
     int abl = 0;
@@ -480,8 +490,8 @@
     if (n_keys > 0) {
         const long long ptiles = (n + OSP_TILE - 1) / OSP_TILE;
         const int pgrid = (int)std::min<long long>(std::max<long long>(ptiles, 1), 2LL * os_cus());
-        if (skip_zeros) hipLaunchKernelGGL((k_os_prep<true>), dim3(pgrid), dim3(OSP_THREADS), 0, s, x, (long long)n, ka, ctrl, (long long)n_keys, km, pl.rb[0], ghist);
-        else hipLaunchKernelGGL((k_os_prep<false>), dim3(pgrid), dim3(OSP_THREADS), 0, s, x, (long long)n, (unsigned *)nullptr, ctrl, (long long)n_keys, km, pl.rb[0], ghist);
+        if (skip_zeros) hipLaunchKernelGGL((k_os_prep<true>), dim3(pgrid), dim3(OSP_THREADS), 0, s, x, (long long)n, ka, ctrl, (long long)n_keys, km, pl.rb[0], ghist, zero16, n16);
+        else hipLaunchKernelGGL((k_os_prep<false>), dim3(pgrid), dim3(OSP_THREADS), 0, s, x, (long long)n, (unsigned *)nullptr, ctrl, (long long)n_keys, km, pl.rb[0], ghist, zero16, n16);
         if ((e = hipGetLastError()) != hipSuccess) return nnc_set_error_(NNC_EHIP, hipGetErrorString(e));
         const long long ntiles = (n_keys + OS_TILE - 1) / OS_TILE;
         const int grid = (int)std::min<long long>(ntiles, (long long)OS_BLOCKS_PER_CU * os_cus());
@@ -506,10 +516,6 @@
             dst = (dst == ka) ? kb : ka;
         }
     }
-    if (flag_dev) {
-        hipLaunchKernelGGL(k_os_verdict, dim3(1), dim3(1), 0, s, (const unsigned long long *)ctrl, flag_dev);
-        if ((e = hipGetLastError()) != hipSuccess) return nnc_set_error_(NNC_EHIP, hipGetErrorString(e));
-    }
     return NNC_OK;
 }
 
@@ -526,7 +532,7 @@
 {
     if (n < 0 || n >= ((int64_t)1 << 31) || (n > 0 && (!x || !sorted_out))) return nnc_set_error_(NNC_EINVAL, "nnc_sort_f32: bad argument");
     if (n == 0) return NNC_OK;
-    return os_sort(x, n, false, 0, 0, os_identity(), 32, sorted_out, ws, ws_bytes, nullptr, "nnc_sort_f32", stream);
+    return os_sort(x, n, false, 0, 0, os_identity(), 32, sorted_out, ws, ws_bytes, false, "nnc_sort_f32", stream);
 }
 
 extern "C" size_t nnc_sort_pruned_workspace_bytes(int64_t n, int64_t n_neg, int64_t n_zero)
@@ -541,7 +547,7 @@
     if (n < 0 || n_neg < 0 || n_zero < 0 || n_neg + n_zero > n || n >= ((int64_t)1 << 31) || (n > 0 && (!x || !sorted_out)))
         return nnc_set_error_(NNC_EINVAL, "nnc_sort_pruned_f32: bad argument");
     if (n == 0) return NNC_OK;
-    return os_sort(x, n, true, n_neg, n_zero, os_identity(), 32, sorted_out, ws, ws_bytes, nullptr, "nnc_sort_pruned_f32", stream);
+    return os_sort(x, n, true, n_neg, n_zero, os_identity(), 32, sorted_out, ws, ws_bytes, false, "nnc_sort_pruned_f32", stream);
 }
 
 static int rs_bounds(float vmin, float vmax, float thr, int64_t n_neg, int64_t n_pos, OsMap *bd)
@@ -581,23 +587,8 @@
     return os_ws_bytes(n_nz);
 }
 
-int nnc_sort_pruned_bounded_flagged_(const float *x, int64_t n, int64_t n_neg, int64_t n_zero, float vmin, float vmax, float thr,
-                                     float *sorted_out, void *ws, size_t ws_bytes, int32_t *flag_dev, void *stream);
-extern "C" int nnc_sort_pruned_bounded_f32(const float *x, int64_t n, int64_t n_neg, int64_t n_zero, float vmin, float vmax, float thr,
-                                           float *sorted_out, void *ws, size_t ws_bytes, void *stream)
-{
-    return nnc_sort_pruned_bounded_flagged_(x, n, n_neg, n_zero, vmin, vmax, thr, sorted_out, ws, ws_bytes, nullptr, stream);
-}
-
-extern "C" const int32_t *nnc_sort_pruned_bounded_flag(void *ws, int64_t n_nonzero)
-{
-    if (!ws || n_nonzero < 0) return nullptr;
-    unsigned char *b = os_ws_base(ws) + 2 * al256((size_t)n_nonzero * 4 + 16);
-    return reinterpret_cast<const int32_t *>(b + 8);
-}
-
-int nnc_sort_pruned_bounded_flagged_(const float *x, int64_t n, int64_t n_neg, int64_t n_zero, float vmin, float vmax, float thr,
-                                     float *sorted_out, void *ws, size_t ws_bytes, int32_t *flag_dev, void *stream)
+static int os_sort_bounded(const float *x, int64_t n, int64_t n_neg, int64_t n_zero, float vmin, float vmax, float thr, float *sorted_out, void *ws,
+                           size_t ws_bytes, bool head_cleared, void *stream)
 {
     if (n < 0 || n_neg < 0 || n_zero < 0 || n_neg + n_zero > n || n >= ((int64_t)1 << 31) || (n > 0 && (!x || !sorted_out)))
         return nnc_set_error_(NNC_EINVAL, "nnc_sort_pruned_bounded_f32: bad argument");
@@ -608,5 +599,34 @@
     bd.bounded = 1;
     const int bits = n_nz > 0 ? rs_bounds(vmin, vmax, thr, n_neg, n_pos, &bd) : 1;
     if (bits == 0) return nnc_set_error_(NNC_EINVAL, "nnc_sort_pruned_bounded_f32: bounds do not apply (see nnc_sort_pruned_bounded_bits)");
-    return os_sort(x, n, true, n_neg, n_zero, bd, bits, sorted_out, ws, ws_bytes, flag_dev, "nnc_sort_pruned_bounded_f32", stream);
-}
+    return os_sort(x, n, true, n_neg, n_zero, bd, bits, sorted_out, ws, ws_bytes, head_cleared, "nnc_sort_pruned_bounded_f32", stream);
+}
+
+extern "C" int nnc_sort_pruned_bounded_f32(const float *x, int64_t n, int64_t n_neg, int64_t n_zero, float vmin, float vmax, float thr,
+                                           float *sorted_out, void *ws, size_t ws_bytes, void *stream)
+{
+    return os_sort_bounded(x, n, n_neg, n_zero, vmin, vmax, thr, sorted_out, ws, ws_bytes, false, stream);
+}
+
+extern "C" const int32_t *nnc_sort_pruned_bounded_flag(void *ws, int64_t n_nonzero)
+{
+    if (!ws || n_nonzero < 0) return nullptr;
+    return reinterpret_cast<const int32_t *>(os_ws_base(ws) + 8);
+}
+
+int nnc_sort_head_(void *ws, size_t ws_bytes, void **head, size_t *head_bytes)
+{
+    if (!ws || !head || !head_bytes || ws_bytes < os_head_bytes() + 256) return nnc_set_error_(NNC_ENOSPACE, "nnc_sort_head_: workspace too small");
+    *head = os_ws_base(ws);
+    *head_bytes = os_head_bytes();
+    return NNC_OK;
+}
+
+int nnc_sort_cleared_(int kind, const float *x, int64_t n, int64_t n_neg, int64_t n_zero, float vmin, float vmax, float thr, float *sorted_out,
+                      void *ws, size_t ws_bytes, void *stream)
+{
+    if (n < 1 || n >= ((int64_t)1 << 31) || !x || !sorted_out || n_neg < 0 || n_zero < 0 || n_neg + n_zero > n) return nnc_set_error_(NNC_EINVAL, "nnc_sort_cleared_: bad argument");
+    if (kind == 2) return os_sort_bounded(x, n, n_neg, n_zero, vmin, vmax, thr, sorted_out, ws, ws_bytes, true, stream);
+    if (kind == 1) return os_sort(x, n, true, n_neg, n_zero, os_identity(), 32, sorted_out, ws, ws_bytes, true, "nnc_sort_pruned_f32", stream);
+    return os_sort(x, n, false, 0, 0, os_identity(), 32, sorted_out, ws, ws_bytes, true, "nnc_sort_f32", stream);
+}
```

Measured after the change: 10.59 billion, median of 6. 1.01x the previous value.
